# FelixBronnhuber/RenderBaby

Measured on AMD Instinct MI355X. Metric: Msamples/s (ray-segments/s), higher is better.
Workload: dtype f32; 1 GPU; C2 Cornell box (12 tris, 8 spheres, 1 area light), 1920x1080, 1024 spp, 8 bounces; width=1920, height=1080, spp=1024, max_depth=8, parallelism=single GPU, stripe_rows=8, walk=library default, tree_builder=, device=AMD Radeon Graphics (gfx950:sramecc+:xnack-, 256 CUs)

## Files before the change

include/rb_abi.h:

```cpp
#ifndef RB_ABI_H
#define RB_ABI_H

#include <stddef.h>
#include <stdint.h>

#ifdef __cplusplus
extern "C" {
#endif


typedef struct rb_camera {
    float pane_distance;
    float pane_width;
    float _pad0[2];
    float pos[3];
    float _pad1;
    float dir[3];
    float _pad2;
} rb_camera;

typedef struct rb_uniforms {
    uint32_t width;
    uint32_t height;
    uint32_t total_samples;
// ... 248 lines not shown
int rb_get_stats(rb_engine* e, rb_stats* out);
int rb_reset_stats(rb_engine* e);
int rb_last_dispatch_ms(rb_engine* e, float* ms);

int rb_bvh_build(const rb_gpu_triangle* tris, size_t n_tris,
                 rb_bvh_node* nodes_out, size_t nodes_capacity, size_t* n_nodes,
                 uint32_t* indices_out);

int rb_bvh_build_canonical(const rb_gpu_triangle* tris, size_t n_tris,
                           rb_bvh_node* nodes_out, size_t nodes_capacity, size_t* n_nodes,
                           uint32_t* indices_out);
int rb_bvh_build_device(int32_t device, const rb_gpu_triangle* tris, size_t n_tris,
                        rb_bvh_node* nodes_out, size_t nodes_capacity, size_t* n_nodes,
                        uint32_t* indices_out);
int rb_engine_tree(rb_engine* e, rb_bvh_node* nodes_out, size_t nodes_capacity, size_t* n_nodes,
                   uint32_t* indices_out, size_t indices_capacity, size_t* n_indices);
const char* rb_tree_builder(const rb_engine* e, float* build_ms);

int rb_debug_chunk_tree(const rb_gpu_triangle* tris, size_t n_tris, const rb_bvh_node* nodes, size_t n_nodes, const uint32_t* indices,
                        size_t n_indices, uint64_t out6[6]);
int rb_debug_engine_chunk_tree(rb_engine* e, uint64_t out6[6]);
typedef struct rb_debug_own_node {
    float lmin[3];
    uint32_t left;
    float lmax[3];
    uint32_t right;
    float rmin[3];
    float left_fa;
    float rmax[3];
    float right_fa;
} rb_debug_own_node;
typedef struct rb_debug_sphere_node {
    float cx[4], cy[4], cz[4], hx[4], hy[4], hz[4];
    uint32_t ref[4];
    uint32_t axes;
    uint32_t _pad[3];
} rb_debug_sphere_node;
int rb_debug_own_tree(const rb_gpu_triangle* tris, size_t n_tris, const rb_bvh_node* nodes, size_t n_nodes, const uint32_t* indices,
                      size_t n_indices, rb_debug_own_node* nodes_out, size_t nodes_capacity, uint32_t* slots_out, size_t slots_capacity,
                      uint32_t* slot_meta_out, size_t slot_meta_capacity, uint64_t counts3[3], uint32_t root_depth[2], float bounds6[6]);
int rb_debug_engine_own_tree(rb_engine* e, rb_debug_own_node* nodes_out, size_t nodes_capacity, uint32_t* slots_out, size_t slots_capacity,
                             uint32_t* slot_meta_out, size_t slot_meta_capacity, uint64_t counts3[3], uint32_t root_depth[2], float bounds6[6]);
int rb_debug_sphere_tree(const rb_sphere* spheres, size_t n, rb_debug_sphere_node* nodes_out, size_t nodes_capacity, float* leaf_out,
                         uint32_t* id_out, size_t spheres_capacity, uint64_t counts2[2], uint32_t root_depth[2]);
int rb_debug_engine_sphere_tree(rb_engine* e, rb_debug_sphere_node* nodes_out, size_t nodes_capacity, float* leaf_out, uint32_t* id_out,
                                size_t spheres_capacity, uint64_t counts2[2], uint32_t root_depth[2]);
const char* rb_chunk_tree_builder(const rb_engine* e, float* build_ms);
int rb_measure_l1_gather(int32_t device, uint64_t table_bytes, double* accesses_per_s);
int rb_debug_math(const float* a, const float* b, float* out8n, uint32_t n);
int rb_debug_walk_profile(uint64_t out64[64], int reset);
int rb_debug_rcp_exhaustive(uint32_t biased_exponent, uint32_t* out16);
int rb_debug_rcp_det_exhaustive(uint32_t biased_exponent, uint32_t* out16);
int rb_debug_triangle_trip(uint32_t n, uint32_t seed, uint32_t* out32);
int rb_debug_root_box(const float* rays, uint32_t n, const float* box6, uint32_t* out);
int rb_debug_normalize_sites(const float* xyz, uint32_t n, uint32_t n_unit, uint32_t seed0, uint32_t n_seeds, uint32_t* out16);
int rb_measure_salu_mix(int32_t device, uint32_t scalar_per_16, uint32_t branch, double* out3);
int rb_debug_rnd_pm1_exhaustive(uint32_t* out16);
int rb_debug_div_exhaustive(uint32_t b_begin, uint32_t b_count, uint32_t ea, uint32_t eb, uint32_t a_begin,
                            uint32_t a_count, unsigned long long* out16);

const char* rb_last_kernel_name(const rb_engine* e);

typedef struct rb_ray { float origin[3]; float _pad0; float dir[3]; float _pad1; } rb_ray;
enum { RB_HIT_NONE = 0, RB_HIT_GROUND = 1, RB_HIT_TRIANGLE = 2, RB_HIT_SPHERE = 3, RB_HIT_LIGHT = 4,
       RB_HIT_INVALID = 0xFFFFFFFFu };
typedef struct rb_hit {
    float t;
    uint32_t kind;
    uint32_t prim;
    uint32_t mesh;
    float u, v;
    uint32_t _pad[2];
    float normal[3];
    float _pad1;
} rb_hit;
typedef struct rb_surface {
    float albedo[3];
    uint32_t flags;
    float emissive[3];
    int32_t texture_index;
    float uv[2];
    float _pad[2];
} rb_surface;
int rb_cast_rays(rb_engine* e, const rb_ray* rays, size_t n, rb_hit* hits_out, rb_surface* surf_out);
int rb_render_hits(rb_engine* e, rb_hit* hits_out, rb_surface* surf_out);
int rb_pick(rb_engine* e, uint32_t px, uint32_t py, rb_hit* hit_out, rb_surface* surf_out);
const char* rb_last_query_kernel_name(const rb_engine* e);
int rb_last_query_ms(rb_engine* e, float* ms);

enum { RB_OCCL_VISIBLE = 0, RB_OCCL_OCCLUDED = 1, RB_OCCL_INVALID = 255 };
enum { RB_MASK_GROUND = 1, RB_MASK_TRIANGLES = 2, RB_MASK_SPHERES = 4, RB_MASK_LIGHTS = 8, RB_MASK_ALL = 15 };
int rb_occluded(rb_engine* e, const rb_ray* rays, const float* tmax, size_t n, uint32_t mask, uint8_t* out);
int rb_occluded_device(rb_engine* e, const rb_ray* d_rays, const float* d_tmax, size_t n, uint32_t mask, uint8_t* d_out);
int rb_cast_rays_device(rb_engine* e, const rb_ray* d_rays, size_t n, rb_hit* d_hits, rb_surface* d_surf);

typedef struct rb_radiance { float sum[3]; float weight; } rb_radiance;
#define RB_TRACE_PIECE_ITEMS (1u << 24)
int rb_trace_rays(rb_engine* e, const rb_ray* rays, const uint32_t* seeds, size_t n, uint32_t first_sample, uint32_t samples,
                  rb_radiance* out);
int rb_trace_rays_device(rb_engine* e, const rb_ray* d_rays, const uint32_t* d_seeds, size_t n, uint32_t first_sample,
                         uint32_t samples, rb_radiance* d_out);

enum { RB_CAM_PERSPECTIVE = 1, RB_CAM_ORTHO = 2, RB_CAM_EQUIRECT = 3 };
enum { RB_CAM_NO_JITTER = 1u };
typedef struct rb_camera_ex {
    uint32_t kind, width, height, flags;
    float pos[3];     float tan_half_fov;
    float right[3];   float half_width;
    float up[3];      float half_height;
    float forward[3]; float lens_radius;
    float focus_distance;
    uint32_t _reserved[3];
} rb_camera_ex;
#define RB_CAMERA_PIECE_ITEMS (1u << 23)
// ... 299 lines not shown
```

renderbaby_amd/_lib.py:

```python
import ctypes as C
import os

from . import abi

_HERE = os.path.dirname(os.path.abspath(__file__))
LIB_PATH = os.environ.get("RB_LIBRARY_PATH") or os.path.join(_HERE, "librenderbaby_hip.so")
_lib = None


P = C.POINTER
vp, u32, i32, sz = C.c_void_p, C.c_uint32, C.c_int, C.c_size_t
SIGNATURES = {
    "rb_create": (vp, [P(abi.Config)]),
    "rb_create_ex": (vp, [P(abi.Config), P(abi.Options)]),
    "rb_create_multi": (vp, [P(abi.Config), P(abi.Options), P(C.c_int32), u32]),
    "rb_comm_unique_id": (i32, [vp]),
    "rb_comm_available": (i32, []),
    "rb_comm_init_rank": (i32, [vp, vp, u32, u32]),
    "rb_comm_info": (i32, [vp, P(u32), P(u32), P(C.c_float)]),
    "rb_destroy": (None, [vp]),
    "rb_update": (i32, [vp, P(abi.Config)]),
    "rb_render": (i32, [vp, vp]),
    "rb_render_config": (i32, [vp, P(abi.Config), vp]),
    "rb_iter_begin": (i32, [vp, P(abi.Config)]),
    "rb_iter_has_next": (i32, [vp]),
    "rb_iter_next": (i32, [vp, vp]),
    "rb_iter_destroy": (None, [vp]),
    "rb_iter_set_passes_per_frame": (i32, [vp, u32]),
    "rb_last_error": (C.c_char_p, [vp]),
    "rb_get_size": (i32, [vp, P(u32), P(u32)]),
    "rb_clear": (i32, [vp]),
    "rb_dispatch": (i32, [vp, u32, u32]),
    "rb_reserve": (i32, [vp, u32]),
    "rb_sync": (i32, [vp]),
    "rb_read_rgba": (i32, [vp, vp]),
    "rb_read_accumulation": (i32, [vp, vp]),
    "rb_device_rgba": (i32, [vp, P(vp), P(sz)]),
    "rb_host_alloc": (vp, [sz]),
    "rb_host_free": (None, [vp]),
    "rb_local_rows": (i32, [vp, P(u32), P(u32)]),
    "rb_global_row": (i32, [vp, u32, P(u32)]),
    "rb_shard_layout": (i32, [u32, u32, u32, u32, P(u32), P(u32)]),
    "rb_shard_global_row": (u32, [u32, u32, u32, u32]),
    "rb_get_stats": (i32, [vp, P(abi.Stats)]),
    "rb_reset_stats": (i32, [vp]),
    "rb_last_dispatch_ms": (i32, [vp, P(C.c_float)]),
    "rb_bvh_build": (i32, [vp, sz, vp, sz, P(sz), vp]),
    "rb_bvh_build_canonical": (i32, [vp, sz, vp, sz, P(sz), vp]),
    "rb_bvh_build_device": (i32, [i32, vp, sz, vp, sz, P(sz), vp]),
    "rb_engine_tree": (i32, [vp, vp, sz, P(sz), vp, sz, P(sz)]),
    "rb_tree_builder": (C.c_char_p, [vp, vp]),
    "rb_debug_chunk_tree": (i32, [vp, sz, vp, sz, vp, sz, vp]),
    "rb_measure_l1_gather": (i32, [i32, C.c_uint64, P(C.c_double)]),
    "rb_debug_math": (i32, [vp, vp, vp, u32]),
    "rb_debug_walk_profile": (i32, [vp, i32]),
    "rb_debug_rcp_exhaustive": (i32, [u32, vp]),
    "rb_debug_rcp_det_exhaustive": (i32, [u32, vp]),
    "rb_debug_rnd_pm1_exhaustive": (i32, [vp]),
    "rb_debug_triangle_trip": (i32, [u32, u32, vp]),
    "rb_debug_root_box": (i32, [vp, u32, vp, vp]),
    "rb_debug_normalize_sites": (i32, [vp, u32, u32, u32, u32, vp]),
    "rb_measure_salu_mix": (i32, [i32, u32, u32, P(C.c_double)]),
    "rb_debug_div_exhaustive": (i32, [u32, u32, u32, u32, u32, u32, vp]),
    "rb_last_kernel_name": (C.c_char_p, [vp]),
    "rb_cast_rays": (i32, [vp, vp, sz, vp, vp]),
    "rb_render_hits": (i32, [vp, vp, vp]),
    "rb_pick": (i32, [vp, u32, u32, vp, vp]),
    "rb_occluded": (i32, [vp, vp, vp, sz, u32, vp]),
    "rb_occluded_device": (i32, [vp, vp, vp, sz, u32, vp]),
    "rb_cast_rays_device": (i32, [vp, vp, sz, vp, vp]),
    "rb_trace_rays": (i32, [vp, vp, vp, sz, u32, u32, vp]),
    "rb_trace_rays_device": (i32, [vp, vp, vp, sz, u32, u32, vp]),
    "rb_camera_rays": (i32, [i32, vp, C.c_uint64, sz, u32, u32, vp, vp]),
    "rb_trace_camera": (i32, [vp, vp, C.c_uint64, sz, u32, u32, vp]),
    "rb_trace_camera_device": (i32, [vp, vp, C.c_uint64, sz, u32, u32, vp]),
    "rb_last_camera_rays_ms": (i32, [vp, P(C.c_float)]),
    "rb_hemisphere_rays": (i32, [i32, vp, vp, sz, vp, u32, u32, vp, vp]),
    "rb_trace_hemisphere": (i32, [vp, vp, vp, sz, vp, u32, u32, vp]),
    "rb_trace_hemisphere_device": (i32, [vp, vp, vp, sz, vp, u32, u32, vp]),
    "rb_openness_hemisphere": (i32, [vp, vp, vp, sz, vp, u32, u32, vp]),
    "rb_openness_hemisphere_device": (i32, [vp, vp, vp, sz, vp, u32, u32, vp]),
    "rb_scene_emitters": (i32, [vp, vp, sz, P(sz)]),
    "rb_scene_emitters_device": (i32, [vp, vp, sz, vp]),
    "rb_light_rays": (i32, [i32, vp, sz, vp, vp, sz, vp, u32, u32, vp, vp, vp]),
    "rb_direct_light": (i32, [vp, vp, sz, vp, vp, sz, vp, u32, u32, vp]),
    "rb_direct_light_device": (i32, [vp, vp, sz, vp, vp, sz, vp, u32, u32, vp]),
    "rb_lightmap_surfels": (i32, [i32, vp, sz, vp, sz, vp, vp, vp]),
    "rb_lightmap_surfels_device": (i32, [vp, vp, vp, vp]),
    "rb_lightmap_resolve": (i32, [i32, u32, u32, vp, u32, vp]),
    "rb_bake_lightmap": (i32, [vp, vp, u32, u32, vp, vp]),
    "rb_bake_lightmap_device": (i32, [vp, vp, u32, u32, vp, vp]),
    "rb_last_lightmap_ms": (i32, [vp, P(C.c_float), P(C.c_float)]),
    "rb_probe_rays": (i32, [i32, vp, vp, sz, u32, u32, vp, vp]),
    "rb_bake_probes": (i32, [vp, vp, vp, sz, u32, u32, vp]),
    "rb_bake_probes_device": (i32, [vp, vp, vp, sz, u32, u32, vp]),
    "rb_last_probe_project_ms": (i32, [vp, P(C.c_float)]),
    "rb_probe_coefficients": (i32, [i32, vp, sz, vp]),
    "rb_probe_coefficients_device": (i32, [vp, vp, sz, vp]),
    "rb_light_points": (i32, [i32, vp, vp, vp, sz, vp]),
    "rb_light_points_device": (i32, [vp, vp, vp, vp, sz, vp]),
    "rb_bake_probe_depth": (i32, [vp, vp, vp, sz, u32, u32, C.c_float, vp]),
    "rb_bake_probe_depth_device": (i32, [vp, vp, vp, sz, u32, u32, C.c_float, vp]),
    "rb_last_probe_depth_project_ms": (i32, [vp, P(C.c_float)]),
    "rb_probe_moments": (i32, [i32, vp, sz, vp, vp]),
    "rb_probe_moments_device": (i32, [vp, vp, sz, vp, vp]),
    "rb_light_points_visible": (i32, [i32, vp, vp, vp, vp, sz, vp, vp]),
    "rb_light_points_visible_device": (i32, [vp, vp, vp, vp, vp, sz, vp, vp]),
    "rb_last_query_kernel_name": (C.c_char_p, [vp]),
    "rb_last_query_ms": (i32, [vp, P(C.c_float)]),
    "rb_denoise_default_params": (i32, [vp]),
    "rb_denoise_buffers": (i32, [i32, vp, u32, u32, vp, vp, vp, vp]),
    "rb_denoise": (i32, [vp, vp, vp, vp]),
# ... 62 lines not shown
```

renderbaby_amd/abi.py:

```python
import ctypes as C

import numpy as np

f4, u4, i4 = np.float32, np.uint32, np.int32

CAMERA = np.dtype([
    ("pane_distance", f4), ("pane_width", f4), ("_pad0", f4, (2,)),
    ("pos", f4, (3,)), ("_pad1", f4), ("dir", f4, (3,)), ("_pad2", f4)])

UNIFORMS = np.dtype([
    ("width", u4), ("height", u4), ("total_samples", u4), ("color_hash_enabled", u4),
    ("camera", CAMERA),
    ("spheres_count", u4), ("triangles_count", u4), ("bvh_node_count", u4),
    ("bvh_triangle_count", u4), ("bvh_root", u4), ("ground_height", f4),
    ("ground_enabled", u4), ("checkerboard_enabled", u4),
    ("sky_color", f4, (3,)), ("max_depth", u4),
    ("checkerboard_color_1", f4, (3,)), ("_pad1", u4),
    ("checkerboard_color_2", f4, (3,)), ("_pad2", u4)])

MATERIAL = np.dtype([
    ("ambient", f4, (3,)), ("_pad0", f4), ("diffuse", f4, (3,)), ("_pad1", f4),
    ("specular", f4, (3,)), ("shininess", f4), ("emissive", f4, (3,)), ("ior", f4),
    ("opacity", f4), ("illum", u4), ("texture_index", i4), ("_pad2", u4)])

# ... 37 lines not shown
PROBE_PIECE_ITEMS = 1 << 23
PROBE_GRID = np.dtype([("origin", f4, (3,)), ("_pad0", u4), ("step", f4, (3,)), ("_pad1", u4), ("counts", u4, (3,)), ("flags", u4)])
LIT = np.dtype([("value", f4, (3,)), ("weight", f4)])
LIGHT_PIECE_POINTS = 1 << 22
PROBE_DEPTH = np.dtype([("texel", f4, (64, 4))])
LIGHT_VISIBILITY = np.dtype([("normal_bias", f4), ("min_visibility", f4), ("flags", u4), ("_pad", u4)])
VIS_NO_WRAP, VIS_NO_DEPTH = 1, 2
EMITTER = np.dtype([("a", f4, (3,)), ("kind", u4), ("b", f4, (3,)), ("prim", u4), ("c", f4, (3,)), ("area", f4),
                    ("emissive", f4, (3,)), ("_pad", f4)])
LIGHT_PARAMS = np.dtype([("offset", f4), ("shorten", f4), ("mask", u4), ("flags", u4), ("_reserved", u4, (4,))])
MAX_EMITTERS = 1 << 24
OCCL_VISIBLE, OCCL_OCCLUDED, OCCL_INVALID = 0, 1, 255
MASK_GROUND, MASK_TRIANGLES, MASK_SPHERES, MASK_LIGHTS, MASK_ALL = 1, 2, 4, 8, 15
GUIDE = np.dtype([("normal", f4, (3,)), ("t", f4), ("pos", f4, (3,)), ("cls", u4), ("albedo", f4, (3,)), ("_pad", f4)])
DENOISE_PARAMS = np.dtype([("iterations", u4), ("normal_power_log2", u4), ("sigma_depth", f4), ("sigma_color", f4),
                           ("albedo_floor", f4), ("flags", u4), ("_reserved", u4, (2,))])
VIEW = np.dtype([("pos", f4, (3,)), ("cx", f4), ("right", f4, (3,)), ("cy", f4), ("up", f4, (3,)), ("sx", f4), ("fwd", f4, (3,)), ("sy", f4)])
REPROJECT_PARAMS = np.dtype([("sigma_depth", f4), ("normal_min", f4), ("albedo_floor", f4), ("max_history", f4), ("flags", u4),
                             ("_reserved", u4, (3,))])
FRAME_RECORD = np.dtype([("mean", f4, (3,)), ("count", f4)])
OWN_NODE = np.dtype([("lmin", f4, (3,)), ("left", u4), ("lmax", f4, (3,)), ("right", u4),
                     ("rmin", f4, (3,)), ("left_fa", f4), ("rmax", f4, (3,)), ("right_fa", f4)])
SPHERE_NODE = np.dtype([("cx", f4, (4,)), ("cy", f4, (4,)), ("cz", f4, (4,)), ("hx", f4, (4,)), ("hy", f4, (4,)), ("hz", f4, (4,)),
                        ("ref", u4, (4,)), ("axes", u4), ("_pad", u4, (3,))])

SIZES = {"camera": (CAMERA, 48), "uniforms": (UNIFORMS, 144), "material": (MATERIAL, 80),
         "sphere": (SPHERE, 96), "point_light": (POINT_LIGHT, 96), "mesh": (MESH, 96),
         "bvh_node": (BVH_NODE, 48), "gpu_triangle": (GPU_TRIANGLE, 64),
         "ray": (RAY, 32), "hit": (HIT, 48), "surface": (SURFACE, 48),
         "guide": (GUIDE, 48), "denoise_params": (DENOISE_PARAMS, 32), "view": (VIEW, 64),
         "reproject_params": (REPROJECT_PARAMS, 32), "frame_record": (FRAME_RECORD, 16), "camera_ex": (CAMERA_EX, 96),
         "surfel": (SURFEL, 32), "hemi_params": (HEMI_PARAMS, 32), "openness": (OPENNESS, 8),
         "lightmap_params": (LIGHTMAP_PARAMS, 32), "probe": (PROBE, 16), "sh9": (SH9, 112),
         "probe_grid": (PROBE_GRID, 48), "lit": (LIT, 16),
         "probe_depth": (PROBE_DEPTH, 1024), "light_visibility": (LIGHT_VISIBILITY, 16),
         "emitter": (EMITTER, 64), "light_params": (LIGHT_PARAMS, 32),
         "own_node": (OWN_NODE, 64), "sphere_node": (SPHERE_NODE, 128)}
for _n, (_dt, _sz) in SIZES.items():
    assert _dt.itemsize == _sz, (_n, _dt.itemsize, _sz)

KEEP, CREATE, UPDATE, DELETE = 0, 1, 2, 3

RB_OK = 0
ERR = {
    1: "PaneDistanceOutOfBounds", 2: "PaneWidthOutOfBounds", 3: "InvalidCameraDirection",
    4: "InvalidUniforms", 5: "InvalidSpheres", 6: "InvalidUVs", 7: "InvalidMeshes",
    8: "InvalidLights", 9: "InvalidTextures", 10: "CannotDeleteNonexistent",
    11: "UniformsNotInitialized", 12: "NoMoreFrames", 13: "InvalidBVH", 14: "UnsupportedDelete",
    15: "NullArgument", 16: "Device", 17: "NotInitialized", 18: "InvalidOptions"}
RB_ERR_NO_MORE_FRAMES = 12
RB_ERR_DEVICE = 16

KERNEL_DEFAULT, KERNEL_PIXEL, KERNEL_QUEUE, KERNEL_STREAM = 0, 1, 2, 3
FLAG_STATS = 1
FLAG_NO_SPHERE_BVH = 2
FLAG_FAST_BVH = 4
FLAG_DEVICE_BVH = 8
FLAG_DEVICE_LBVH = 16
FLAG_REFERENCE_WALK = 32
FLAG_HOST_BVH = 64
FLAG_GATHER_PEER_COPY = 128
FLAG_NO_RUN_AHEAD = 256
FLAG_SKIP_NEAR_DEGENERATE = 512
FLAG_CHUNK_WALK = 1024
FLAG_SPHERE_TREE_HOST = 2048
FLAG_SPHERE_TREE_DEVICE = 4096
FLAG_CHUNK_TREE_HOST = 8192
FLAG_CHUNK_TREE_DEVICE = 16384
FLAG_BUILD_TREE = 32768
FLAG_BUILD_TREE_HOST = 65536
COMM_ID_BYTES = 128


class Field(C.Structure):
    _fields_ = [("change", C.c_uint32), ("ptr", C.c_void_p), ("count", C.c_size_t)]


class Config(C.Structure):
    _fields_ = [(n, Field) for n in ("uniforms", "spheres", "uvs", "meshes", "lights", "bvh_nodes",
                                      "bvh_indices", "bvh_triangles", "textures")]


class Texture(C.Structure):
    _fields_ = [("width", C.c_uint32), ("height", C.c_uint32), ("rgba_data", C.c_void_p)]


class Options(C.Structure):
    _fields_ = [("device", C.c_int32), ("shard_rank", C.c_uint32), ("shard_count", C.c_uint32),
                ("stripe_rows", C.c_uint32), ("passes_per_launch", C.c_uint32), ("kernel", C.c_uint32),
                ("flags", C.c_uint32), ("_reserved", C.c_uint32 * 5)]


class Ray(C.Structure):
    _fields_ = [("origin", C.c_float * 3), ("_pad0", C.c_float), ("dir", C.c_float * 3), ("_pad1", C.c_float)]


class Hit(C.Structure):
    _fields_ = [("t", C.c_float), ("kind", C.c_uint32), ("prim", C.c_uint32), ("mesh", C.c_uint32), ("u", C.c_float),
                ("v", C.c_float), ("_pad", C.c_uint32 * 2), ("normal", C.c_float * 3), ("_pad1", C.c_float)]


class Surface(C.Structure):
    _fields_ = [("albedo", C.c_float * 3), ("flags", C.c_uint32), ("emissive", C.c_float * 3),
                ("texture_index", C.c_int32), ("uv", C.c_float * 2), ("_pad", C.c_float * 2)]


# ... 17 lines not shown
```

renderbaby_amd/csrc/rb_debug.hip:

```cpp
#include <algorithm>

#include "rb_device_shade.hpp"

#pragma clang fp contract(off)

namespace rb {
namespace {

__global__ void k_rcp_exhaustive(uint32_t expo, uint32_t* mismatch) {
    const uint32_t m = blockIdx.x * blockDim.x + threadIdx.x;
    if (m >= (1u << 23)) return;
    for (uint32_t sign = 0; sign < 2; sign++) {
        const uint32_t bits = (sign << 31) | ((expo & 0xFFu) << 23) | m;
        const float b = __uint_as_float(bits);
        float want, got;
        if (expo & 0x100u) {
            if (sign) continue;
            want = sqrtf(b);
            got = sqrt_exact(b);
        } else {
            if (!rcp_safe(b)) continue;
            want = 1.0f / b;
            got = rcp_newton(b);
        }
// ... 60 lines not shown
DEV void trip_case(uint32_t k, f3& o, f3& d, f3& v0, f3& e1, f3& e2) {
    o = mk(0.25f, 0.25f, -1.0f);
    d = mk(0.0f, 0.0f, 1.0f);
    v0 = mk(0.0f, 0.0f, 0.0f);
    e1 = mk(0.0f, 1.0f, 0.0f);
    e2 = mk(1.0f, 0.0f, 0.0f);
    const uint32_t eps = 0x358637BDu, big = 0x71800000u, one = 0x3F800000u, tmin = 0x3A83126Fu;
    const float nan = __uint_as_float(0x7FC00000u), inf = __uint_as_float(0x7F800000u);
    switch (k) {
        case 0: case 1: case 2: e1.y = __uint_as_float(eps - 1u + k); break;
        case 3: case 4: case 5: e1.y = -__uint_as_float(eps - 1u + (k - 3u)); break;
        case 6: case 7: case 8: e1.y = __uint_as_float(big - 1u + (k - 6u)); break;
        case 9: e1.y = -0x1p100f; break;
        case 10: e1.y = 0x1p120f; break;
        case 11: e1.y = __uint_as_float(0x3F80FFFFu); break;
        case 12: e1.y = __uint_as_float(0xC123FFFFu); break;
        case 13: e1.y = __uint_as_float(0x3FFFFFFFu); break;
        case 14: o.y = 0.0f; break;
        case 15: o.y = -0.0f; break;
        case 16: o.y = -0x1p-149f; break;
        case 17: o.y = 1.0f; o.x = 0.0f; break;
        case 18: o.y = __uint_as_float(one + 1u); o.x = 0.0f; break;
        case 19: o.x = 0.0f; break;
        case 20: o.x = -0.0f; break;
        case 21: o.x = -0x1p-149f; break;
        case 22: o.x = 0.75f; break;
        case 23: o.x = 0.75f; o.y = __uint_as_float(0x3E800001u); break;
        case 24: o.z = -__uint_as_float(tmin); break;
        case 25: o.z = -__uint_as_float(tmin + 1u); break;
        case 26: o.z = -__uint_as_float(tmin - 1u); break;
        case 27: o.z = 0.0f; break;
        case 28: o.z = 1.0f; break;
        case 29: o.x = nan; break;
        case 30: o.y = nan; break;
        case 31: o.z = nan; break;
        case 32: d.x = nan; break;
        case 33: d.y = nan; break;
        case 34: d.z = nan; break;
        case 35: o.x = inf; break;
        case 36: o.y = -inf; break;
        case 37: o.z = -inf; break;
        case 38: d.x = inf; break;
        case 39: d.y = -inf; break;
        case 40: d.z = inf; break;
        case 41: e1.y = 0.0f; break;
        case 42: e1.y = nan; break;
        default: e2.x = inf; break;
    }
}
DEV float trip_unit(uint32_t& s) {
    s = pcg(s);
    return (float)(int32_t)s * 0x1p-31f;
}
__global__ void __launch_bounds__(256) k_triangle_trip(uint32_t n_waves, uint32_t seed, uint32_t* mismatch) {
    const uint32_t wave = (blockIdx.x * 256u + threadIdx.x) >> 6, lane = threadIdx.x & 63u;
    if (wave >= n_waves + kTripCases) return;
    f3 o, d, v0, e1, e2;
    float hit_t = 1e20f;
    bool on = true;
    if (wave < n_waves) {
        uint32_t sw = pcg(seed ^ (wave * 0x9E3779B9u)), sl = pcg(sw + lane * 0x85EBCA6Bu + 1u);
        const uint32_t kind = pcg(sw) & 15u;
        const float scale = kind == 0u ? 0x1p-10f : kind == 1u ? 0x1p52f : 1.0f;
        v0 = mk(trip_unit(sw), trip_unit(sw), trip_unit(sw));
        e1 = scale * mk(trip_unit(sw), trip_unit(sw), trip_unit(sw));
        e2 = scale * mk(trip_unit(sw), trip_unit(sw), trip_unit(sw));
        o = 2.0f * mk(trip_unit(sl), trip_unit(sl), trip_unit(sl));
        const float a = 0.7f * trip_unit(sl) + 0.5f, b = 0.7f * trip_unit(sl) + 0.5f;
        const f3 to = (v0 + a * e1 + b * e2) - o;
        d = __builtin_amdgcn_rsqf(dot(to, to) + 1e-30f) * to;
        const uint32_t r = pcg(sl);
        if (r & 1u) hit_t = 2.0f * (float)(r >> 8) * 0x1p-24f;
        on = (r & 6u) != 0u;
    } else {
        trip_case(wave - n_waves, o, d, v0, e1, e2);
        on = (lane & 8u) == 0u;
    }
    auto uni = [](float x) { return __uint_as_float((uint32_t)__builtin_amdgcn_readfirstlane((int)__float_as_uint(x))); };
    const v4f ra = {uni(v0.x), uni(v0.y), uni(v0.z), 0.0f}, rb_ = {uni(e1.x), uni(e1.y), uni(e1.z), 0.0f},
              rc = {uni(e2.x), uni(e2.y), uni(e2.z), 1.0f};
    const uint32_t slot = (uint32_t)__builtin_amdgcn_readfirstlane((int)(wave + 1u));
    if (wave >= n_waves) {
        TriHit own;
        own.t = 1e20f, own.u = 0.0f, own.v = 0.0f, own.slot = 0u, own.hit = false;
        accept_slot<true>(ra, rb_, rc, slot, o, d, own);
        const uint32_t v = lane & 3u;
        hit_t = v == 0u ? 1e20f : v == 1u ? 0.5f : v == 2u ? own.t : __uint_as_float(__float_as_uint(own.t) + 1u);
    }
    TriHit want, got;
    want.t = hit_t, want.u = -2.0f, want.v = -3.0f, want.slot = 0xABCDu, want.hit = false;
    got = want;
    float big = 0x1p100f;
    if constexpr (RB_TRIP_BLOCK) asm("s_mov_b32 %0, 0x71800000" : "=s"(big));
    if (on) {
        accept_slot<true>(ra, rb_, rc, slot, o, d, want);
        if constexpr (RB_TRIP_BLOCK) accept_trip<RB_TRIP_ASM - 1>(ra, rb_, rc, slot, o, d, big, got);
        else accept_slot<true>(ra, rb_, rc, slot, o, d, got);
    }
    if (__float_as_uint(want.t) != __float_as_uint(got.t) || __float_as_uint(want.u) != __float_as_uint(got.u) ||
        __float_as_uint(want.v) != __float_as_uint(got.v) || want.slot != got.slot) {
        if (atomicAdd(&mismatch[0], 1u) == 0u) {
            mismatch[1] = wave * 64u + lane;
            const float in[16] = {o.x, o.y, o.z, d.x, d.y, d.z, ra.x, ra.y, ra.z, rb_.x, rb_.y, rb_.z, rc.x, rc.y, rc.z, hit_t};
            for (int k = 0; k < 16; k++) mismatch[2 + k] = __float_as_uint(in[k]);
            mismatch[18] = __float_as_uint(got.t), mismatch[19] = __float_as_uint(got.u), mismatch[20] = __float_as_uint(got.v);
            mismatch[21] = got.slot;
            mismatch[22] = __float_as_uint(want.t), mismatch[23] = __float_as_uint(want.u), mismatch[24] = __float_as_uint(want.v);
            mismatch[25] = want.slot;
        }
    }
}

template <int SALU, bool BRANCH>
__global__ void __launch_bounds__(256, 8) k_salu_mix(uint32_t rounds, float c, float* sink, unsigned long long* stamp) {
    float v[16];
#pragma unroll
    for (int k = 0; k < 16; k++) v[k] = (float)(threadIdx.x + k) * 0x1p-20f;
    const float c2 = c * 0x1p-20f;
    uint32_t s0 = rounds, s1 = rounds + 1u, s2 = rounds + 2u, s3 = rounds + 3u;
    const unsigned long long t0 = __builtin_amdgcn_s_memtime(), r0 = __builtin_amdgcn_s_memrealtime();
#define RB_MIX_F(k) "v_fmac_f32_e32 %" #k ", %[c], %[c2]\n\t"
#define RB_MIX_S(j) "s_add_u32 %[s" #j "], %[s" #j "], 1\n\t"
#define RB_MIX_Q0(a, b, c, d) RB_MIX_F(a) RB_MIX_F(b) RB_MIX_F(c) RB_MIX_F(d)
#define RB_MIX_Q1(a, b, c, d) RB_MIX_F(a) RB_MIX_F(b) RB_MIX_S(0) RB_MIX_F(c) RB_MIX_F(d)
#define RB_MIX_Q2(a, b, c, d) RB_MIX_F(a) RB_MIX_S(0) RB_MIX_F(b) RB_MIX_F(c) RB_MIX_S(1) RB_MIX_F(d)
#define RB_MIX_Q3(a, b, c, d) RB_MIX_F(a) RB_MIX_S(0) RB_MIX_F(b) RB_MIX_S(1) RB_MIX_F(c) RB_MIX_S(2) RB_MIX_F(d)
#define RB_MIX_Q4(a, b, c, d) RB_MIX_F(a) RB_MIX_S(0) RB_MIX_F(b) RB_MIX_S(1) RB_MIX_F(c) RB_MIX_S(2) RB_MIX_F(d) RB_MIX_S(3)
#define RB_MIX_BR "s_cbranch_execz .Lmix_out_%=\n\t"
#define RB_MIX_GROUP(Q, BR) Q(0, 1, 2, 3) Q(4, 5, 6, 7) Q(8, 9, 10, 11) Q(12, 13, 14, 15) BR
#define RB_MIX_ASM(Q, BR)                                                                                                 \
    asm volatile(RB_MIX_GROUP(Q, BR) RB_MIX_GROUP(Q, BR) RB_MIX_GROUP(Q, BR) RB_MIX_GROUP(Q, BR) ".Lmix_out_%=:"          \
                 : "+v"(v[0]), "+v"(v[1]), "+v"(v[2]), "+v"(v[3]), "+v"(v[4]), "+v"(v[5]), "+v"(v[6]), "+v"(v[7]), "+v"(v[8]), \
                   "+v"(v[9]), "+v"(v[10]), "+v"(v[11]), "+v"(v[12]), "+v"(v[13]), "+v"(v[14]), "+v"(v[15]), [s0] "+s"(s0), \
                   [s1] "+s"(s1), [s2] "+s"(s2), [s3] "+s"(s3)                                                            \
                 : [c] "v"(c), [c2] "v"(c2)                                                                                             \
                 : "scc")
    for (uint32_t r = rounds; r != 0u; r--) {
        if constexpr (BRANCH) {
            if constexpr (SALU == 0) RB_MIX_ASM(RB_MIX_Q0, RB_MIX_BR);
            else if constexpr (SALU == 4) RB_MIX_ASM(RB_MIX_Q1, RB_MIX_BR);
            else if constexpr (SALU == 8) RB_MIX_ASM(RB_MIX_Q2, RB_MIX_BR);
            else if constexpr (SALU == 12) RB_MIX_ASM(RB_MIX_Q3, RB_MIX_BR);
            else RB_MIX_ASM(RB_MIX_Q4, RB_MIX_BR);
        } else {
            if constexpr (SALU == 0) RB_MIX_ASM(RB_MIX_Q0, "");
            else if constexpr (SALU == 4) RB_MIX_ASM(RB_MIX_Q1, "");
            else if constexpr (SALU == 8) RB_MIX_ASM(RB_MIX_Q2, "");
            else if constexpr (SALU == 12) RB_MIX_ASM(RB_MIX_Q3, "");
            else RB_MIX_ASM(RB_MIX_Q4, "");
// ... 165 lines not shown
    while (lines * 2 * 128 <= table_bytes) lines *= 2;
    float4 *table = nullptr, *sink = nullptr;
    if (hipMalloc(reinterpret_cast<void**>(&table), lines * 128) != hipSuccess) return 0.0;
    if (hipMalloc(reinterpret_cast<void**>(&sink), 16) != hipSuccess) { (void)hipFree(table); return 0.0; }
    (void)hipMemset(table, 0, lines * 128);
    hipEvent_t t0, t1;
    (void)hipEventCreate(&t0);
    (void)hipEventCreate(&t1);
    double best = 0.0;
    for (int shape = 0; shape < 4; shape++) {
        const uint32_t inflight = (shape & 1) ? 16u : 8u, blocks = device_cu_count_cached() * ((shape & 2) ? 8u : 4u);
        for (int rep = 0; rep < 2; rep++) {
            (void)hipEventRecord(t0, nullptr);
            if (inflight == 16u) hipLaunchKernelGGL(k_l1_gather<16>, dim3(blocks), dim3(256), 0, nullptr, table, (uint32_t)(lines - 1), rounds, sink);
            else hipLaunchKernelGGL(k_l1_gather<8>, dim3(blocks), dim3(256), 0, nullptr, table, (uint32_t)(lines - 1), rounds, sink);
            (void)hipEventRecord(t1, nullptr);
            if (hipEventSynchronize(t1) != hipSuccess) break;
            float ms = 0.0f;
            (void)hipEventElapsedTime(&ms, t0, t1);
            if (ms > 0.0f) best = std::max(best, (double)blocks * 256.0 * rounds * inflight / (ms * 1e-3));
        }
    }
    (void)hipEventDestroy(t0);
    (void)hipEventDestroy(t1);
    (void)hipFree(table);
    (void)hipFree(sink);
    return best;
}
}
}

extern "C" {

int rb_debug_rcp_exhaustive(uint32_t biased_exponent, uint32_t* out16) {
    if (!out16) return RB_ERR_NULL_ARGUMENT;
    return rb::round_trip(out16, 64, 64, [&](uint32_t* d) {
        hipLaunchKernelGGL(rb::k_rcp_exhaustive, dim3((1u << 23) / 256), dim3(256), 0, nullptr, biased_exponent, d);
    });
}

int rb_debug_rcp_det_exhaustive(uint32_t biased_exponent, uint32_t* out16) {
    if (!out16) return RB_ERR_NULL_ARGUMENT;
    if (biased_exponent > 255u) return RB_ERR_INVALID_OPTIONS;
    return rb::round_trip(out16, 64, 64, [&](uint32_t* d) {
        hipLaunchKernelGGL(rb::k_rcp_det_exhaustive, dim3((1u << 23) / 256), dim3(256), 0, nullptr, biased_exponent, d);
    });
}

int rb_debug_triangle_trip(uint32_t n, uint32_t seed, uint32_t* out32) {
    if (!out32) return RB_ERR_NULL_ARGUMENT;
    if (n > (1u << 26)) return RB_ERR_INVALID_OPTIONS;
    return rb::round_trip(out32, 128, 128, [&](uint32_t* d) {
        const uint32_t n_waves = (n + 63u) / 64u, waves = n_waves + rb::kTripCases;
        hipLaunchKernelGGL(rb::k_triangle_trip, dim3((waves + 3u) / 4u), dim3(256), 0, nullptr, n_waves, seed, d);
    });
}

int rb_debug_root_box(const float* rays, uint32_t n, const float* box6, uint32_t* out) {
    if (!rays || !box6 || !out) return RB_ERR_NULL_ARGUMENT;
    if (n == 0u) return RB_OK;
    if (n > (1u << 24)) return RB_ERR_INVALID_OPTIONS;
    const size_t out_bytes = (size_t)n * 4u, in_bytes = (size_t)n * 24u;
    const rb::f3 bmin = {box6[0], box6[1], box6[2]}, bmax = {box6[3], box6[4], box6[5]};
    return rb::round_trip(out, out_bytes, out_bytes + in_bytes, [&](uint32_t* d) {
        float* dr = reinterpret_cast<float*>(d + n);
        (void)hipMemcpy(dr, rays, in_bytes, hipMemcpyHostToDevice);
        hipLaunchKernelGGL(rb::k_root_box, dim3((n + 255u) / 256u), dim3(256), 0, nullptr, dr, n, bmin, bmax, d);
    });
}

int rb_debug_normalize_sites(const float* xyz, uint32_t n, uint32_t n_unit, uint32_t seed0, uint32_t n_seeds, uint32_t* out16) {
    if (!out16 || (!xyz && n + n_unit != 0u)) return RB_ERR_NULL_ARGUMENT;
    if (n > (1u << 26) || n_unit > (1u << 26) || n_seeds > (1u << 26)) return RB_ERR_INVALID_OPTIONS;
    const size_t total = (size_t)n + n_unit + n_seeds, in_bytes = ((size_t)n + n_unit) * 12u;
    if (total == 0u) {
        std::fill(out16, out16 + 16, 0u);
        return RB_OK;
    }
    return rb::round_trip(out16, 64, 64 + in_bytes, [&](uint32_t* d) {
        float* dv = reinterpret_cast<float*>(d + 16);
        if (in_bytes) (void)hipMemcpy(dv, xyz, in_bytes, hipMemcpyHostToDevice);
        hipLaunchKernelGGL(rb::k_normalize_sites, dim3((uint32_t)((total + 255u) / 256u)), dim3(256), 0, nullptr, dv, n, n_unit, seed0, n_seeds, d);
    });
}

int rb_measure_salu_mix(int32_t device, uint32_t scalar_per_16, uint32_t branch, double* out3) {
    if (!out3) return RB_ERR_NULL_ARGUMENT;
    if (scalar_per_16 > 16u || (scalar_per_16 & 3u) != 0u) return RB_ERR_INVALID_OPTIONS;
    int before = -1;
    if (device >= 0 && (hipGetDevice(&before) != hipSuccess || hipSetDevice(device) != hipSuccess)) return RB_ERR_DEVICE;
    const bool ok = rb::measure_salu_mix(scalar_per_16, branch != 0u, 4096u, out3);
    if (before >= 0) (void)hipSetDevice(before);
    return ok ? RB_OK : RB_ERR_DEVICE;
}

int rb_debug_rnd_pm1_exhaustive(uint32_t* out16) {
    if (!out16) return RB_ERR_NULL_ARGUMENT;
    return rb::round_trip(out16, 64, 64, [&](uint32_t* d) {
        hipLaunchKernelGGL(rb::k_rnd_pm1_exhaustive, dim3(1u << 16), dim3(256), 0, nullptr, d);
    });
}

int rb_debug_div_exhaustive(uint32_t b_begin, uint32_t b_count, uint32_t ea, uint32_t eb, uint32_t a_begin,
                            uint32_t a_count, unsigned long long* out16) {
    if (!out16) return RB_ERR_NULL_ARGUMENT;
    return rb::round_trip(out16, 128, 128, [&](unsigned long long* d) {
        hipLaunchKernelGGL(rb::k_div_exhaustive, dim3((b_count + 255) / 256), dim3(256), 0, nullptr, b_begin, ea, eb, a_begin, a_count, d);
// ... 24 lines not shown
```

renderbaby_amd/csrc/rb_device_intersect.hpp:

```cpp
#pragma once
#include "rb_device_math.hpp"

#pragma clang fp contract(off)

namespace rb {
namespace {

DEV f3 sample_texture(const KParams& p, int32_t index, float uvx, float uvy) {
    if (index < 0) {
        if (p.u.checkerboard_enabled > 0u) {
            int32_t u2 = f2i(floorf(uvx * 10.0f));
            int32_t v2 = f2i(floorf(uvy * 10.0f));
            int32_t sum = (int32_t)((uint32_t)u2 + (uint32_t)v2);
            return (sum % 2 == 0) ? ld3(p.u.checkerboard_color_1) : ld3(p.u.checkerboard_color_2);
        }
        return mk(1.0f, 1.0f, 1.0f);
    }
    if ((uint32_t)index >= p.n_tex) return mk(0.0f, 0.0f, 0.0f);
    const v4u iw = ((cu4p)p.tex_info)[index];
    rb_texture_info info;
    info.offset = iw.x;
    info.width = iw.y;
    info.height = iw.z;
    float u = uvx - floorf(uvx);
    float v = uvy - floorf(uvy);
    uint32_t x = min(f2u(u * (float)info.width), info.width - 1u);
    uint32_t y = min(f2u((1.0f - v) * (float)info.height), info.height - 1u);
    const uint32_t pixel = cptr(p.tex_data)[info.offset + y * info.width + x];
    const RB_CONST float* lut = cptr(p.srgb_lut);
    return mk(lut[pixel & 255u], lut[(pixel >> 8) & 255u], lut[(pixel >> 16) & 255u]);
}

DEV float isect_sphere(f3 o, f3 d, float a, f3 center, float radius) {
    f3 oc = o - center;
    float half_b = dot(oc, d);
    float c = dot(oc, oc) - radius * radius;
    float disc = half_b * half_b - a * c;
    if (disc < 0.0f) return -1.0f;
    float sqrtd = sqrtf(disc);
    float root = (-half_b - sqrtd) / a;
    if (root <= 0.001f) {
        root = (-half_b + sqrtd) / a;
        if (root <= 0.001f) return -1.0f;
    }
    return root;
}

DEV float isect_triangle(f3 o, f3 d, f3 v0, f3 edge1, f3 edge2, float& uo, float& vo) {
    const f3 h = cross(d, edge2);
    const float a = dot(edge1, h);
    if (fabsf(a) < 1e-6f) return -1.0f;
    const float f = rcp_tri(a);
    const f3 s = o - v0;
    const float u = f * dot(s, h);
    if (u < 0.0f || u > 1.0f) return -1.0f;
    const f3 q = cross(s, edge1);
    const float v = f * dot(d, q);
    if (v < 0.0f || u + v > 1.0f) return -1.0f;
    const float t = f * dot(edge2, q);
    if (t > 0.0f) {
        uo = u;
        vo = v;
// ... 27 lines not shown
    asm("" : "+s"(a));
    return a < 0x7F800000u;
}
DEV uint64_t root_inside_mask(f3 o, f3 d, f3 bmin, f3 bmax) {
    return __builtin_amdgcn_fcmpf(o.x, bmin.x, 2) & __builtin_amdgcn_fcmpf(o.x, bmax.x, 4) & __builtin_amdgcn_fcmpf(o.y, bmin.y, 2) &
           __builtin_amdgcn_fcmpf(o.y, bmax.y, 4) & __builtin_amdgcn_fcmpf(o.z, bmin.z, 2) & __builtin_amdgcn_fcmpf(o.z, bmax.z, 4) &
           __builtin_amdgcn_fcmpf(d.x, d.y, 7) & __builtin_amdgcn_fcmpf(d.z, d.z, 7);
}
DEV bool root_inside(f3 o, f3 d, f3 bmin, f3 bmax) { return ((root_inside_mask(o, d, bmin, bmax) >> __lane_id()) & 1ull) != 0ull; }
constexpr uint32_t kBoxUnknown = 0u, kBoxMiss = 1u, kBoxHit = 2u;

DEV float isect_ground(f3 o, f3 d, float ground_height) {
    if (fabsf(d.y) < 1e-6f) return -1.0f;
    float t = (ground_height - o.y) / d.y;
    return (t > 0.0f) ? t : -1.0f;
}

template <bool STATS>
struct Tally {
    uint32_t segments = 0, paths = 0;
    unsigned long long nodes = 0, tris = 0, spheres = 0, lights = 0, mesh_hits = 0;
};
template <>
struct Tally<false> {
    uint32_t segments = 0, paths = 0;
};

DEV unsigned long long wave_sum(unsigned long long v) {
    for (int off = 32; off > 0; off >>= 1) v += __shfl_xor(v, off, 64);
    return v;
}
template <bool STATS>
DEV void flush_tally(const Tally<STATS>& t, unsigned long long* counters) {
    unsigned long long seg = wave_sum((unsigned long long)t.segments);
    unsigned long long pth = wave_sum((unsigned long long)t.paths);
    const bool lead = (__lane_id() == 0);
    if (lead) {
        atomicAdd(&counters[C_SEGMENTS], seg);
        atomicAdd(&counters[C_PATHS], pth);
    }
    if constexpr (STATS) {
        unsigned long long a = wave_sum(t.nodes), b = wave_sum(t.tris), c = wave_sum(t.spheres),
                           d = wave_sum(t.lights), e = wave_sum(t.mesh_hits);
        if (lead) {
            atomicAdd(&counters[C_NODES], a);
            atomicAdd(&counters[C_TRIS], b);
            atomicAdd(&counters[C_SPHERES], c);
            atomicAdd(&counters[C_LIGHTS], d);
            atomicAdd(&counters[C_MESH_HITS], e);
        }
    }
}

struct TriHit {
    float t, u, v;
    uint32_t slot;
    bool hit;
};

DEV void test_slot(const v4f a, const v4f b, const v4f c, uint32_t slot, f3 o, f3 d, TriHit& h) {
    float u, v;
    const float t = isect_triangle(o, d, mk(a.x, a.y, a.z), mk(b.x, b.y, b.z), mk(c.x, c.y, c.z), u, v);
    if (t > 0.001f && t < h.t) {
        h.hit = true;
        h.t = t;
        h.u = u;
        h.v = v;
        h.slot = slot;
    }
}

template <bool DET = false>
DEV void accept_slot(const v4f a, const v4f b, const v4f c, uint32_t slot, f3 o, f3 d, TriHit& hit) {
    const f3 v0 = mk(a.x, a.y, a.z), edge1 = mk(b.x, b.y, b.z), edge2 = mk(c.x, c.y, c.z);
    const f3 h = cross(d, edge2);
    const float det = dot(edge1, h);
    if (!(fabsf(det) < 1e-6f)) {
        const float f = DET ? rcp_det(det) : rcp_tri(det);
        const f3 s = o - v0;
        const float u = f * dot(s, h);
        if (!(u < 0.0f || u > 1.0f)) {
            const f3 q = cross(s, edge1);
            const float v = f * dot(d, q);
            if (!(v < 0.0f || u + v > 1.0f)) {
                const float t = f * dot(edge2, q);
                if (t > 0.0f && t > 0.001f && t < hit.t) {
                    hit.t = t;
                    hit.u = u;
                    hit.v = v;
                    hit.slot = slot;
                }
            }
        }
    }
}

#ifndef RB_TRIP_PLAIN
#define RB_TRIP_PLAIN 1
#endif
#ifndef RB_TRIP_ASM
#define RB_TRIP_ASM 3
#endif
#define RB_TRIP_BLOCK (RB_TRIP_ASM != 0 && RB_FAST_RCP && RB_RCP_DET)

template <int SKIP>
DEV void accept_trip(const v4f a, const v4f b, const v4f c, uint32_t slot, f3 o, f3 d, float big, TriHit& hit) {
    float r8, r10, r11, r12, r13, r14, r15, r16, r17;
    uint64_t entry, keep, m, ds;
#define RB_TRIP_HEAD                                                                                                     \
    "s_mov_b64 %[entry], exec\n\t"                                                                                       \
    "v_mul_f32_e32 %[r8], %[cz], %[dy]\n\t"                                                                              \
    "v_mul_f32_e32 %[r10], %[cy], %[dz]\n\t"                                                                             \
    "v_sub_f32_e32 %[r10], %[r8], %[r10]\n\t"                                                                            \
    "v_mul_f32_e32 %[r8], %[cx], %[dz]\n\t"                                                                              \
    "v_mul_f32_e32 %[r11], %[cz], %[dx]\n\t"                                                                             \
    "v_sub_f32_e32 %[r11], %[r8], %[r11]\n\t"                                                                            \
    "v_mul_f32_e32 %[r8], %[cy], %[dx]\n\t"                                                                              \
    "v_mul_f32_e32 %[r12], %[cx], %[dy]\n\t"                                                                             \
    "v_sub_f32_e32 %[r12], %[r8], %[r12]\n\t"                                                                            \
    "v_mul_f32_e32 %[r8], %[bx], %[r10]\n\t"                                                                             \
    "v_mul_f32_e32 %[r13], %[by], %[r11]\n\t"                                                                            \
    "v_add_f32_e32 %[r8], %[r8], %[r13]\n\t"                                                                             \
    "v_mul_f32_e32 %[r13], %[bz], %[r12]\n\t"                                                                            \
    "v_add_f32_e32 %[r13], %[r13], %[r8]\n\t"                                                                            \
    "v_cmpx_nlt_f32_e64 vcc, |%[r13]|, %[eps]\n\t"                                                  \
    "v_cmp_eq_u16_e64 %[m], -1, %[r13]\n\t"                                     \
    "v_cmp_nlt_f32_e64 vcc, |%[r13]|, %[big]\n\t"                                               \
    "v_rcp_f32_e32 %[r8], %[r13]\n\t"                                                                                    \
    "s_or_b64 %[m], vcc, %[m]\n\t"                                                                                       \
    "v_fma_f32 %[r14], -%[r13], %[r8], 1.0\n\t"                                                                          \
    "v_fmac_f32_e32 %[r8], %[r14], %[r8]\n\t"                                                                            \
    "s_and_saveexec_b64 %[keep], %[m]\n\t"                                                                               \
    "s_cbranch_execz .Ltrip_rcp_%=\n\t"                                                                                  \
    "v_div_scale_f32 %[r8], %[ds], %[r13], %[r13], 1.0\n\t"                   \
    "v_rcp_f32_e32 %[r14], %[r8]\n\t"                                                                                    \
    "v_div_scale_f32 %[r15], vcc, 1.0, %[r13], 1.0\n\t"                                                                  \
    "v_fma_f32 %[r16], -%[r8], %[r14], 1.0\n\t"                                                                          \
    "v_fmac_f32_e32 %[r14], %[r16], %[r14]\n\t"                                                                          \
    "v_mul_f32_e32 %[r16], %[r15], %[r14]\n\t"                                                                           \
    "v_fma_f32 %[r17], -%[r8], %[r16], %[r15]\n\t"                                                                       \
    "v_fmac_f32_e32 %[r16], %[r17], %[r14]\n\t"                                                                          \
    "v_fma_f32 %[r8], -%[r8], %[r16], %[r15]\n\t"                                                                        \
    "v_div_fmas_f32 %[r8], %[r8], %[r14], %[r16]\n\t"                                                                    \
    "v_div_fixup_f32 %[r8], %[r8], %[r13], 1.0\n"                                                                        \
    ".Ltrip_rcp_%=:\n\t"                                                                                                 \
    "s_mov_b64 exec, %[keep]\n\t"                                                                                        \
    "v_subrev_f32_e32 %[r13], %[ax], %[ox]\n\t"                                                                          \
    "v_subrev_f32_e32 %[r14], %[ay], %[oy]\n\t"                                                                          \
    "v_subrev_f32_e32 %[r15], %[az], %[oz]\n\t"                                                                          \
    "v_mul_f32_e32 %[r10], %[r13], %[r10]\n\t"                                                                           \
    "v_mul_f32_e32 %[r11], %[r14], %[r11]\n\t"                                                                           \
    "v_add_f32_e32 %[r10], %[r10], %[r11]\n\t"                                                                           \
    "v_mul_f32_e32 %[r11], %[r15], %[r12]\n\t"                                                                           \
    "v_add_f32_e32 %[r10], %[r11], %[r10]\n\t"                                                                           \
    "v_mul_f32_e32 %[r10], %[r10], %[r8]\n\t"                                                                     \
    "v_cmpx_ngt_f32_e32 vcc, 0, %[r10]\n\t"                                                                \
    "v_cmpx_nlt_f32_e32 vcc, 1.0, %[r10]\n\t"
#define RB_TRIP_TAIL                                                                                                     \
    "v_mul_f32_e32 %[r11], %[bz], %[r14]\n\t"                                                                            \
    "v_mul_f32_e32 %[r12], %[by], %[r15]\n\t"                                                                            \
    "v_sub_f32_e32 %[r12], %[r11], %[r12]\n\t"                                                                           \
    "v_mul_f32_e32 %[r11], %[bx], %[r15]\n\t"                                                                            \
    "v_mul_f32_e32 %[r15], %[bz], %[r13]\n\t"                                                                            \
    "v_sub_f32_e32 %[r15], %[r11], %[r15]\n\t"                                                                           \
    "v_mul_f32_e32 %[r11], %[by], %[r13]\n\t"                                                                            \
    "v_mul_f32_e32 %[r13], %[bx], %[r14]\n\t"                                                                            \
    "v_sub_f32_e32 %[r13], %[r11], %[r13]\n\t"                                                                           \
    "v_mul_f32_e32 %[r11], %[dx], %[r12]\n\t"                                                                            \
    "v_mul_f32_e32 %[r14], %[dy], %[r15]\n\t"                                                                            \
    "v_add_f32_e32 %[r11], %[r11], %[r14]\n\t"                                                                           \
    "v_mul_f32_e32 %[r14], %[dz], %[r13]\n\t"                                                                            \
    "v_add_f32_e32 %[r11], %[r14], %[r11]\n\t"                                                                           \
    "v_mul_f32_e32 %[r11], %[r11], %[r8]\n\t"                                                                     \
    "v_add_f32_e32 %[r14], %[r10], %[r11]\n\t"                                                                           \
    "v_cmpx_ngt_f32_e32 vcc, 0, %[r11]\n\t"                                                                \
    "v_cmpx_nlt_f32_e32 vcc, 1.0, %[r14]\n\t"
#define RB_TRIP_LAST                                                                                                     \
    "v_mul_f32_e32 %[r12], %[cx], %[r12]\n\t"                                                                            \
    "v_mul_f32_e32 %[r14], %[cy], %[r15]\n\t"                                                                            \
    "v_add_f32_e32 %[r12], %[r12], %[r14]\n\t"                                                                           \
    "v_mul_f32_e32 %[r13], %[cz], %[r13]\n\t"                                                                            \
    "v_add_f32_e32 %[r12], %[r13], %[r12]\n\t"                                                                           \
    "v_mul_f32_e32 %[r8], %[r12], %[r8]\n\t"                                                                      \
    "v_cmpx_lt_f32_e32 vcc, %[tmin], %[r8]\n\t"                                                           \
    "v_cmpx_lt_f32_e32 vcc, %[r8], %[ht]\n\t"                                                             \
    "v_mov_b32_e32 %[hs], %[slot]\n\t"                                                                                   \
    "v_mov_b32_e32 %[hv], %[r11]\n\t"                                                                                    \
    "v_mov_b32_e32 %[ht], %[r8]\n\t"                                                                                     \
    "v_mov_b32_e32 %[hu], %[r10]\n"
#define RB_TRIP_OPERANDS                                                                                                 \
    : [ht] "+v"(hit.t), [hu] "+v"(hit.u), [hv] "+v"(hit.v), [hs] "+v"(hit.slot), [r8] "=&v"(r8), [r10] "=&v"(r10),        \
      [r11] "=&v"(r11), [r12] "=&v"(r12), [r13] "=&v"(r13), [r14] "=&v"(r14), [r15] "=&v"(r15), [r16] "=&v"(r16),         \
      [r17] "=&v"(r17), [entry] "=&s"(entry), [keep] "=&s"(keep), [m] "=&s"(m), [ds] "=&s"(ds)                            \
    : [ax] "s"(a.x), [ay] "s"(a.y), [az] "s"(a.z), [bx] "s"(b.x), [by] "s"(b.y), [bz] "s"(b.z), [cx] "s"(c.x),            \
      [cy] "s"(c.y), [cz] "s"(c.z), [slot] "s"(slot), [ox] "v"(o.x), [oy] "v"(o.y), [oz] "v"(o.z), [dx] "v"(d.x),         \
      [dy] "v"(d.y), [dz] "v"(d.z), [eps] "s"(1e-6f), [big] "s"(big), [tmin] "s"(0.001f)                             \
    : "vcc", "scc"
#define RB_TRIP_SKIP "s_cbranch_execz .Ltrip_end_%=\n\t"
    if constexpr (SKIP == 2) {
        asm volatile(RB_TRIP_HEAD RB_TRIP_SKIP RB_TRIP_TAIL RB_TRIP_SKIP RB_TRIP_LAST ".Ltrip_end_%=:\n\t"
                     "s_mov_b64 exec, %[entry]" RB_TRIP_OPERANDS);
    } else if constexpr (SKIP == 1) {
        asm volatile(RB_TRIP_HEAD RB_TRIP_SKIP RB_TRIP_TAIL RB_TRIP_LAST ".Ltrip_end_%=:\n\t"
                     "s_mov_b64 exec, %[entry]" RB_TRIP_OPERANDS);
    } else {
        asm volatile(RB_TRIP_HEAD RB_TRIP_TAIL RB_TRIP_LAST "\ts_mov_b64 exec, %[entry]" RB_TRIP_OPERANDS);
    }
#undef RB_TRIP_SKIP
#undef RB_TRIP_HEAD
#undef RB_TRIP_TAIL
#undef RB_TRIP_LAST
#undef RB_TRIP_OPERANDS
}


DEV float cone_cos_bound(f3 d, v4f cone) {
    const float y = fabsf(__builtin_fmaf(d.z, cone.z, __builtin_fmaf(d.y, cone.y, d.x * cone.x)));
    const float k2 = __builtin_fmaf(cone.z, cone.z, __builtin_fmaf(cone.y, cone.y, cone.x * cone.x));
    const float root = 1.000001f * __builtin_amdgcn_sqrtf(fmaxf(__builtin_fmaf(-y, y, k2), 0.0f) + 4e-6f * k2);
    return __builtin_fmaf(-cone.w, root, y - 1e-6f);
}
DEV bool cone_admits_grazing(f3 d, v4f cone) {
    if (cone.w < 0.0f) return false;
    return !(cone_cos_bound(d, cone) >= kFastGrazeCos);
}
constexpr float kFastKF = 27.0f * 5.9604645e-8f * 1.01f;
constexpr float kFastKS = 20.0f * 5.9604645e-8f * 1.01f;
template <bool STATS>
struct FastWalk {
    f3 o, d, inv;
    float m_ref;
    TriHit h;
    uint32_t best_rank;
    uint32_t cur;
    uint32_t gend;
    bool graze;
    int sp;

    DEV void begin(const KParams& p, f3 o_, f3 d_) {
        o = o_;
        d = d_;
        h.hit = false;
        h.t = 1e20f;
        h.u = 0.0f;
        h.v = 0.0f;
        h.slot = 0u;
        best_rank = 0xFFFFFFFFu;
        inv = mk(rcp_exact(d.x), rcp_exact(d.y), rcp_exact(d.z));
        const f3 fb0 = ld3(p.fast_bmin), fb1 = ld3(p.fast_bmax);
        const float sx_ = fmaxf(fabsf(o.x - fb0.x), fabsf(o.x - fb1.x)), sy_ = fmaxf(fabsf(o.y - fb0.y), fabsf(o.y - fb1.y)),
                    sz_ = fmaxf(fabsf(o.z - fb0.z), fabsf(o.z - fb1.z));
        m_ref = 1e-6f * sqrtf(sx_ * sx_ + sy_ * sy_ + sz_ * sz_) + 1e-30f;
        cur = p.fast_root;
        gend = 0u;
        graze = false;
        sp = 0;
    }
    DEV bool at_leaf() const { return (cur & 0x80000000u) != 0u; }
    DEV uint32_t kind() const { return (graze ? 2u : 0u) | (cur >> 31); }

    DEV static volatile uint32_t* spill(const KParams& p, int at) {
        return p.stack_overflow + ((size_t)(uint32_t)(at - (int)kStackDepth) * (gridDim.x * blockDim.x) + blockIdx.x * blockDim.x + threadIdx.x);
    }
    DEV static void push(const KParams& p, uint32_t* stack, uint32_t stride, int at, uint32_t v) {
        if (__builtin_expect(at < (int)kStackDepth, 1)) stack[at * stride] = v;
// ... 150 lines not shown
            const float tn = fmaxf(fmaxf(fminf(t0.x, t1.x), fminf(t0.y, t1.y)), fminf(t0.z, t1.z));
            const float tf = fminf(fminf(fmaxf(t0.x, t1.x), fmaxf(t0.y, t1.y)), fmaxf(t0.z, t1.z));
            const bool finite = (t0.x == t0.x) && (t0.y == t0.y) && (t0.z == t0.z) && (t1.x == t1.x) && (t1.y == t1.y) &&
                                (t1.z == t1.z);
            if (thick && finite && tf >= fmaxf(tn, 0.0f)) return true;
        }
        uint32_t n = leaf_node;
        for (;;) {
            const v4f n0 = rnodes[n * 3u], n1 = rnodes[n * 3u + 1u];
            if constexpr (STATS) tl.nodes++;
            if (!isect_aabb(o, inv, mk(n0.x, n0.y, n0.z), mk(n1.x, n1.y, n1.z))) return false;
            if (n == 0u) return true;
            n = parent[n];
        }
    }

    DEV bool leaf_step(const KParams& p, uint32_t* stack, uint32_t stride, Tally<STATS>& tl) {
        const cf4p ftris = (cf4p)p.fast_tris;
        const RB_CONST uint32_t* fslots = cptr(p.fast_slots);
        const RB_CONST uint32_t* meta = cptr(p.slot_meta);
        const uint32_t first = cur & 0x0FFFFFFFu, count = ((cur >> 28) & 3u) + 1u;
        for (uint32_t j = first; j < first + count; j++) {
            const v4f a = ftris[j * 4u], b = ftris[j * 4u + 1u], c = ftris[j * 4u + 2u];
            if constexpr (STATS) tl.tris++;
            float u, v;
            const float t = isect_triangle(o, d, mk(a.x, a.y, a.z), mk(b.x, b.y, b.z), mk(c.x, c.y, c.z), u, v);
            if (t > 0.001f && !(t > h.t)) {
                const uint32_t slot = fslots[j];
                const uint32_t leaf_node = meta[slot * 2u], rank = meta[slot * 2u + 1u] & ~kSlotLarge;
                if ((t < h.t || rank < best_rank) && reference_would_test(p, leaf_node, tl)) {
                    h.hit = true;
                    h.t = t;
                    h.u = u;
                    h.v = v;
                    h.slot = slot;
                    best_rank = rank;
                    if constexpr (STATS) tl.mesh_hits++;
                }
            }
        }
        return pop(p, stack, stride);
    }
};

template <bool STATS>
DEV TriHit intersect_bvh_fast(const KParams& p, f3 o, f3 d, uint32_t* stack, uint32_t stride, Tally<STATS>& tl) {
    FastWalk<STATS> w;
    w.begin(p, o, d);
    while (w.step(p, stack, stride, tl)) {
    }
    return w.h;
}

template <bool STATS, bool MULTI = true, bool TRIP = false>
DEV TriHit intersect_bvh(const KParams& p, f3 o, f3 d, uint32_t* stack, uint32_t stride, Tally<STATS>& tl, uint32_t box = kBoxUnknown) {
    TriHit h;
    h.hit = false;
    h.t = 1e20f;
    h.u = 0.0f;
    h.v = 0.0f;
    h.slot = 0u;
    const uint32_t node_count = p.u.bvh_node_count;
    if (node_count == 0u) return h;
    if constexpr (MULTI) {
        if (p.fast_nodes != nullptr) return intersect_bvh_fast<STATS>(p, o, d, stack, stride, tl);
    }
    constexpr bool skip_box = TRIP && !MULTI && RB_ROOT_INSIDE != 0;
    const f3 inv = skip_box ? d : mk(rcp_exact(d.x), rcp_exact(d.y), rcp_exact(d.z));
    const cf4p nodes = (cf4p)p.nodes;
    const cf4p ptris = (cf4p)p.ptris;

    if (node_count == 1u) {
        const v4f n0 = nodes[0], n1 = nodes[1];
        const v4u n2 = ((cu4p)p.nodes)[2];
        if constexpr (STATS) tl.nodes++;
        const uint32_t first = n2.z, count = n2.w;
        const uint32_t end = (first + count < p.index_len) ? first + count : p.index_len;
        auto in_box = [&]() {
            const f3 b0 = mk(n0.x, n0.y, n0.z), b1 = mk(n1.x, n1.y, n1.z);
            if constexpr (skip_box) {
                const uint64_t unknown = __builtin_amdgcn_uicmp(box, kBoxUnknown, 32) & ~root_inside_mask(o, d, b0, b1);
                if (__builtin_expect(unknown == 0ull && box_finite(b0, b1), 1)) return box != kBoxMiss;
                return isect_aabb(o, mk(rcp_exact(d.x), rcp_exact(d.y), rcp_exact(d.z)), b0, b1);
            } else {
                return isect_aabb(o, inv, b0, b1);
            }
        };
        if (first < end && in_box()) {
            constexpr bool trip = TRIP && !MULTI;
            float big = 0x1p100f;
            if constexpr (trip && RB_TRIP_BLOCK) asm("s_mov_b32 %0, 0x71800000" : "=s"(big));
            auto test = [&](const v4f a, const v4f b, const v4f c, uint32_t slot) {
                if constexpr (STATS) tl.tris++;
                const float before = h.t;
                if constexpr (trip && RB_TRIP_BLOCK) accept_trip<RB_TRIP_ASM - 1>(a, b, c, slot, o, d, big, h);
                else accept_slot<!MULTI>(a, b, c, slot, o, d, h);
                if constexpr (STATS) tl.mesh_hits += (h.t != before) ? 1u : 0u;
            };
            if constexpr (trip && RB_TRIP_PLAIN != 0) {
                cf4p rec = ptris + (size_t)first * 4u;
                for (uint32_t slot = first; slot != end; slot++, rec += 4) {
                    v4f a = rec[0], b = rec[1], c = rec[2];
                    uint32_t live = __float_as_uint(c.w);
                    asm volatile("" : "+s"(a.x), "+s"(b.x), "+s"(live));
                    if (live != 0u) test(a, b, c, slot);
                }
            } else {
                const uint32_t last = end - 1u;
                cf4p rec = ptris + (size_t)first * 4u;
                v4f a = rec[0], b = rec[1], c = rec[2];
                bool live = __float_as_uint(c.w) != 0u;
                for (uint32_t slot = first;; slot++) {
                    if (slot < last) rec += 4;
                    const v4f na = rec[0], nb = rec[1], nc = rec[2];
                    if (live) test(a, b, c, slot);
                    if (slot == last) break;
                    a = na;
                    b = nb;
                    c = nc;
                    live = __float_as_uint(nc.w) != 0u;
                }
            }
            h.hit = h.t < 1e20f;
        }
        return h;
    }
    if constexpr (!MULTI) return h;

    int sp = 0;
    stack[0] = 0u;
    sp = 1;
    while (sp > 0) {
        sp--;
        const uint32_t node_idx = stack[sp * stride];
        if (node_idx >= node_count) continue;
        const v4f n0 = nodes[node_idx * 3u], n1 = nodes[node_idx * 3u + 1u];
        const v4u n2 = ((cu4p)p.nodes)[node_idx * 3u + 2u];
        if constexpr (STATS) tl.nodes++;
        if (!isect_aabb(o, inv, mk(n0.x, n0.y, n0.z), mk(n1.x, n1.y, n1.z))) continue;
        const uint32_t left = n2.x, right = n2.y, first = n2.z, count = n2.w;
        if (count > 0u) {
            for (uint32_t i = 0; i < count; i++) {
                const uint32_t slot = first + i;
                if (slot >= p.index_len) continue;
                const v4f a = ptris[slot * 4u], b = ptris[slot * 4u + 1u], c = ptris[slot * 4u + 2u];
                if (__float_as_uint(c.w) == 0u) continue;
                if constexpr (STATS) tl.tris++;
                const float before = h.t;
// ... 33 lines not shown
```

renderbaby_amd/csrc/rb_device_shade.hpp:

```cpp
#pragma once
#include "rb_device_intersect.hpp"

#pragma clang fp contract(off)

namespace rb {
namespace {

DEV const KParams& fresh_params(const KParams&) {
    const RB_CONST char* k = (const RB_CONST char*)__builtin_amdgcn_kernarg_segment_ptr();
    asm volatile("" : "+s"(k));
    return *(const KParams*)k;
}

struct Mat {
    f3 diffuse, specular, emissive;
    float fuzz;
    bool metal;
    int32_t tex;
};
DEV Mat load_mat(const rb_material* m) {
    const cf4p q = (cf4p)m;
    const v4f d = q[1], s = q[2], e = q[3];
    const v4u t = ((cu4p)m)[4];
    Mat r;
// ... 67 lines not shown
    const bool h0 = r0 != kSphNone, h1 = r1 != kSphNone, h2 = r2 != kSphNone;
    if (r3 != kSphNone && (h0 || h1 || h2)) push(r3);
    if (h2 && (h0 || h1)) push(r2);
    if (h1 && h0) push(r1);
    return h0 ? r0 : h1 ? r1 : h2 ? r2 : r3;
}

DEV void intersect_spheres_bvh(const KParams& p, f3 o, f3 d, float a, float& closest_t, uint32_t& sphere_idx,
                               uint32_t* stack, uint32_t stride, unsigned long long* n_tested) {
    const f3 inv = mk(__builtin_amdgcn_rcpf(d.x), __builtin_amdgcn_rcpf(d.y), __builtin_amdgcn_rcpf(d.z));
    const uint32_t dneg = sph_dir_signs(d);
    const cf4p leafs = (cf4p)p.sph_leaf;
    const RB_CONST uint32_t* ids = cptr(p.sph_id);
    float best = closest_t;
    uint32_t best_id = 0xFFFFFFFFu, cur = p.sph_root;
    int sp = 0;
    for (;;) {
        if (cur != kSphNone && (cur & 0x80000000u) == 0u) {
            cur = sphere_node_step(p, cur, o, inv, dneg, best, [&](uint32_t ref) {
                stack[sp * stride] = ref;
                sp++;
            });
            if (cur != kSphNone) continue;
        } else if (cur != kSphNone) {
            const uint32_t first = sph_leaf_first(cur), count = sph_leaf_count(cur);
            for (uint32_t j = first; j < first + count; j++) {
                const v4f cr = leafs[j];
                const uint32_t id = ids[j];
                if (n_tested) (*n_tested)++;
                const float t = isect_sphere(o, d, a, mk(cr.x, cr.y, cr.z), cr.w);
                if (t > 0.001f && (t < best || (t == best && best_id != 0xFFFFFFFFu && id < best_id))) {
                    best = t;
                    best_id = id;
                }
            }
        }
        if (sp == 0) break;
        sp--;
        cur = stack[sp * stride];
    }
    if (best_id != 0xFFFFFFFFu) {
        closest_t = best;
        sphere_idx = best_id;
    }
}

struct SegState {
    float closest_t;
    uint32_t kind;
    float uvx, uvy;
    bool use_tex, tri_won_a;
};

template <bool STATS>
DEV SegState segment_pre(const KParams& p, const Path& pt, const TriHit th, Tally<STATS>& tl) {
    const f3 o = pt.o, d = pt.d;
    tl.segments++;

    float closest_t = 1e20f;
    uint32_t kind = K_NONE;
    float uvx = 0.0f, uvy = 0.0f;
    bool use_tex = false;

    if (p.u.ground_enabled > 0u) {
        const float t = isect_ground(o, d, p.u.ground_height);
        if (t > 0.001f && t < closest_t) {
            closest_t = t;
            kind = K_GROUND;
            const f3 gp = o + t * d;
            uvx = gp.x;
            uvy = gp.z;
            use_tex = true;
        }
    }

    const bool tri_won_a = th.hit && th.t < closest_t;
    if (tri_won_a) {
        closest_t = th.t;
        kind = K_TRI;
    }

    SegState st;
    st.closest_t = closest_t;
    st.kind = kind;
    st.uvx = uvx;
    st.uvy = uvy;
    st.use_tex = use_tex;
    st.tri_won_a = tri_won_a;
    return st;
}

#ifndef RB_SCAN_LEAN
#define RB_SCAN_LEAN 1
#endif
#ifndef RB_SCAN_RECORD
#define RB_SCAN_RECORD 1
#endif
#ifndef RB_PASS2_MAD24
#define RB_PASS2_MAD24 1
#endif
DEV uint32_t shift_in_ge0(uint32_t cand, float x, float y) {
    const uint64_t ge = __builtin_amdgcn_fcmpf(x, y, 11 );
    uint32_t out;
    uint64_t carry;
    asm("v_addc_co_u32 %0, %1, %2, %2, %3" : "=v"(out), "=s"(carry) : "v"(cand), "s"(ge));
    return out;
}
template <bool STATS, bool SPHTREE = true, bool LEAN = false>
// ... 5 lines not shown
        if (p.sph_nodes != nullptr) {
            unsigned long long* cnt = nullptr;
            if constexpr (STATS) cnt = &tl.spheres;
            intersect_spheres_bvh(p, o, d, a, closest_t, sphere_idx, stack, stride, cnt);
            return;
        }
    }
    constexpr bool lean = LEAN && RB_SCAN_LEAN != 0;
    constexpr bool record = lean && RB_SCAN_RECORD != 0;
    for (uint32_t base = 0; base < ns; base += 32u) {
        uint32_t cand = 0u;
        if constexpr (lean) {
            const uint32_t n = (uint32_t)__builtin_amdgcn_readfirstlane((int)((ns - base < 32u) ? ns - base : 32u));
            constexpr uint32_t step = record ? 1u : 6u;
            cf4p sp_ = (record ? (cf4p)p.sph_scan : sph4) + (size_t)(base + n) * step;
            for (uint32_t k = n; k != 0u; k--) {
                sp_ -= step;
                const v4f cr = sp_[0];
                if constexpr (STATS) tl.spheres++;
                const f3 oc = o - mk(cr.x, cr.y, cr.z);
                const float half_b = dot(oc, d);
                const float c = dot(oc, oc) - (record ? cr.w : cr.w * cr.w);
                cand = shift_in_ge0(cand, half_b * half_b, a * c);
            }
        } else {
            const uint32_t n = (ns - base < 32u) ? ns - base : 32u;
            cf4p sp_ = sph4 + (size_t)base * 6u;
            for (uint32_t k = 0; k < n; k++, sp_ += 6) {
                const v4f cr = sp_[0];
                if constexpr (STATS) tl.spheres++;
                const f3 oc = o - mk(cr.x, cr.y, cr.z);
                const float half_b = dot(oc, d);
                const float c = dot(oc, oc) - cr.w * cr.w;
                const float disc = half_b * half_b - a * c;
                cand |= (disc < 0.0f) ? 0u : (1u << k);
            }
        }
        while (cand != 0u) {
            const uint32_t k = (uint32_t)__ffs((int)cand) - 1u;
            cand &= cand - 1u;
            const v4f cr = (LEAN && RB_PASS2_MAD24 != 0) ? (sph4 + (size_t)base * 6u)[__umul24(k, 6u)] : sph4[(base + k) * 6u];
            const float t = isect_sphere(o, d, a, mk(cr.x, cr.y, cr.z), cr.w);
            if (t > 0.001f && t < closest_t) {
                closest_t = t;
                sphere_idx = base + k;
            }
        }
    }
}

#ifndef RB_ONE_NORMALIZE
#define RB_ONE_NORMALIZE 1
#endif
template <bool STATS, bool PARK = true, bool JOINED = true, bool TRIM = false>
DEV bool segment_post(const KParams& p, Path& pt, const TriHit th, const SegState st, float closest_t, uint32_t sphere_idx,
                      Tally<STATS>& tl) {
    const f3 o = pt.o, d = pt.d;
    const float a = dot(d, d);
    uint32_t kind = st.kind;
    float uvx = st.uvx, uvy = st.uvy;
    bool use_tex = st.use_tex;
    const bool tri_won_a = st.tri_won_a;
    [[maybe_unused]] const uint32_t ns = p.u.spheres_count;
    [[maybe_unused]] const cf4p sph4 = (cf4p)p.spheres;
    if (sphere_idx != 0xFFFFFFFFu) kind = K_SPHERE;

    uint32_t light_idx = 0xFFFFFFFFu;
    const cf4p lgt4 = (cf4p)p.lights;
    for (uint32_t base = 0; base < p.n_lights; base += 32u) {
        const uint32_t n = (p.n_lights - base < 32u) ? p.n_lights - base : 32u;
        uint32_t cand = 0u;
        for (uint32_t k = 0; k < n; k++) {
            const v4f cr = lgt4[(base + k) * 6u];
            if constexpr (STATS) tl.lights++;
            const f3 oc = o - mk(cr.x, cr.y, cr.z);
            const float half_b = dot(oc, d);
            const float c = dot(oc, oc) - cr.w * cr.w;
            const float disc = half_b * half_b - a * c;
            cand |= (disc < 0.0f) ? 0u : (1u << k);
        }
        while (cand != 0u) {
            const uint32_t k = (uint32_t)__ffs((int)cand) - 1u;
            cand &= cand - 1u;
            const v4f cr = lgt4[(base + k) * 6u];
            const float t = isect_sphere(o, d, a, mk(cr.x, cr.y, cr.z), cr.w);
            if (t > 0.001f && t < closest_t) {
                closest_t = t;
                light_idx = base + k;
            }
        }
    }
    if (light_idx != 0xFFFFFFFFu) kind = K_LIGHT;

    if (kind == K_NONE) {
        pt.color = pt.color + pt.att * ld3(p.u.sky_color);
        return false;
    }

    const f3 pos = o + closest_t * d;
    f3 normal = mk(0.0f, 1.0f, 0.0f);
    Mat m;
    m.diffuse = mk(0, 0, 0);
    m.specular = mk(0, 0, 0);
    m.emissive = mk(0, 0, 0);
    m.fuzz = 1.0f;
    m.metal = false;
    m.tex = -1;
    if (tri_won_a) {
// ... 10 lines not shown
            if (kind == K_TRI) {
                m = load_mat(mm);
                use_tex = m.tex >= 0;
            } else {
                use_tex = load_tex_index(mm) >= 0;
            }
        }
    }
    if (kind == K_GROUND) {
        m.diffuse = mk(0.5f, 0.5f, 0.5f);
    } else if (kind == K_TRI) {
        const v4f s = ((cf4p)p.ptris)[th.slot * 4u + 3u];
        normal = mk(s.x, s.y, s.z);
    } else {
        if (sphere_idx != 0xFFFFFFFFu) {
            const rb_sphere* s = p.spheres + sphere_idx;
            if (kind == K_SPHERE) {
                m = load_mat(&s->material);
                use_tex = m.tex >= 0;
                const v4f cr = ((cf4p)s)[0];
                normal = normalize_for<TRIM>(pos - mk(cr.x, cr.y, cr.z));
            } else {
                use_tex = load_tex_index(&s->material) >= 0;
            }
        }
        if (kind == K_LIGHT) {
            const rb_point_light* l = p.lights + light_idx;
            m = load_mat(&l->material);
            const v4f cr = ((cf4p)l)[0];
            normal = normalize_for<TRIM>(pos - mk(cr.x, cr.y, cr.z));
        }
    }

    const bool is_metal = m.metal;

    pt.color = pt.color + pt.att * m.emissive;

    const f3 ruv = random_unit_vector<PARK, TRIM && PARK>(pt.seed);
    f3 scattered, albedo;
    bool absorbed = false;
    constexpr bool one_norm = JOINED && RB_ONE_NORMALIZE != 0;
    const f3 sd = normal + ruv;
    f3 nin = sd;
    if constexpr (one_norm) nin = normalize_for<TRIM>(is_metal ? d : sd);
    if (is_metal) {
        const f3 reflected = reflect_vector(one_norm ? nin : normalize_for<TRIM>(d), normal);
        scattered = reflected + m.fuzz * ruv;
        absorbed = dot(scattered, normal) <= 0.0f;
        albedo = m.specular;
    } else {
        scattered = near_zero(sd) ? normal : (one_norm ? nin : normalize_for<TRIM>(sd));
        albedo = m.diffuse;
        if (use_tex) {
            if (tri_won_a) tri_uv(p, th, uvx, uvy);
            albedo = albedo * sample_texture(p, m.tex, uvx, uvy);
        }
    }
    if (absorbed) return false;
    pt.att = pt.att * albedo;
    pt.o = pos + 0.001f * normal;
    pt.d = normalize_for<TRIM>(scattered);
    pt.depth++;
    return pt.depth < p.u.max_depth;
}

struct HitQuads {
    v4f h0, h1, h2, s0, s1, s2;
};
DEV void hit_quads_empty(HitQuads& out, uint32_t kind, f3 emissive) {
    const uint32_t none = 0xFFFFFFFFu;
    out.h0 = v4f{1e20f, __uint_as_float(kind), __uint_as_float(none), __uint_as_float(none)};
    out.h1 = out.h2 = out.s0 = out.s2 = v4f{0.0f, 0.0f, 0.0f, 0.0f};
    out.s1 = v4f{emissive.x, emissive.y, emissive.z, __uint_as_float(none)};
}
DEV void segment_resolve(const KParams& p, f3 o, f3 d, const TriHit th, const SegState st, float closest_t, uint32_t sphere_idx,
                         HitQuads& out) {
    const float a = dot(d, d);
    uint32_t kind = st.kind;
    float uvx = st.uvx, uvy = st.uvy;
    bool use_tex = st.use_tex;
    const bool tri_won_a = st.tri_won_a;
    if (sphere_idx != 0xFFFFFFFFu) kind = K_SPHERE;

    uint32_t light_idx = 0xFFFFFFFFu;
    const cf4p lgt4 = (cf4p)p.lights;
    for (uint32_t base = 0; base < p.n_lights; base += 32u) {
        const uint32_t n = (p.n_lights - base < 32u) ? p.n_lights - base : 32u;
        uint32_t cand = 0u;
        for (uint32_t k = 0; k < n; k++) {
            const v4f cr = lgt4[(base + k) * 6u];
            const f3 oc = o - mk(cr.x, cr.y, cr.z);
            const float half_b = dot(oc, d);
            const float c = dot(oc, oc) - cr.w * cr.w;
            const float disc = half_b * half_b - a * c;
            cand |= (disc < 0.0f) ? 0u : (1u << k);
        }
        while (cand != 0u) {
            const uint32_t k = (uint32_t)__ffs((int)cand) - 1u;
            cand &= cand - 1u;
            const v4f cr = lgt4[(base + k) * 6u];
            const float t = isect_sphere(o, d, a, mk(cr.x, cr.y, cr.z), cr.w);
            if (t > 0.001f && t < closest_t) {
                closest_t = t;
                light_idx = base + k;
            }
        }
    }
    if (light_idx != 0xFFFFFFFFu) kind = K_LIGHT;
// ... 19 lines not shown
        const v4u p0 = pr[0], p1 = pr[1];
        tri_uv(p, th, uvx, uvy);
        if (p.u.color_hash_enabled != 0u) {
            use_tex = false;
            if (kind == K_TRI) m.diffuse = hash_to_color(p0.w + 1u);
        } else {
            const rb_material* mm = &p.meshes[p1.w].material;
            if (kind == K_TRI) {
                m = load_mat(mm);
                use_tex = m.tex >= 0;
            } else {
                use_tex = load_tex_index(mm) >= 0;
            }
        }
        if (kind == K_TRI) {
            prim = p0.w;
            mesh = p1.w;
            bu = th.u;
            bv = th.v;
            const v4f s = ((cf4p)p.ptris)[th.slot * 4u + 3u];
            normal = mk(s.x, s.y, s.z);
        }
    }
    if (kind == K_GROUND) m.diffuse = mk(0.5f, 0.5f, 0.5f);
    if (sphere_idx != 0xFFFFFFFFu) {
        const rb_sphere* s = p.spheres + sphere_idx;
        if (kind == K_SPHERE) {
            m = load_mat(&s->material);
            use_tex = m.tex >= 0;
            const v4f cr = ((cf4p)s)[0];
            normal = normalize(pos - mk(cr.x, cr.y, cr.z));
            prim = sphere_idx;
        } else {
            use_tex = load_tex_index(&s->material) >= 0;
        }
    }
    if (kind == K_LIGHT) {
        const rb_point_light* l = p.lights + light_idx;
        m = load_mat(&l->material);
        const v4f cr = ((cf4p)l)[0];
        normal = normalize(pos - mk(cr.x, cr.y, cr.z));
        prim = light_idx;
    }
    f3 albedo = m.metal ? m.specular : m.diffuse;
    if (!m.metal && use_tex) albedo = albedo * sample_texture(p, m.tex, uvx, uvy);
    out.h0 = v4f{closest_t, __uint_as_float(kind), __uint_as_float(prim), __uint_as_float(mesh)};
    out.h1 = v4f{bu, bv, 0.0f, 0.0f};
    out.h2 = v4f{normal.x, normal.y, normal.z, 0.0f};
    out.s0 = v4f{albedo.x, albedo.y, albedo.z, __uint_as_float((m.metal ? 1u : 0u) | (use_tex ? 2u : 0u))};
    out.s1 = v4f{m.emissive.x, m.emissive.y, m.emissive.z, __uint_as_float((uint32_t)m.tex)};
    out.s2 = v4f{uvx, uvy, 0.0f, 0.0f};
}

template <bool STATS, bool SPHTREE = true, bool PARK = true, bool JOINED = true, bool LEAN = false, bool TRIM = false>
DEV bool segment_finish(const KParams& p, Path& pt, const TriHit th, uint32_t* stack, uint32_t stride,
                        Tally<STATS>& tl) {
    const SegState st = segment_pre<STATS>(fresh_params(p), pt, th, tl);
    float closest_t = st.closest_t;
    uint32_t sphere_idx = 0xFFFFFFFFu;
    segment_spheres<STATS, SPHTREE, LEAN>(fresh_params(p), pt.o, pt.d, dot(pt.d, pt.d), closest_t, sphere_idx, stack, stride, tl);
    return segment_post<STATS, PARK, JOINED, TRIM>(fresh_params(p), pt, th, st, closest_t, sphere_idx, tl);
}

template <bool STATS, bool MULTI = true, bool JOINED = true, bool TRIP = false>
DEV bool segment(const KParams& p, Path& pt, uint32_t* stack, uint32_t stride, Tally<STATS>& tl, uint32_t box = kBoxUnknown) {
    const TriHit th = intersect_bvh<STATS, MULTI, TRIP>(fresh_params(p), pt.o, pt.d, stack, stride, tl, box);
    return segment_finish<STATS, MULTI, true, JOINED, !MULTI, TRIP && !MULTI>(p, pt, th, stack, stride, tl);
}

DEV void start_path_hashed(const KParams& p, uint32_t x, uint32_t y, uint32_t pixel_index, uint32_t sample_hash, Path& pt) {
    const Cam& c = p.cam;
    uint32_t seed = pcg(pixel_index + sample_hash);
    const float off_x = rnd(seed) - 0.5f;
    const float off_y = rnd(seed) - 0.5f;
    const float ax = (float)x + off_x, ay = (float)y + off_y;
    float qx, qy;
    if (c.fast_wh) {
        qx = __builtin_copysignf(div_newton(ax, c.wm1, c.inv_wm1), ax);
        qy = __builtin_copysignf(div_newton(ay, c.hm1, c.inv_hm1), ay);
    } else {
        qx = ax / c.wm1;
        qy = ay / c.hm1;
    }
    const float u = ((qx * 2.0f) - 1.0f) * c.aspect;
    const float v = 1.0f - qy * 2.0f;
    pt.o = ld3(c.pos);
    pt.d = normalize(((c.fov * u) * ld3(c.right) + (c.fov * v) * ld3(c.up)) + ld3(c.fwd));
    pt.seed = seed;
    pt.color = mk(0, 0, 0);
    pt.att = mk(1, 1, 1);
    pt.depth = 0;
}

DEV void start_ray_hashed(const KParams& p, uint32_t x, uint32_t y, uint32_t pixel_index, uint32_t sample_hash, f3& d, uint32_t& seed_out) {
    const Cam& c = p.cam;
    uint32_t seed = pcg(pixel_index + sample_hash);
    const float off_x = rnd(seed) - 0.5f;
    const float off_y = rnd(seed) - 0.5f;
    const float ax = (float)x + off_x, ay = (float)y + off_y;
    float qx, qy;
    if (c.fast_wh) {
        qx = __builtin_copysignf(div_newton(ax, c.wm1, c.inv_wm1), ax);
        qy = __builtin_copysignf(div_newton(ay, c.hm1, c.inv_hm1), ay);
    } else {
        qx = ax / c.wm1;
        qy = ay / c.hm1;
    }
    const float u = ((qx * 2.0f) - 1.0f) * c.aspect;
    const float v = 1.0f - qy * 2.0f;
    d = normalize(((c.fov * u) * ld3(c.right) + (c.fov * v) * ld3(c.up)) + ld3(c.fwd));
    seed_out = seed;
}

DEV void start_path(const KParams& p, uint32_t x, uint32_t y, uint32_t pixel_index, uint32_t sample_offset, Path& pt) {
    start_path_hashed(p, x, y, pixel_index, pcg(sample_offset), pt);
}

DEV uint32_t global_row(const KParams& p, uint32_t ly) {
    if (p.shard_count <= 1u) return ly;
    if (p.stripe_rows == 1u) return ly * p.shard_count + p.shard_rank;
// ... 65 lines not shown
```

renderbaby_amd/csrc/rb_engine.hpp:

```cpp
#pragma once
#include <hip/hip_runtime_api.h>

#include <algorithm>
#include <memory>
#include <mutex>
#include <string>
#include <vector>

#include "rb_color_plan.hpp"
#include "rb_internal.hpp"
#include "rb_rccl.hpp"
#include "rb_stage_timer.hpp"
#include "rb_update_plan.hpp"

namespace rb {

template <typename T>
struct DevBuf {
    T* ptr = nullptr;
    size_t count = 0;
    ~DevBuf() { release(); }
    void release() {
        if (ptr) (void)hipFree(ptr);
        ptr = nullptr;
// ... 35 lines not shown
    uint32_t root = 0, depth = 0;
    BuildRecord rec;
};

struct ChunkAccel {
    DevBuf<ChunkNode> nodes;
    DevBuf<float> a, b, c;
    DevBuf<uint32_t> rank_slot;
    DevBuf<uint32_t> pos_slot, pos_rank;
    size_t n_nodes = 0;
    uint32_t root = 0, depth = 0;
    BuildRecord rec;
};

struct OwnAccel {
    DevBuf<SphereNode> nodes;
    DevBuf<PrepTri> tris;
    DevBuf<uint32_t> slots, slot_meta, ref_parent, stack_overflow;
    DevBuf<GrazeNode> gnodes;
    DevBuf<uint32_t> gslots;
    DeviceTreeInfo info{};
    BuildRecord rec;
};

struct MeshWalks {
    bool host_mesh = false;
    bool chunk = false;
    bool own_named = false;
    bool own(uint32_t n_tris) const { return host_mesh && (own_named || n_tris >= kOwnTreeDefaultMinTriangles); }
};

}

struct rb_engine {
    std::mutex mu;
    mutable std::mutex err_mu;
    mutable std::string error;
    int device = 0;
    hipStream_t stream = nullptr;
    hipStream_t copy_stream = nullptr;
    hipStream_t accum_stream = nullptr;
    hipStream_t trace_stream = nullptr;
    hipEvent_t ev_begin = nullptr, ev_end = nullptr;
    hipEvent_t ev_top = nullptr;
    hipEvent_t ev_traced[2] = {nullptr, nullptr};
    hipEvent_t ev_accumulated[2] = {nullptr, nullptr};
    std::vector<hipEvent_t> ev_pool;
    uint32_t ev_used = 0;
    const char* last_kernel_name = "";
    rb_options opt{};

    rb::SceneFacts sc;
    bool scene_valid = false;
    rb_progressive prh{};
    bool iter_initialized = false;
    uint32_t iter_passes_per_frame = 1;

    bool prep_dirty = true;
    uint32_t prep_tri_count = 0xFFFFFFFFu;

    rb::DevBuf<rb_sphere> spheres;
    rb::DevBuf<float> sph_scan;
    rb::DevBuf<rb_point_light> lights;
    rb::DevBuf<rb_mesh> meshes;
    rb::DevBuf<rb_bvh_node> nodes;
    rb::DevBuf<uint32_t> indices;
    rb::DevBuf<rb_gpu_triangle> tris;
    rb::DevBuf<rb::PrepTri> ptris;
    rb::DevBuf<rb::PrepTriShade> pshade;
    rb::DevBuf<float> uvs;
    rb::DevBuf<uint32_t> tex_data;
    rb::DevBuf<rb_texture_info> tex_info;
    rb::DevBuf<float> srgb_lut;
    rb::FrameSlot slot[2];
    int cur = 0;
    bool spec_valid = false;
    uint32_t spec_first = 0, spec_n = 0;
    rb::DevBuf<unsigned long long> counters;
    rb::DevBuf<uint32_t> queue;
    rb::SphereAccel sph;
    rb::ChunkAccel chunk;
    rb::OwnAccel own;
    rb::BuildRecord tree;
    std::vector<rb_gpu_triangle> host_tris;
    std::vector<uint32_t> host_indices;
    size_t host_tri_len = 0, host_index_len = 0;
    bool host_tris_stale = false, host_indices_stale = false;
    bool stack_depth_covers = true;
    rb::DevBuf<float> colors;
    size_t color_part_floats = 0;
    uint64_t color_budget = 0;

    rb::DevBuf<rb_ray> q_rays;
    rb::DevBuf<rb_hit> q_hits;
    rb::DevBuf<rb_surface> q_surf;
    rb::DevBuf<float> q_tmax;
    rb::DevBuf<uint8_t> q_occl;
    rb::DevBuf<float> rad_colors;
    rb::DevBuf<uint32_t> rad_seeds, rad_queue;
    rb::DevBuf<rb_radiance> rad_out;
    rb::DevBuf<rb_surfel> hemi_surfels;
    rb::DevBuf<rb_openness> hemi_open;
    rb::DevBuf<rb_probe> probe_pos;
    rb::DevBuf<rb_sh9> probe_out;
    rb::DevBuf<rb_probe_depth> depth_out;
    rb::DevBuf<rb_emitter> emit_table, emit_given;
// ... 89 lines not shown
```

renderbaby_amd/csrc/rb_internal.hpp:

```cpp
#pragma once

#include <cstddef>
#include <cstdint>
#include <string>
#include <vector>

#include "../../include/rb_abi.h"

#if defined(__HIPCC__) || defined(__HIP__)
#define RB_HD __host__ __device__
#else
#define RB_HD
#endif

namespace rb {

constexpr uint32_t kStackDepth = 32;
constexpr uint32_t kStackEntryBytes = 4;
constexpr uint32_t kDefaultStripeRows = 8;

void bvh_build(const rb_gpu_triangle* tris, size_t n_tris, std::vector<rb_bvh_node>& nodes,
               std::vector<uint32_t>& indices);
bool bvh_validate(const rb_bvh_node* nodes, uint32_t node_count, uint32_t max_stack, std::string& why,
                  uint32_t* depth_out);
// ... 202 lines not shown
    const uint32_t* tex_data;
    const rb_texture_info* tex_info;
    const float* srgb_lut;
    const SphereNode* fast_nodes;
    const GrazeNode* gnodes;
    const uint32_t* gslots;
    uint32_t fast_skip_second_pass;
    const float* fast_tris;
    const uint32_t* fast_slots;
    const uint32_t* slot_meta;
    const uint32_t* ref_parent;
    uint32_t fast_root;
    float fast_margin;
    float fast_bmin[3];
    float fast_root_amax;
    float fast_bmax[3];
    uint32_t _pad_fast;
    const ChunkNode* chunk_nodes;
    const float* chunk_a;
    const float* chunk_b;
    const float* chunk_c;
    const uint32_t* chunk_rank_slot;
    uint32_t chunk_root;
    uint32_t chunk_n;
    const SphereNode4* sph_nodes;
    const float* sph_leaf;
    const uint32_t* sph_id;
    uint32_t sph_root;
    uint32_t _pad_sph;
    const float* accum_in;
    float* accum_out;
    uint32_t* out_rgba;
    unsigned long long* counters;
    uint32_t* queue;
    float* colors;
    uint32_t n_lights;
    uint32_t n_meshes;
    uint32_t index_len;
    uint32_t n_uvs;
    uint32_t n_tex;
    uint32_t first_pass, n_passes, samples_per_pass;
    uint32_t shard_rank, shard_count, stripe_rows, local_rows;
    uint32_t stack_depth;
    uint32_t blocks_per_cu;
    uint32_t queue_batch;
    uint32_t queue_groups;
    uint32_t queue_region;
    uint32_t no_leaf_stepping;
    uint32_t lds_mode;
    uint32_t magic_S, magic_tiles_x;
    uint32_t* stack_overflow;
    Cam cam;
    const float* sph_scan;
};

struct LaunchInfo {
    uint32_t grid, block;
    size_t lds_bytes;
    const char* kernel_name;
};

enum QueryWalk : uint32_t { kWalkPlain, kWalkBvh, kWalkChunk };
inline QueryWalk query_walk(KParams& p) {
    if (p.u.bvh_node_count > 1u && !p.no_leaf_stepping && p.chunk_nodes != nullptr) return kWalkChunk;
    p.fast_nodes = nullptr;
    return (p.u.bvh_node_count > 1u || p.sph_nodes != nullptr) ? kWalkBvh : kWalkPlain;
}

struct QueryArgs {
    const rb_ray* rays;
    rb_hit* hits;
    rb_surface* surf;
    uint32_t n;
    uint32_t win_x, win_y, win_w, win_h;
    uint32_t win_global;
};
#ifndef RB_QUERY_PIECE_LOG2
#define RB_QUERY_PIECE_LOG2 22
#endif
constexpr uint32_t kQueryPiece = 1u << RB_QUERY_PIECE_LOG2;
int launch_query(const KParams& p, const QueryArgs& q, void* stream, LaunchInfo* info);
struct OcclArgs {
    QueryArgs q;
    const float* tmax;
    uint8_t* out;
    uint32_t mask;
};
int launch_occluded(const KParams& p, const OcclArgs& a, void* stream, LaunchInfo* info);
struct RadArgs {
    const rb_ray* rays;
    const uint32_t* seeds;
    float* colors;
    rb_radiance* out;
    uint32_t* queue;
    uint32_t n;
    uint32_t seed_base;
    uint32_t first_sample, samples;
    uint32_t batch, magic_S;
};
int launch_radiance(const KParams& p, const RadArgs& a, void* stream, LaunchInfo* info, bool records = false);
struct CamGenArgs {
    rb_camera_ex cam;
    rb_ray* recs;
    uint32_t* seeds;
    uint32_t first_pixel;
    uint32_t n;
    uint32_t item_base;
    uint32_t first_sample, samples;
    uint32_t linear;
};
int launch_camera_rays(const CamGenArgs& g, void* stream);
struct HemiGenArgs {
// ... 142 lines not shown
```

renderbaby_amd/csrc/rb_kernels.hip:

```cpp
#include "rb_device_shade.hpp"

namespace rb {
namespace {
constexpr float kChunkFMax = 1.5e5f;
constexpr float kChunkKS = 24.0f * 5.9604645e-8f * 1.01f;
constexpr float kChunkKP = 12.0f * 5.9604645e-8f * 1.01f;
constexpr float kChunkKT = 11.0f * 5.9604645e-8f * 1.01f;
constexpr float kChunkKD = 16.0f * 5.9604645e-8f * 1.01f;
}
}
#define RB_CHUNK_MARGINS_DEFINED
#include "rb_device_chunk.hpp"
#include "rb_launch_plan.hpp"
#include "rb_host_cam.hpp"

#pragma clang fp contract(off)

namespace rb {
namespace {

constexpr uint32_t kPixelBlock = 256;

template <bool STATS>
__global__ void __launch_bounds__(kPixelBlock) k_pixel(const KParams p) {
// ... 264 lines not shown
            uint32_t b = 0;
            if (lane == 0u) b = atomicAdd(p.queue, batch);
            b = (uint32_t)__builtin_amdgcn_readfirstlane((int)b);
            if (b >= total_items) return false;
            loc_next = b;
            loc_end = (total_items - b < batch) ? total_items : b + batch;
            return true;
        }
        while (tried < p.queue_groups) {
            uint32_t b = 0;
            if (lane == 0u) b = atomicAdd(p.queue + grp * kQueueStride, batch);
            b = (uint32_t)__builtin_amdgcn_readfirstlane((int)b);
            uint32_t it = 0;
            if (band_item(p, grp, b, total_items, it)) {
                loc_next = it;
                loc_end = (total_items - it < batch) ? total_items : it + batch;
                return true;
            }
            grp = (grp + 1u == p.queue_groups) ? 0u : grp + 1u;
            tried++;
        }
        return false;
    }

    template <class IsIdle, class OnItem>
    DEV void refill(const KParams& p, uint32_t lane, uint32_t total_items, uint32_t S, uint32_t tiles_x,
                    uint32_t sample_base, IsIdle&& is_idle, OnItem&& on_item) {
        unsigned long long idle = __ballot(is_idle());
        for (int round = 0; round < 2 && idle != 0ull; round++) {
            if (loc_next == loc_end) {
                if (exhausted) break;
                if (!reserve(p, lane, total_items)) {
                    exhausted = true;
                    break;
                }
            }
            const ItemRows rows = item_rows(p, loc_next, S, tiles_x, sample_base);
            const uint32_t avail = loc_end - loc_next;
            const uint32_t rank = (uint32_t)__popcll(idle & ((1ull << lane) - 1ull));
            const bool take = ((idle >> lane) & 1ull) != 0ull && rank < avail;
            const uint32_t n_idle = (uint32_t)__popcll(idle);
            const uint32_t taken = n_idle < avail ? n_idle : avail;
            if (take) {
                uint32_t x = 0, y = 0, sample_hash = 0;
                if (item_pixel(p, rows, rank, x, y, sample_hash)) on_item(loc_next + rank, x, y, sample_hash);
            }
            loc_next += taken;
            idle = __ballot(is_idle());
            if (taken == n_idle) break;
        }
    }
};

template <bool STATS, bool MULTI, bool STAGED, bool JOINED>
DEV void trace_body(const KParams& p, v4f* s_ring) {
    extern __shared__ __attribute__((aligned(16))) uint32_t s_stack[];
    const uint32_t tid = threadIdx.x;
    const uint32_t lane = tid & 63u;
    const uint32_t tiles_x = (p.u.width + 7u) / 8u;
    const uint32_t tiles_y = (p.local_rows + 7u) / 8u;
    const uint32_t S = p.n_passes * p.samples_per_pass;
    const uint32_t total_items = tiles_x * tiles_y * S * 64u;
    float4* __restrict__ colors = reinterpret_cast<float4*>(p.colors);
    Tally<STATS> tl;
    ColorRing cring(s_ring, tid >> 6, lane, STAGED ? kRingWaveStaged : kRingWave);
    bool active = false, exhausted = false;
    uint32_t item = 0;
    uint32_t loc_next = 0, loc_end = 0;
    const uint32_t batch = p.queue_batch;
    {
        const uint64_t first = (uint64_t)(blockIdx.x * (kTraceBlock / 64u) + (tid >> 6)) * batch;
        if (first < total_items) {
            loc_next = (uint32_t)__builtin_amdgcn_readfirstlane((int)(uint32_t)first);
            loc_end = (total_items - loc_next < batch) ? total_items : loc_next + batch;
        }
    }
    Path pt;
    pt.depth = 0;

    for (;;) {
        unsigned long long idle = __ballot(!active);
        uint32_t box = kBoxUnknown;
        for (int round = 0; round < 2 && idle != 0ull; round++) {
            if (loc_next == loc_end) {
                if (exhausted) break;
                uint32_t b = 0;
                if (lane == 0u) b = atomicAdd(p.queue, batch);
                b = (uint32_t)__builtin_amdgcn_readfirstlane((int)b);
                if (b >= total_items) {
                    exhausted = true;
                    break;
                }
                loc_next = b;
                loc_end = (total_items - b < batch) ? total_items : b + batch;
            }
            const KParams& rp = fresh_params(p);
            const uint32_t rS = rp.n_passes * rp.samples_per_pass, r_tiles_x = (rp.u.width + 7u) / 8u;
            const uint32_t r_sample_base = rp.first_pass * rp.samples_per_pass, r_width = rp.u.width;
            const uint32_t direct_mask = (rp.queue_batch % (kRingRows * 64u)) ? kDirect : 0u;
            const ItemRows rows = item_rows(rp, loc_next, rS, r_tiles_x, r_sample_base);
            const uint32_t avail = loc_end - loc_next;
            const uint32_t rank = (uint32_t)__popcll(idle & ((1ull << lane) - 1ull));
            const bool take = !active && rank < avail;
            const uint32_t n_idle = (uint32_t)__popcll(idle);
            const uint32_t taken = n_idle < avail ? n_idle : avail;
            if constexpr (STAGED) {
                if (rows.in0 == 0u || rows.in0 + taken > 64u) {
                    const uint32_t nx = rows.in0 != 0u ? 1u : 0u, row = (loc_next >> 6) + nx;
                    cring.open_row(colors, lane, row, active, item);
                    cring.stage_row(rp, lane, row, rows.tx[nx], rows.ty[nx], rows.hs[nx]);
                    __builtin_amdgcn_fence(__ATOMIC_ACQ_REL, "wavefront");
                }
                if (take) {
                    const uint32_t it = loc_next + rank;
                    if (cring.take(it, pt.d, pt.seed, box)) {
                        pt.o = ld3(rp.cam.pos);
                        pt.color = mk(0, 0, 0);
                        pt.att = mk(1, 1, 1);
                        pt.depth = 0;
                        item = it;
                        if (rp.u.max_depth > 0u) {
                            active = true;
                        } else {
                            colors[it] = make_float4(0.0f, 0.0f, 0.0f, 0.0f);
                            tl.paths++;
                        }
                    }
                }
            } else {
                if (direct_mask == 0u) {
                    if (rows.in0 == 0u) cring.open_row(colors, lane, loc_next >> 6, active, item);
                    else if (rows.in0 + taken > 64u) cring.open_row(colors, lane, (loc_next >> 6) + 1u, active, item);
                }
                if (take) {
                    const uint32_t it = loc_next + rank;
                    uint32_t x = 0, y = 0, sample_hash = 0;
                    if (item_pixel(rp, rows, rank, x, y, sample_hash)) {
                        start_path_hashed(rp, x, y, y * r_width + x, sample_hash, pt);
                        item = it | direct_mask;
                        if (rp.u.max_depth > 0u) {
                            active = true;
                        } else {
                            colors[it] = make_float4(0.0f, 0.0f, 0.0f, 0.0f);
                            tl.paths++;
                        }
                    }
                }
            }
            loc_next += taken;
            idle = __ballot(!active) & ~0ull;
            if (taken == n_idle) break;
        }
        if (__ballot(active) == 0ull && exhausted && loc_next == loc_end) break;
        if (active) {
            const bool alive = segment<STATS, MULTI, JOINED, !MULTI>(p, pt, &s_stack[tid], kTraceBlock, tl, box);
            if (!alive) {
                cring.finish(colors, item, pt.color);
                tl.paths++;
                active = false;
            }
        }
    }
    for (uint32_t k = 0; k < kRingRows; k++) cring.drain(colors, lane, k);
    flush_tally<STATS>(tl, fresh_params(p).counters);
}
template <bool STATS, bool MULTI, int WAVES = RB_TRACE_WAVES>
__global__ void __launch_bounds__(kTraceBlock, WAVES) k_trace(const KParams p) {
    __shared__ __attribute__((aligned(16))) v4f s_ring[(kTraceBlock / 64u) * (MULTI ? kRingWave : kRingWaveStaged)];
    trace_body<STATS, MULTI, !MULTI, !(STATS && MULTI)>(p, s_ring);
}
template <bool STATS, bool MULTI, int WAVES = RB_TRACE_WAVES>
__global__ void __launch_bounds__(kTraceBlock, WAVES) k_trace_direct(const KParams p) {
    __shared__ __attribute__((aligned(16))) v4f s_ring[(kTraceBlock / 64u) * kRingRows * 64u];
    trace_body<STATS, MULTI, false, STATS || MULTI>(p, s_ring);
}

#ifndef RB_BVH_WAVES
#define RB_BVH_WAVES 1
#endif
template <bool STATS, bool LDS, uint32_t BLOCK>
__global__ void __launch_bounds__(BLOCK, RB_BVH_WAVES) k_trace_bvh(const KParams p) {
    extern __shared__ __attribute__((aligned(16))) uint32_t s_stack[];
    const uint32_t tid = threadIdx.x;
    const uint32_t lane = tid & 63u;
    const uint32_t width = p.u.width;
    const uint32_t tiles_x = (width + 7u) / 8u;
    const uint32_t tiles_y = (p.local_rows + 7u) / 8u;
    const uint32_t S = p.n_passes * p.samples_per_pass;
    const uint32_t total_items = tiles_x * tiles_y * S * 64u;
    const uint32_t sample_base = p.first_pass * p.samples_per_pass;
    const uint32_t node_count = p.u.bvh_node_count;
    float4* __restrict__ colors = reinterpret_cast<float4*>(p.colors);
    const cf4p nodes = (cf4p)p.nodes;
    const cf4p ptris = (cf4p)p.ptris;
    uint32_t* const stack = stack_column(s_stack, tid);
    Tally<STATS> tl;

    v4f* const lds_nodes = reinterpret_cast<v4f*>(s_stack + p.stack_depth * BLOCK);
    v4f* const lds_tris = lds_nodes + node_count * 3u;
    if constexpr (LDS) {
        const v4f* gn = reinterpret_cast<const v4f*>(p.nodes);
        const v4f* gt = reinterpret_cast<const v4f*>(p.ptris);
        for (uint32_t i = tid; i < node_count * 3u; i += BLOCK) lds_nodes[i] = gn[i];
        for (uint32_t i = tid; i < p.index_len * 3u; i += BLOCK) {
            const uint32_t slot = i / 3u, part = i - slot * 3u;
            lds_tris[i] = gt[slot * 4u + part];
        }
        __syncthreads();
    }
    auto node_q = [&](uint32_t idx, uint32_t part) -> v4f {
        if constexpr (LDS) return lds_nodes[idx * 3u + part];
        else return nodes[idx * 3u + part];
    };
    auto tri_q = [&](uint32_t slot, uint32_t part) -> v4f {
        if constexpr (LDS) return lds_tris[slot * 3u + part];
        else return ptris[slot * 4u + part];
    };

    enum : uint32_t { IDLE = 0, BEGIN = 1, TRAV = 2, FINISH = 3 };
    uint32_t state = IDLE;
    uint32_t item = 0;
    ItemQueue iq(p, total_items);
    Path pt;
    pt.depth = 0;
    TriHit th;
    th.hit = false;
    th.t = 1e20f;
    th.u = th.v = 0.0f;
// ... 755 lines not shown
                                                       uint32_t width, uint32_t height, uint32_t padded_rows,
                                                       uint32_t stripe_rows, uint32_t n) {
    const uint32_t x = blockIdx.x * 256u + threadIdx.x;
    if (x >= width) return;
    for (uint32_t y = blockIdx.y; y < height; y += gridDim.y) {
        const uint32_t s = y / stripe_rows, r = y - s * stripe_rows;
        const uint32_t rank = s % n, local_row = (s / n) * stripe_rows + r;
        frame[(size_t)y * width + x] = gathered[((size_t)rank * padded_rows + local_row) * width + x];
    }
}

}

int device_cu_count(int device) {
    hipDeviceProp_t prop;
    if (hipGetDeviceProperties(&prop, device) != hipSuccess) return 256;
    return prop.multiProcessorCount > 0 ? prop.multiProcessorCount : 256;
}

uint32_t device_cu_count_cached() {
    static int cached[64] = {0};
    int dev = 0;
    (void)hipGetDevice(&dev);
    if (dev < 0 || dev >= 64) return (uint32_t)device_cu_count(dev);
    if (cached[dev] == 0) cached[dev] = device_cu_count(dev);
    return (uint32_t)cached[dev];
}

uint32_t stream_kernel_max_threads(uint32_t blocks_per_cu) {
    return device_cu_count_cached() * (blocks_per_cu ? blocks_per_cu : 8u) * 256u;
}

Cam host_cam(const rb_uniforms& u) {
    auto fast_den = [](float b) {
        uint32_t x;
        __builtin_memcpy(&x, &b, 4);
        x &= 0x7FFFFFFFu;
        return (x - 0x0D800000u) < 0x64000000u && (x - 0x21800000u) < 0x3C000000u && (x & 0x007FFFFFu) != 0x007FFFFFu;
    };
    Cam c{};
    const CamBasis b = host_cam_basis(u.camera, u.width, u.height);
    c.aspect = b.aspect;
    for (int i = 0; i < 3; i++) c.pos[i] = u.camera.pos[i], c.fwd[i] = b.fwd[i], c.right[i] = b.right[i], c.up[i] = b.up[i];
    c.fov = b.fov;
    c.wm1 = b.wm1;
    c.hm1 = b.hm1;
    c.fast_wh = (RB_FAST_DIV && fast_den(c.wm1) && fast_den(c.hm1)) ? 1u : 0u;
    c.inv_wm1 = c.fast_wh ? 1.0f / c.wm1 : 0.0f;
    c.inv_hm1 = c.fast_wh ? 1.0f / c.hm1 : 0.0f;
    return c;
}

using TraceKernel = void (*)(const KParams);
constexpr LaunchConsts kLaunchConsts = {kTraceBlock, kRingRows, kTraceManyItems, kChunkWaveLds, kSphWaveLds, RB_SPH_WAVES, RB_CHUNK_WAVES, RB_XCD_BANDS != 0};
template <bool STATS>
static TraceKernel trace_kernel(const LaunchPlan& pl) {
    switch (pl.variant) {
        case kTraceSph: return k_trace_sph<STATS>;
        case kTraceChunk: return pl.sph_tree ? k_trace_chunk<STATS, true> : k_trace_chunk<STATS, false>;
        case kTraceFast: return k_trace_fast<STATS>;
        case kTraceBvhLds: return k_trace_bvh<STATS, true, 1024u>;
        case kTraceBvh: return k_trace_bvh<STATS, false, kTraceBlock>;
        case kTracePlain: break;
    }
    if (pl.plain == kPlainMulti) return k_trace<STATS, true>;
    if constexpr (!STATS)
        if (pl.big) return pl.plain == kPlainStaged ? k_trace<false, false, RB_TRACE_WAVES_BIG> : k_trace_direct<false, false, RB_TRACE_WAVES_BIG>;
    return pl.plain == kPlainStaged ? k_trace<STATS, false> : k_trace_direct<STATS, false>;
}

int launch_render(const KParams& p_, uint32_t kernel, bool stats, void* stream_, LaunchInfo* info) {
    KParams p = p_;
    p.cam = host_cam(p.u);
    hipStream_t stream = static_cast<hipStream_t>(stream_);
    LaunchInfo li{};
    const size_t lds = (size_t)kStackEntryBytes * p.stack_depth * 256u;
    li.lds_bytes = lds;
    if (kernel == RB_KERNEL_PIXEL) {
        const uint32_t tiles_x = (p.u.width + 15u) / 16u, tiles_y = (p.local_rows + 15u) / 16u;
        li.grid = tiles_x * tiles_y;
        li.block = kPixelBlock;
        li.kernel_name = "k_pixel";
        if (li.grid == 0) return 0;
        if (stats)
            hipLaunchKernelGGL(k_pixel<true>, dim3(li.grid), dim3(li.block), lds, stream, p);
        else
            hipLaunchKernelGGL(k_pixel<false>, dim3(li.grid), dim3(li.block), lds, stream, p);
    } else if (kernel == RB_KERNEL_QUEUE) {
        const uint64_t items = (uint64_t)((p.u.width + 7u) / 8u) * ((p.local_rows + 7u) / 8u) * 64u;
        li.grid = persistent_blocks(items, kQueueBlock, device_cu_count_cached(), p.blocks_per_cu ? p.blocks_per_cu : 8u);
        li.block = kQueueBlock;
        li.kernel_name = "k_queue";
        if (li.grid == 0) return 0;
        hipError_t e = hipMemsetAsync(p.queue, 0, sizeof(uint32_t), stream);
        if (e != hipSuccess) return (int)e;
        if (stats)
            hipLaunchKernelGGL(k_queue<true>, dim3(li.grid), dim3(li.block), lds, stream, p);
        else
            hipLaunchKernelGGL(k_queue<false>, dim3(li.grid), dim3(li.block), lds, stream, p);
    } else {
        int dev = 0;
        (void)hipGetDevice(&dev);
        const LaunchPlan pl = plan_launch(p, stats, device_cu_count_cached(), max_dynamic_lds(dev), kLaunchConsts);
        li = pl.li;
        if (li.grid == 0) return 0;
        KParams q = p;
        q.queue_batch = pl.queue_batch, q.queue_groups = pl.queue_groups, q.queue_region = pl.queue_region;
        q.magic_S = pl.magic_S, q.magic_tiles_x = pl.magic_tiles_x;
        hipError_t e = hipSuccess;
        if (pl.queue_groups > 1u) {
            QueueInit qi;
            for (uint32_t g = 0; g < kQueueGroups; g++) qi.start[g] = pl.queue_start[g];
            hipLaunchKernelGGL(k_queue_init, dim3(1), dim3(64), 0, stream, p.queue, qi);
            e = hipGetLastError();
        } else {
            e = hipMemsetD32Async(reinterpret_cast<hipDeviceptr_t>(p.queue), (int)pl.queue_start[0], 1, stream);
        }
        if (e != hipSuccess) return (int)e;
        const TraceKernel fn = stats ? trace_kernel<true>(pl) : trace_kernel<false>(pl);
        if (pl.variant == kTraceBvhLds) {
            e = hipFuncSetAttribute(reinterpret_cast<const void*>(fn), hipFuncAttributeMaxDynamicSharedMemorySize, (int)li.lds_bytes);
            if (e != hipSuccess) return (int)e;
        }
        hipLaunchKernelGGL(fn, dim3(li.grid), dim3(li.block), li.lds_bytes, stream, q);
    }
    if (info) *info = li;
    return (int)hipGetLastError();
}

int launch_accumulate(const KParams& p, void* stream_) {
    const uint64_t tiles = (uint64_t)((p.u.width + 7u) / 8u) * ((p.local_rows + 7u) / 8u);
    if (tiles == 0 || p.n_passes * p.samples_per_pass == 0) return 0;
    hipLaunchKernelGGL(k_accumulate, dim3((uint32_t)((tiles + 3u) / 4u)), dim3(256), 0, static_cast<hipStream_t>(stream_), p);
    return (int)hipGetLastError();
}

int launch_prep_tris(const rb_gpu_triangle* tris, uint32_t tri_count, const uint32_t* indices,
                     uint32_t index_len, PrepTri* out, PrepTriShade* shade, void* stream_) {
    if (index_len == 0) return 0;
    hipStream_t stream = static_cast<hipStream_t>(stream_);
    const uint32_t block = 256, grid = (index_len + block - 1) / block;
    hipLaunchKernelGGL(k_prep_tris, dim3(grid), dim3(block), 0, stream, tris, tri_count, indices, index_len, out,
                       shade);
    return (int)hipGetLastError();
}

int launch_prep_materials(void* first_material, uint32_t stride, uint32_t n, void* stream_) {
    if (n == 0) return 0;
    hipStream_t stream = static_cast<hipStream_t>(stream_);
    hipLaunchKernelGGL(k_prep_materials, dim3((n + 255) / 256), dim3(256), 0, stream,
                       static_cast<unsigned char*>(first_material), stride, n);
    return (int)hipGetLastError();
}

int launch_prep_sphere_scan(const rb_sphere* spheres, uint32_t n, float* out, void* stream_) {
    if (n == 0) return 0;
    hipStream_t stream = static_cast<hipStream_t>(stream_);
    hipLaunchKernelGGL(k_prep_sphere_scan, dim3((n + 255) / 256), dim3(256), 0, stream, spheres, n, reinterpret_cast<float4*>(out));
// ... 40 lines not shown
```

renderbaby_amd/csrc/rb_launch_plan.hpp:

```cpp
#pragma once
#include <algorithm>
#include <cstdint>

#include "rb_internal.hpp"

namespace rb {

struct LaunchConsts {
    uint32_t trace_block, ring_rows;
    uint64_t many_items;
    uint32_t chunk_wave_lds, sph_wave_lds;
    uint32_t sph_waves, chunk_waves;
    bool xcd_bands;
};

enum TraceVariant : uint32_t { kTracePlain, kTraceBvh, kTraceBvhLds, kTraceFast, kTraceSph, kTraceChunk };
enum PlainKind : uint32_t { kPlainMulti, kPlainStaged, kPlainDirect };

struct LaunchPlan {
    TraceVariant variant = kTracePlain;
    LaunchInfo li{};
    PlainKind plain = kPlainDirect;
    bool big = false;
    bool sph_tree = false;
    uint32_t queue_batch = 0, queue_groups = 1, queue_region = 0, magic_S = 0, magic_tiles_x = 0;
    uint32_t queue_start[kQueueGroups] = {};
};

inline uint32_t dense_blocks_per_cu(uint64_t items, uint32_t cus) { return (items >= (uint64_t)cus * 8u * 4u * 1024u) ? 8u : 4u; }

inline uint32_t persistent_blocks(uint64_t items, uint32_t block, uint32_t cus, uint32_t blocks_per_cu) {
    uint32_t blocks = cus * blocks_per_cu;
    const uint64_t needed = (items + block - 1) / block;
    if (needed < blocks) blocks = (uint32_t)needed;
    return blocks;
}

inline uint64_t reservation(uint64_t items, uint64_t waves, bool plain) {
    uint64_t batch = items / (waves * (plain ? 8u : 64u));
    batch = (batch / 64u) * 64u;
    if (batch < 64u) batch = 64u;
    if (batch > (plain ? 512u : 4096u)) batch = (plain ? 512u : 4096u);
    return batch;
}

inline uint32_t magic_of(uint64_t d) { return d > 1u ? (uint32_t)((1ull << 32) / d) : 0xFFFFFFFFu; }

inline LaunchPlan plan_launch(const KParams& p, bool stats, uint32_t cus, size_t max_lds, const LaunchConsts& k) {
    LaunchPlan pl;
    const size_t lds = (size_t)kStackEntryBytes * p.stack_depth * 256u;
    const uint64_t tiles = (uint64_t)((p.u.width + 7u) / 8u) * ((p.local_rows + 7u) / 8u);
    const uint64_t items = tiles * 64u * p.n_passes * p.samples_per_pass;
    const bool multi = p.u.bvh_node_count > 1u && !p.no_leaf_stepping;
    const size_t scene_lds = (size_t)p.u.bvh_node_count * 48u + (size_t)p.index_len * 48u;
    TraceVariant v = kTracePlain;
    if (multi && p.chunk_nodes != nullptr) v = kTraceChunk;
    else if (multi && p.fast_nodes != nullptr) v = kTraceFast;
    else if (multi) v = (p.lds_mode != 1u && lds * 4u + scene_lds <= max_lds) ? kTraceBvhLds : kTraceBvh;
    else if (p.sph_nodes != nullptr && !p.no_leaf_stepping) v = kTraceSph;
    static const char* const names[] = {"k_trace", "k_trace_bvh", "k_trace_bvh_lds", "k_trace_fast", "k_trace_sph", "k_trace_chunk"};
    pl.variant = v;
    pl.sph_tree = p.sph_nodes != nullptr;
    pl.li.kernel_name = names[v];
    pl.li.block = v == kTraceBvhLds ? 1024u : k.trace_block;
    pl.li.lds_bytes = v == kTraceBvhLds ? lds * 4u + scene_lds : v == kTraceChunk ? lds + (k.trace_block / 64u) * k.chunk_wave_lds
                                        : v == kTraceSph ? lds + (k.trace_block / 64u) * k.sph_wave_lds : lds;
    const uint32_t blocks_per_cu = v == kTraceBvhLds ? 1u : p.blocks_per_cu ? p.blocks_per_cu : v == kTraceFast ? 4u : v == kTraceSph ? k.sph_waves
                                                                                                   : v == kTraceChunk ? k.chunk_waves : dense_blocks_per_cu(items, cus);
    pl.li.grid = persistent_blocks(items, pl.li.block, cus, blocks_per_cu);
    if (pl.li.grid == 0) return pl;
    const uint64_t waves = (uint64_t)pl.li.grid * (pl.li.block / 64u);
    uint64_t batch = reservation(items, waves, v == kTracePlain);
    if (v == kTracePlain && batch >= 256u) batch = (batch / 256u) * 256u;
    if (p.queue_batch) batch = p.queue_batch;
    pl.queue_batch = (uint32_t)batch;
    pl.magic_S = magic_of((uint64_t)p.n_passes * p.samples_per_pass);
    pl.magic_tiles_x = magic_of((p.u.width + 7u) / 8u);
    const uint64_t row_items = (uint64_t)((p.u.width + 7u) / 8u) * 64u * p.n_passes * p.samples_per_pass;
    const uint64_t stripe = std::max<uint64_t>(((4u * row_items + batch - 1u) / batch) * batch, 8u * batch);
    const bool banded = v != kTracePlain && k.xcd_bands && pl.li.grid >= kQueueGroups && items >= 4u * kQueueGroups * stripe && stripe < (1ull << 30);
    if (banded) {
        pl.queue_groups = kQueueGroups;
        pl.queue_region = (uint32_t)stripe;
        for (uint32_t g = 0; g < kQueueGroups; g++) {
            const uint64_t blocks_g = (pl.li.grid + kQueueGroups - 1u - g) / kQueueGroups;
            pl.queue_start[g] = (uint32_t)std::min<uint64_t>(blocks_g * (pl.li.block / 64u) * batch, 0x7FFFFFFFull);
        }
    } else {
        pl.queue_start[0] = (uint32_t)(waves * batch);
    }
    if (v == kTracePlain) {
        pl.plain = (p.u.bvh_node_count > 1u || p.sph_nodes != nullptr) ? kPlainMulti
                   : pl.queue_batch % (k.ring_rows * 64u) == 0u        ? kPlainStaged : kPlainDirect;
        pl.big = pl.plain != kPlainMulti && !stats && items >= k.many_items;
    }
    return pl;
}

}
```

renderbaby_amd/csrc/rb_runtime.cpp:

```cpp
#include <cmath>
#include <cstdarg>
#include <cstdio>
#include <cstdlib>
#include <cstring>

#include "rb_engine.hpp"

static thread_local std::string g_create_error;

int rb::fail(const rb_engine* e, int code, const char* fmt, ...) {
    char buf[512];
    va_list ap;
    va_start(ap, fmt);
    vsnprintf(buf, sizeof buf, fmt, ap);
    va_end(ap);
    if (e) {
        std::lock_guard<std::mutex> g(e->err_mu);
        e->error = buf;
    } else {
        g_create_error = buf;
    }
    return code;
}

// ... 128 lines not shown
    int rc = rb::launch_prep_tris(e->tris.ptr, tri_count, e->indices.ptr, len, e->ptris.ptr, e->pshade.ptr, e->stream);
    if (rc) return rb::fail(e, RB_ERR_DEVICE, "prep kernel launch failed: %s", hipGetErrorString(static_cast<hipError_t>(rc)));
    e->prep_dirty = false;
    e->prep_tri_count = tri_count;
    e->chunk.rec = e->own.rec = {};
    rc = rb::build_chunk_tree(e, tri_count);
    return (rc || e->chunk.rec.built()) ? rc : rb::build_own_tree(e, tri_count);
}

rb::KParams rb::make_params(rb_engine* e, uint32_t first_pass, uint32_t n_passes, int src, int dst) {
    rb::KParams p{};
    p.u = e->sc.uniforms;
    p.u.spheres_count = rb::spheres_count(e->sc);
    p.u.bvh_node_count = rb::node_count(e->sc);
    p.u.bvh_triangle_count = rb::triangle_count(e->sc);
    p.spheres = e->spheres.ptr;
    p.sph_scan = e->sph_scan.ptr;
    p.lights = e->lights.ptr;
    p.meshes = e->meshes.ptr;
    p.nodes = e->nodes.ptr;
    p.indices = e->indices.ptr;
    p.tris = e->tris.ptr;
    p.ptris = e->ptris.ptr;
    p.pshade = e->pshade.ptr;
    p.uvs = e->uvs.ptr;
    p.tex_data = e->tex_data.ptr;
    p.tex_info = e->tex_info.ptr;
    p.srgb_lut = e->srgb_lut.ptr;
    p.accum_in = e->slot[src].accum.ptr;
    p.accum_out = e->slot[dst].accum.ptr;
    p.out_rgba = e->slot[dst].rgba.ptr;
    p.counters = e->counters.ptr;
    p.queue = e->queue.ptr;
    p.n_lights = e->sc.n_lights;
    p.n_meshes = e->sc.n_meshes;
    p.index_len = e->sc.n_indices;
    p.n_uvs = e->sc.n_uvs;
    p.n_tex = e->sc.n_tex;
    p.first_pass = first_pass;
    p.n_passes = n_passes;
    p.samples_per_pass = e->prh.samples_per_pass;
    const rb::ShardLayout rows = e->sc.layout(e->sc.height);
    p.shard_rank = rows.rank;
    p.shard_count = rows.count;
    p.stripe_rows = rows.stripe;
    p.local_rows = e->sc.local_rows;
    p.colors = e->colors.ptr;
    p.stack_depth = rb::accel_params(e, p);
    e->stack_depth_covers = p.stack_depth <= rb::kStackDepth;
    p.blocks_per_cu = e->opt._reserved[0];
    p.queue_batch = e->opt._reserved[2] ? std::min<uint32_t>(((std::min<uint32_t>(e->opt._reserved[2], 4096u) + 63u) / 64u) * 64u, 4096u) : 0u;
    p.no_leaf_stepping = e->opt._reserved[3];
    p.lds_mode = e->opt._reserved[4];
    return p;
}

int rb::require_ready(rb_engine* e) {
    if (!e->sc.initialized) return rb::fail(e, RB_ERR_NOT_INITIALIZED, "engine has not received its first update");
    if (!e->scene_valid) return rb::fail(e, RB_ERR_DEVICE, "the last update failed half-way on the device; send the scene again");
    if (!e->sc.have_uniforms) return rb::fail(e, RB_ERR_UNIFORMS_NOT_INITIALIZED, "Uniforms must be initialized");
    return RB_OK;
}

void rb::copy_error(rb_engine* g, const rb_engine* part) {
    std::string msg;
    {
        std::lock_guard<std::mutex> l(part->err_mu);
        msg = part->error;
    }
    std::lock_guard<std::mutex> l(g->err_mu);
    g->error = "device " + std::to_string(part->device) + ": " + msg;
}

namespace {

int clear_accum(rb_engine* e) {
    const size_t px = static_cast<size_t>(e->sc.width) * e->sc.padded_rows;
    e->spec_valid = false;
    if (px) HIP_TRY(e, hipMemsetAsync(e->slot[e->cur].accum.ptr, 0, px * 16, e->stream));
    return RB_OK;
}

int accumulate_timing(rb_engine* e) {
    float ms = 0.0f;
    if (e->last_launches > 0) {
        HIP_TRY(e, hipEventSynchronize(e->ev_end));
        HIP_TRY(e, hipEventElapsedTime(&ms, e->ev_begin, e->ev_end));
    }
    e->last_dispatch_ms = ms;
    if (e->timing_pending) {
        e->stats.kernel_ms += ms;
        for (uint32_t i = 0; i + 4 <= e->ev_used; i += 4) {
            float t = 0.0f, a = 0.0f;
            HIP_TRY(e, hipEventElapsedTime(&t, e->ev_pool[i], e->ev_pool[i + 1]));
            HIP_TRY(e, hipEventElapsedTime(&a, e->ev_pool[i + 2], e->ev_pool[i + 3]));
            e->stats.trace_ms += t;
            e->stats.accumulate_ms += a;
        }
        e->timing_pending = false;
    }
    return RB_OK;
}

uint64_t color_budget_bytes(rb_engine* e) {
    if (e->opt._reserved[1]) return static_cast<uint64_t>(e->opt._reserved[1]) << 20;
    if (e->color_budget == 0) {
// ... 27 lines not shown
    *plan_out = pl;
    return RB_OK;
}

int queue_group(rb_engine* e, uint32_t first_pass, uint32_t n_passes, int src, int dst, const rb::ColorPlan& pl) {
    const uint32_t kernel = rb::kernel_of(e->opt);
    const bool stats = (e->opt.flags & RB_FLAG_STATS) != 0;
    const bool two_phase = kernel == RB_KERNEL_STREAM;
    const bool overlap = two_phase && pl.parts == 2;
    hipStream_t acc = overlap ? e->accum_stream : e->stream;
    HIP_TRY(e, hipEventRecord(e->ev_begin, e->stream));
    if (overlap) {
        HIP_TRY(e, hipEventRecord(e->ev_top, e->stream));
        HIP_TRY(e, hipStreamWaitEvent(acc, e->ev_top, 0));
        HIP_TRY(e, hipStreamWaitEvent(e->trace_stream, e->ev_top, 0));
    }
    uint32_t launches = 0;
    e->ev_used = 0;
    for (uint32_t done = 0; done < n_passes;) {
        const uint32_t n = std::min(pl.chunk, n_passes - done);
        const uint32_t part = overlap ? launches % 2u : 0u;
        hipStream_t ts = part ? e->trace_stream : e->stream;
        rb::KParams p = make_params(e, first_pass + done, n, done == 0 ? src : dst, dst);
        if (!e->stack_depth_covers) return rb::fail(e, RB_ERR_DEVICE, "internal: a traversal is deeper than its LDS stack column (%u entries)", p.stack_depth);
        if (two_phase) p.colors = e->colors.ptr + part * e->color_part_floats;
        p.queue = e->queue.ptr + part * rb::kQueueWords;
        rb::LaunchInfo li{};
        hipEvent_t ev[4] = {nullptr, nullptr, nullptr, nullptr};
        if (e->ev_used + 4 <= 1024) {
            while (e->ev_pool.size() < e->ev_used + 4) {
                hipEvent_t x;
                HIP_TRY(e, hipEventCreate(&x));
                e->ev_pool.push_back(x);
            }
            for (int i = 0; i < 4; ++i) ev[i] = e->ev_pool[e->ev_used + i];
            e->ev_used += 4;
        }
        if (overlap && launches >= 2) HIP_TRY(e, hipStreamWaitEvent(ts, e->ev_accumulated[part], 0));
        if (ev[0]) HIP_TRY(e, hipEventRecord(ev[0], ts));
        int rc = rb::launch_render(p, kernel, stats, ts, &li);
        if (rc) return rb::fail(e, RB_ERR_DEVICE, "render kernel launch failed: %s", hipGetErrorString(static_cast<hipError_t>(rc)));
        if (ev[1]) HIP_TRY(e, hipEventRecord(ev[1], ts));
        if (overlap) {
            HIP_TRY(e, hipEventRecord(e->ev_traced[part], ts));
            HIP_TRY(e, hipStreamWaitEvent(acc, e->ev_traced[part], 0));
        }
        if (ev[2]) HIP_TRY(e, hipEventRecord(ev[2], acc));
        if (two_phase) {
            rc = rb::launch_accumulate(p, acc);
            if (rc) return rb::fail(e, RB_ERR_DEVICE, "accumulate kernel launch failed: %s", hipGetErrorString(static_cast<hipError_t>(rc)));
        }
        if (ev[3]) HIP_TRY(e, hipEventRecord(ev[3], acc));
        if (overlap) HIP_TRY(e, hipEventRecord(e->ev_accumulated[part], acc));
        if (li.kernel_name) e->last_kernel_name = li.kernel_name;
        done += n;
        launches++;
    }
    if (overlap) HIP_TRY(e, hipStreamWaitEvent(e->stream, e->ev_accumulated[(launches - 1u) % 2u], 0));
    HIP_TRY(e, hipEventRecord(e->ev_end, e->stream));
    HIP_TRY(e, hipEventRecord(e->slot[dst].done, e->stream));
    e->last_launches = launches;
    e->timing_pending = true;
    e->stats.launches += launches;
    return RB_OK;
}

int dispatch(rb_engine* e, uint32_t first_pass, uint32_t n_passes, int src, int dst) {
    int rc = ensure_prepared(e);
    if (rc) return rc;
    if (n_passes == 0 || e->sc.width == 0 || e->sc.local_rows == 0) {
        e->last_launches = 0;
        return RB_OK;
    }
    if (e->timing_pending) {
        rc = accumulate_timing(e);
        if (rc) return rc;
    }
    rb::ColorPlan pl;
    rc = reserve_colors(e, n_passes, &pl);
    if (rc) return rc;
    rc = queue_group(e, first_pass, n_passes, src, dst, pl);
    if (rc) {
        (void)hipStreamSynchronize(e->accum_stream);
        (void)hipStreamSynchronize(e->trace_stream);
        (void)hipStreamSynchronize(e->stream);
        e->last_launches = 0;
        e->timing_pending = false;
    }
    return rc;
}

int read_slot_rgba(rb_engine* e, int slot, uint8_t* out) {
    if (!out) return rb::fail(e, RB_ERR_NULL_ARGUMENT, "rgba_out is NULL");
    const uint32_t sc = e->opt.shard_count > 1 ? e->opt.shard_count : 1;
    const size_t bytes = static_cast<size_t>(e->sc.width) * 4 * (sc == 1 ? e->sc.height : e->sc.padded_rows);
    if (bytes == 0) return RB_OK;
    hipPointerAttribute_t attr{};
    if (hipPointerGetAttributes(&attr, out) == hipSuccess && attr.type == hipMemoryTypeHost) {
        HIP_TRY(e, hipStreamWaitEvent(e->copy_stream, e->slot[slot].done, 0));
        HIP_TRY(e, hipMemcpyAsync(out, e->slot[slot].rgba.ptr, bytes, hipMemcpyDeviceToHost, e->copy_stream));
        HIP_TRY(e, hipStreamSynchronize(e->copy_stream));
        return RB_OK;
    }
    (void)hipGetLastError();
    HIP_TRY(e, hipEventSynchronize(e->slot[slot].done));
    HIP_TRY(e, hipMemcpy(out, e->slot[slot].rgba.ptr, bytes, hipMemcpyDeviceToHost));
    return RB_OK;
// ... 96 lines not shown
            if (px) HIP_TRY(e, hipMemsetAsync(o.rgba.ptr, 0, px * 4, e->stream));
        }
        const uint32_t n2 = std::min(per, e->prh.total_passes - e->prh.current_pass);
        rc = dispatch(e, e->prh.current_pass, n2, e->cur, 1 - e->cur);
        if (rc) return rc;
        e->spec_valid = true;
        e->spec_first = e->prh.current_pass;
        e->spec_n = n2;
    }
    return RB_OK;
}

int iter_next_locked(rb_engine* e, uint8_t* rgba_out) {
    if (!(e->prh.current_pass < e->prh.total_passes))
        return rb::fail(e, RB_ERR_NO_MORE_FRAMES, "No more frames available");
    const bool multiproc = e->net.nranks > 1;
    if (!rgba_out && !(multiproc && e->net.rank != 0)) return rb::fail(e, RB_ERR_NULL_ARGUMENT, "rgba_out is NULL");
    int rc = iter_advance(e, e->iter_passes_per_frame);
    if (rc) return rc;
    if (multiproc) {
        std::string why;
        if (rb::gather_process(e->net, e->slot[e->cur].rgba.ptr, e->sc.width, e->sc.height, e->sc.padded_rows,
                               e->sc.layout(e->sc.height).stripe, e->copy_stream, e->slot[e->cur].done,
                               rgba_out, why))
            return rb::fail(e, RB_ERR_DEVICE, "%s", why.c_str());
        return RB_OK;
    }
    return read_slot_rgba(e, e->cur, rgba_out);
}

rb_engine* create_single(const rb_config* cfg, const rb_options& opt) {
    if (opt.shard_count > 1 && opt.shard_rank >= opt.shard_count) {
        rb::fail(nullptr, RB_ERR_INVALID_OPTIONS, "shard_rank %u >= shard_count %u", opt.shard_rank, opt.shard_count);
        return nullptr;
    }
    if (opt.kernel > RB_KERNEL_STREAM) { rb::fail(nullptr, RB_ERR_INVALID_OPTIONS, "unknown kernel %u", opt.kernel); return nullptr; }
    if ((opt.flags & rb::kBuildTreeFlags) == rb::kBuildTreeFlags) {
        rb::fail(nullptr, RB_ERR_INVALID_OPTIONS, "RB_FLAG_BUILD_TREE and RB_FLAG_BUILD_TREE_HOST exclude each other");
        return nullptr;
    }
    int dev = opt.device;
    if (dev < 0) {
        if (hipGetDevice(&dev) != hipSuccess) { rb::fail(nullptr, RB_ERR_DEVICE, "no HIP device available"); return nullptr; }
    }
    if (hipSetDevice(dev) != hipSuccess) { rb::fail(nullptr, RB_ERR_DEVICE, "hipSetDevice(%d) failed", dev); return nullptr; }
    rb_engine* e = new rb_engine();
    e->device = dev;
    e->opt = opt;
    e->sc.own_tree = rb::builds_tree(opt);
    e->sc.shard_rank = opt.shard_rank, e->sc.shard_count = opt.shard_count, e->sc.stripe_rows = opt.stripe_rows;
    if (const char* rw = std::getenv("RB_REFERENCE_WALK"); rw && rw[0] == '1')
        e->opt.flags = (e->opt.flags & ~(rb::kOwnTreeFlags | RB_FLAG_DEVICE_LBVH | RB_FLAG_CHUNK_WALK | RB_FLAG_SKIP_NEAR_DEGENERATE)) |
                       RB_FLAG_REFERENCE_WALK;
    auto bail = [&](const char* what, hipError_t st) -> rb_engine* {
        rb::fail(nullptr, RB_ERR_DEVICE, "%s failed: %s", what, hipGetErrorString(st));
        rb_destroy(e);
        return nullptr;
    };
    hipError_t st;
    if ((st = hipStreamCreateWithFlags(&e->stream, hipStreamNonBlocking)) != hipSuccess) return bail("hipStreamCreate", st);
    if ((st = hipStreamCreateWithFlags(&e->copy_stream, hipStreamNonBlocking)) != hipSuccess) return bail("hipStreamCreate", st);
    if ((st = hipStreamCreateWithFlags(&e->accum_stream, hipStreamNonBlocking)) != hipSuccess) return bail("hipStreamCreate", st);
    if ((st = hipStreamCreateWithFlags(&e->trace_stream, hipStreamNonBlocking)) != hipSuccess) return bail("hipStreamCreate", st);
    for (hipEvent_t* x : {&e->ev_top, &e->ev_traced[0], &e->ev_traced[1], &e->ev_accumulated[0], &e->ev_accumulated[1]})
        if ((st = hipEventCreateWithFlags(x, hipEventDisableTiming)) != hipSuccess) return bail("hipEventCreate", st);
    if ((st = hipEventCreate(&e->ev_begin)) != hipSuccess) return bail("hipEventCreate", st);
    if ((st = hipEventCreate(&e->ev_end)) != hipSuccess) return bail("hipEventCreate", st);
    for (rb::FrameSlot& s : e->slot)
        if ((st = hipEventCreateWithFlags(&s.done, hipEventDisableTiming)) != hipSuccess) return bail("hipEventCreate", st);
    if ((st = e->counters.resize(rb::C_COUNT)) != hipSuccess) return bail("hipMalloc(counters)", st);
    if ((st = e->queue.resize(2 * rb::kQueueWords)) != hipSuccess) return bail("hipMalloc(queue)", st);
    if ((st = hipMemsetAsync(e->counters.ptr, 0, sizeof(unsigned long long) * rb::C_COUNT, e->stream)) != hipSuccess)
        return bail("hipMemset(counters)", st);
    float lut[256];
    for (int i = 0; i < 256; ++i) lut[i] = powf(static_cast<float>(i) / 255.0f, 2.2f);
    if ((st = e->srgb_lut.resize(256)) != hipSuccess) return bail("hipMalloc(lut)", st);
    if ((st = hipMemcpy(e->srgb_lut.ptr, lut, sizeof lut, hipMemcpyHostToDevice)) != hipSuccess) return bail("hipMemcpy(lut)", st);
    const rb_uniforms* u = static_cast<const rb_uniforms*>(cfg->uniforms.ptr);
    e->prh.samples_per_pass = 1;
    e->prh.total_samples = u->total_samples;
    e->prh.total_passes = u->total_samples;
    e->prh.current_pass = 0;
    return e;
}

bool check_create(const rb_config* cfg) {
    g_create_error.clear();
    int rc = rb::check_tags(cfg, g_create_error);
    if (!rc) rc = rb::check_first_config(cfg, g_create_error);
    return rc == RB_OK;
}

rb_engine* create_impl(const rb_config* cfg, const rb_options* opt_in) {
    if (!check_create(cfg)) return nullptr;
    rb_options opt{};
    opt.device = -1;
    if (opt_in) opt = *opt_in;
    return create_single(cfg, opt);
}

#define PART_TRY(g, part, call)            \
    do {                                   \
        rb::set_device(part);              \
        const int _rc = (call);            \
        if (_rc) {                         \
            copy_error((g), (part));       \
// ... 471 lines not shown
    e->stats.mesh_hits = c[rb::C_MESH_HITS];
    *out = e->stats;
    return RB_OK;
}

static int part_reset_stats(rb_engine* e);

int rb_reset_stats(rb_engine* e) {
    if (!e) return RB_ERR_NULL_ARGUMENT;
    std::lock_guard<std::mutex> lock(e->mu);
    if (rb::is_group(e)) {
        for (auto& p : e->parts) PART_TRY(e, p.get(), part_reset_stats(p.get()));
        return RB_OK;
    }
    rb::set_device(e);
    return part_reset_stats(e);
}

static int part_reset_stats(rb_engine* e) {
    {
        const int rc = accumulate_timing(e);
        if (rc) return rc;
    }
    HIP_TRY(e, hipMemsetAsync(e->counters.ptr, 0, sizeof(unsigned long long) * rb::C_COUNT, e->stream));
    e->stats = rb_stats{};
    return RB_OK;
}

int rb_last_dispatch_ms(rb_engine* e, float* ms) {
    if (!e || !ms) return RB_ERR_NULL_ARGUMENT;
    std::lock_guard<std::mutex> lock(e->mu);
    if (rb::is_group(e)) {
        *ms = 0.0f;
        for (auto& p : e->parts) {
            PART_TRY(e, p.get(), accumulate_timing(p.get()));
            *ms = std::max(*ms, p->last_dispatch_ms);
        }
        return RB_OK;
    }
    rb::set_device(e);
    int rc = accumulate_timing(e);
    if (rc) return rc;
    *ms = e->last_dispatch_ms;
    return RB_OK;
}

const char* rb_version(void) { return "renderbaby-hip 0.3 (gfx950)"; }

const char* rb_last_kernel_name(const rb_engine* e) {
    if (!e) return "";
    return rb::is_group(e) ? e->parts[0]->last_kernel_name : e->last_kernel_name;
}

int rb_device_name(int device, char* buf, size_t buf_len) {
    if (!buf || buf_len == 0) return RB_ERR_NULL_ARGUMENT;
    hipDeviceProp_t prop;
    if (device < 0 && hipGetDevice(&device) != hipSuccess) return RB_ERR_DEVICE;
    if (hipGetDeviceProperties(&prop, device) != hipSuccess) return RB_ERR_DEVICE;
    snprintf(buf, buf_len, "%s (%s, %d CUs)", prop.name, prop.gcnArchName, prop.multiProcessorCount);
    return RB_OK;
}

int rb_debug_walk_profile(uint64_t out64[64], int reset) {
    if (!out64) return RB_ERR_NULL_ARGUMENT;
    static_assert(sizeof(unsigned long long) == sizeof(uint64_t), "counter width");
    if (hipDeviceSynchronize() != hipSuccess) return RB_ERR_DEVICE;
    return rb::debug_walk_profile(reinterpret_cast<unsigned long long*>(out64), reset) == 0 ? RB_OK : RB_ERR_DEVICE;
}

}
```

renderbaby_amd/csrc/rb_update_plan.hpp:

```cpp
#pragma once
#include <algorithm>
#include <cstdarg>
#include <cstdint>
#include <cstdio>
#include <string>
#include <vector>

#include "rb_internal.hpp"

namespace rb {

struct ShardLayout {
    uint32_t rank = 0, count = 1, stripe = kDefaultStripeRows;
    uint32_t whole_rows = 0;
    uint32_t owned = 0;
    uint32_t padded = 0;
    uint32_t global_row(uint32_t local) const { return count == 1 ? local : ((local / stripe) * count + rank) * stripe + local % stripe; }
};
inline ShardLayout shard_layout(uint32_t height, uint32_t shard_rank, uint32_t shard_count, uint32_t stripe_rows) {
    ShardLayout l;
    l.rank = shard_rank, l.count = shard_count > 1 ? shard_count : 1, l.stripe = stripe_rows ? stripe_rows : kDefaultStripeRows;
    l.whole_rows = l.owned = l.padded = height;
    if (l.count > 1) {
        const uint32_t stripes = (height + l.stripe - 1) / l.stripe;
        const uint32_t mine = l.rank < stripes ? (stripes - l.rank + l.count - 1) / l.count : 0;
        l.padded = ((stripes + l.count - 1) / l.count) * l.stripe;
        l.whole_rows = l.owned = mine * l.stripe;
        if (mine && (stripes - 1) % l.count == l.rank) l.owned -= stripes * l.stripe - height;
    }
    return l;
}

struct SceneFacts {
    bool initialized = false;
    bool have_uniforms = false;
    uint32_t n_spheres = 0, n_lights = 0, n_meshes = 0, n_nodes = 0, n_indices = 0, n_tris = 0, n_uvs = 0, n_tex = 0;
    uint32_t last_change_spheres = RB_KEEP, last_change_nodes = RB_KEEP, last_change_tris = RB_KEEP;
    uint32_t last_spheres_sent = 0;
    uint32_t bvh_stack = 0;
    uint32_t max_mesh_index = 0;
    std::vector<rb_bvh_node> host_nodes;
    rb_uniforms uniforms{};
    uint32_t width = 0, height = 0, local_rows = 0, padded_rows = 0;
    bool own_tree = false;
    uint32_t shard_rank = 0, shard_count = 0, stripe_rows = 0;
    ShardLayout layout(uint32_t h) const { return shard_layout(h, shard_rank, shard_count, stripe_rows); }
};

enum Field : uint32_t { kUniforms, kSpheres, kUvs, kMeshes, kLights, kNodes, kIndices, kTriangles, kTextures, kFieldCount };
struct Refusal {
    int code;
    const char* text;
};
struct FieldDesc {
    const char* name;
    rb_field rb_config::*member;
    uint32_t SceneFacts::*len;
    bool bvh;
    Refusal not_create;
    Refusal del;
};
constexpr Refusal kNoRefusal{RB_OK, ""};
constexpr FieldDesc kFields[kFieldCount] = {
    {"uniforms", &rb_config::uniforms, nullptr, false, {RB_ERR_INVALID_UNIFORMS, "Invalid Uniforms"}, {RB_ERR_CANNOT_DELETE_NONEXISTENT, "Cannot delete none existent"}},
    {"spheres", &rb_config::spheres, &SceneFacts::n_spheres, false, {RB_ERR_INVALID_SPHERES, "Invalid Spheres"}, kNoRefusal},
    {"uvs", &rb_config::uvs, &SceneFacts::n_uvs, false, {RB_ERR_INVALID_UVS, "Invalid UVs"}, {RB_ERR_UNSUPPORTED_DELETE, "not yet implemented: Implement UVs Deletion"}},
    {"meshes", &rb_config::meshes, &SceneFacts::n_meshes, false, {RB_ERR_INVALID_MESHES, "Invalid Meshes"}, {RB_ERR_UNSUPPORTED_DELETE, "not yet implemented: Implement meshes Deletion"}},
    {"lights", &rb_config::lights, &SceneFacts::n_lights, false, {RB_ERR_INVALID_LIGHTS, "Invalid Lights"}, {RB_ERR_UNSUPPORTED_DELETE, "not yet implemented: Implement lights Deletion"}},
    {"bvh_nodes", &rb_config::bvh_nodes, &SceneFacts::n_nodes, true, kNoRefusal, kNoRefusal},
    {"bvh_indices", &rb_config::bvh_indices, &SceneFacts::n_indices, true, kNoRefusal, kNoRefusal},
    {"bvh_triangles", &rb_config::bvh_triangles, &SceneFacts::n_tris, true, kNoRefusal, kNoRefusal},
    {"textures", &rb_config::textures, &SceneFacts::n_tex, false, {RB_ERR_INVALID_TEXTURES, "Invalid Textures"}, {RB_ERR_UNSUPPORTED_DELETE, "not yet implemented: Implement textures Deletion"}},
};
inline const rb_field& field_of(const rb_config* c, Field f) { return c->*kFields[f].member; }
inline bool has_data(const rb_field& f) { return f.change == RB_CREATE || f.change == RB_UPDATE; }

enum class Act : uint8_t { None, Take, Delete };
enum class OwnTree : uint8_t { Keep, Rebuild, Empty };
struct UpdatePlan {
    Act act[kFieldCount] = {};
    uint32_t len[kFieldCount] = {};
    bool resize = false;
    ShardLayout frame;
    OwnTree own_tree = OwnTree::Keep;
    uint32_t bvh_stack = 0, max_mesh_index = 0;
    uint32_t last_change_spheres = RB_KEEP, last_change_nodes = RB_KEEP, last_change_tris = RB_KEEP, last_spheres_sent = 0;
    bool have_uniforms = false;
};

inline int refuse(std::string& why, int code, const char* fmt, ...) __attribute__((format(printf, 3, 4)));
inline int refuse(std::string& why, int code, const char* fmt, ...) {
    char buf[512];
    va_list ap;
    va_start(ap, fmt);
    vsnprintf(buf, sizeof buf, fmt, ap);
    va_end(ap);
    why = buf;
    return code;
}

// ... 97 lines not shown
    } else if (pl.act[kNodes] == Act::Take) {
        nodes = static_cast<const rb_bvh_node*>(f_nodes.ptr);
        if (f_nodes.count >= (1ull << 31)) return refuse(why, RB_ERR_INVALID_BVH, "too many BVH nodes");
        len[kNodes] = f_nodes.count;
    } else if (pl.act[kNodes] == Act::Delete) {
        len[kNodes] = 0;
    }
    if (len[kIndices] >= (1ull << 31)) return refuse(why, RB_ERR_INVALID_BVH, "too many BVH indices");
    pl.bvh_stack = sc.bvh_stack;
    if (const uint32_t n_nodes = static_cast<uint32_t>(len[kNodes])) {
        std::string fault;
        if (!bvh_validate(nodes, n_nodes, kStackDepth, fault, &pl.bvh_stack)) return refuse(why, RB_ERR_INVALID_BVH, "%s", fault.c_str());
        for (uint32_t i = 0; i < n_nodes; ++i) {
            const rb_bvh_node& n = nodes[i];
            if (n.primitive_count > 0 && static_cast<uint64_t>(n.first_primitive) + n.primitive_count > len[kIndices])
                return refuse(why, RB_ERR_INVALID_BVH, "leaf %u covers [%u, +%u) of %llu bvh_indices", i, n.first_primitive, n.primitive_count,
                              static_cast<unsigned long long>(len[kIndices]));
        }
    }
    pl.max_mesh_index = sc.max_mesh_index;
    if (pl.act[kTriangles] == Act::Take) {
        const rb_gpu_triangle* t = static_cast<const rb_gpu_triangle*>(f_tris.ptr);
        pl.max_mesh_index = 0;
        for (size_t i = 0; i < f_tris.count; ++i) pl.max_mesh_index = std::max(pl.max_mesh_index, t[i].mesh_index);
        if (f_tris.count >= (1ull << 31)) return refuse(why, RB_ERR_INVALID_BVH, "too many triangles");
    } else if (pl.act[kTriangles] == Act::Delete) {
        pl.max_mesh_index = 0;
    }
    const uint32_t color_hash = u ? u->color_hash_enabled : sc.uniforms.color_hash_enabled;
    if (len[kTriangles] > 0 && color_hash == 0 && pl.max_mesh_index >= len[kMeshes])
        return refuse(why, RB_ERR_INVALID_MESHES, "a triangle references mesh %u of %llu", pl.max_mesh_index, static_cast<unsigned long long>(len[kMeshes]));
    if (pl.act[kTextures] == Act::Take) {
        const rb_texture* t = static_cast<const rb_texture*>(cfg->textures.ptr);
        for (size_t i = 0; i < cfg->textures.count; ++i) {
            if (t[i].width == 0 || t[i].height == 0) return refuse(why, RB_ERR_INVALID_TEXTURES, "texture %zu is empty", i);
            if (!t[i].rgba_data) return refuse(why, RB_ERR_INVALID_TEXTURES, "texture %zu has no data", i);
        }
    }
    if (u) {
        pl.frame = sc.layout(u->height);
        if (static_cast<uint64_t>(u->width) * pl.frame.padded >= (1ull << 31))
            return refuse(why, RB_ERR_INVALID_UNIFORMS, "frame of %u x %u pixels is too large", u->width, u->height);
        pl.resize = u->width != sc.width || u->height != sc.height;
    }
    for (uint32_t i = 0; i < kFieldCount; ++i) pl.len[i] = static_cast<uint32_t>(len[i]);
    pl.have_uniforms = has_data(cfg->uniforms);
    pl.last_change_spheres = cfg->spheres.change;
    pl.last_spheres_sent = has_data(cfg->spheres) ? static_cast<uint32_t>(std::min<size_t>(cfg->spheres.count, 0xFFFFFFFFu)) : 0xFFFFFFFFu;
    pl.last_change_nodes = sc.own_tree ? f_tris.change : f_nodes.change;
    pl.last_change_tris = f_tris.change;
    return RB_OK;
}

inline void commit_field(SceneFacts& sc, const UpdatePlan& pl, const rb_config* cfg, Field f) {
    if (f == kUniforms) {
        if (pl.act[f] == Act::Take) {
            sc.uniforms = *static_cast<const rb_uniforms*>(cfg->uniforms.ptr);
            sc.width = sc.uniforms.width, sc.height = sc.uniforms.height;
            sc.local_rows = pl.frame.whole_rows, sc.padded_rows = pl.frame.padded;
        }
        sc.have_uniforms = pl.have_uniforms;
        return;
    }
    if (pl.act[f] == Act::None) return;
    sc.*kFields[f].len = pl.len[f];
    if (f == kNodes) {
        const rb_bvh_node* src = static_cast<const rb_bvh_node*>(cfg->bvh_nodes.ptr);
        sc.host_nodes.assign(src, src + pl.len[f]);
    }
}

inline void commit_own_tree(SceneFacts& sc, std::vector<rb_bvh_node>&& nodes, size_t n_tris) {
    sc.n_nodes = static_cast<uint32_t>(nodes.size());
    sc.n_indices = static_cast<uint32_t>(std::max<size_t>(n_tris, 1));
    sc.host_nodes = std::move(nodes);
}

inline void commit_end(SceneFacts& sc, const UpdatePlan& pl) {
    sc.last_change_spheres = pl.last_change_spheres;
    sc.last_spheres_sent = pl.last_spheres_sent;
    sc.last_change_nodes = pl.last_change_nodes;
    sc.last_change_tris = pl.last_change_tris;
    sc.bvh_stack = pl.bvh_stack;
    sc.max_mesh_index = pl.max_mesh_index;
    sc.initialized = true;
}

inline uint32_t patch_count(uint32_t change, uint32_t given, uint32_t len) {
    if (change == RB_CREATE || change == RB_UPDATE) return len;
    if (change == RB_DELETE) return 0u;
    return std::min(given, len);
}
inline uint32_t spheres_count(const SceneFacts& sc) { return patch_count(sc.last_change_spheres, sc.uniforms.spheres_count, std::min(sc.n_spheres, sc.last_spheres_sent)); }
inline uint32_t node_count(const SceneFacts& sc) { return patch_count(sc.last_change_nodes, sc.uniforms.bvh_node_count, sc.n_nodes); }
inline uint32_t triangle_count(const SceneFacts& sc) { return patch_count(sc.last_change_tris, sc.uniforms.bvh_triangle_count, sc.n_tris); }

}
```

renderbaby_amd/engine.py:

```python
import ctypes as C
from dataclasses import dataclass
from functools import partial
from typing import Any, List, Optional

import numpy as np

from . import abi
from ._lib import load
from .bvh import own_tree_readback, sphere_tree_readback
from ._marshal import (SEEDS, Form, device_new, device_tensor, download, grid_records, host_in, host_out, host_ptr, is_tensor, probe_records,
                       ray_records, surfel_records, torch_device, upload)


class RenderError(RuntimeError):

    def __init__(self, code, message):
        super().__init__(f"[{abi.ERR.get(code, code)}] {message}")
        self.code = code
        self.message = message


@dataclass
class Change:
    tag: int
# ... 315 lines not shown
        self._check(self._lib.rb_iter_set_passes_per_frame(self._h, passes_per_frame))
        return FrameIterator(self)

    def clear(self):
        self._check(self._lib.rb_clear(self._h))

    def dispatch(self, first_pass, n_passes):
        self._check(self._lib.rb_dispatch(self._h, first_pass, n_passes))

    def reserve(self, n_passes):
        self._check(self._lib.rb_reserve(self._h, n_passes))

    def sync(self):
        self._check(self._lib.rb_sync(self._h))

    def read_rgba(self):
        w, h = self._frame_shape()
        out = np.empty((h, w, 4), dtype=np.uint8)
        self._check(self._lib.rb_read_rgba(self._h, out.ctypes.data))
        return out

    def read_accumulation(self):
        w, h = self._frame_shape()
        out = np.empty((h, w, 4), dtype=np.float32)
        self._check(self._lib.rb_read_accumulation(self._h, out.ctypes.data))
        return out

    def device_rgba(self):
        p, n = C.c_void_p(), C.c_size_t()
        self._check(self._lib.rb_device_rgba(self._h, C.byref(p), C.byref(n)))
        return p.value, n.value

    def local_rows(self):
        r, pr = C.c_uint32(), C.c_uint32()
        self._check(self._lib.rb_local_rows(self._h, C.byref(r), C.byref(pr)))
        return r.value, pr.value

    def global_row(self, local_row):
        g = C.c_uint32()
        self._check(self._lib.rb_global_row(self._h, local_row, C.byref(g)))
        return g.value

    def stats(self):
        s = abi.Stats()
        self._check(self._lib.rb_get_stats(self._h, C.byref(s)))
        return s.as_dict()

    def reset_stats(self):
        self._check(self._lib.rb_reset_stats(self._h))

    def last_kernel_name(self):
        return (self._lib.rb_last_kernel_name(self._h) or b"").decode()

    _ray_records = staticmethod(ray_records)

    def _device_call(self, fn, *args):
        import torch
        torch.cuda.current_stream(self.query_device).synchronize()
        self._check(fn(self._h, *args))
        self._check(self._lib.rb_sync(self._h))

    def _query(self, form, name, *args):
        if form.on_device:
            self._device_call(getattr(self._lib, name + "_device"), *args)
        else:
            self._check(getattr(self._lib, name)(self._h, *args))

    def _staged(self, *arrays):
        f = Form(self.query_device, *arrays, staged=True)
        return f, partial(self._query, f)

    def _last_ms(self, fn, count=1):
        ms = [C.c_float() for _ in range(count)]
        self._check(fn(self._h, *[C.byref(m) for m in ms]))
        return ms[0].value if count == 1 else tuple(m.value for m in ms)

    def _builder(self, fn):
        ms = C.c_float()
        name = (fn(self._h, C.byref(ms)) or b"").decode()
        return name, ms.value

    def cast_rays(self, origins, dirs, surfaces=False, hits_out=None, surfaces_out=None):
        return self.cast_ray_records(ray_records(origins, dirs), surfaces, hits_out, surfaces_out)

    def cast_ray_records(self, rays, surfaces=False, hits_out=None, surfaces_out=None):
        f = Form(self.query_device, rays, hits_out, surfaces_out)
        rays, rp = f.input("rays", rays, abi.RAY, flat=False)
        n = len(rays)
        hits, hp = f.output("hits_out", hits_out, abi.HIT, n)
        surf, sp = f.output("surfaces_out", surfaces_out, abi.SURFACE, n) if (surfaces or surfaces_out is not None) else (None, None)
        self._query(f, "rb_cast_rays", rp, n, hp, sp)
        return hits if surf is None else (hits, surf)

    def occluded(self, origins, dirs, tmax=None, mask=abi.MASK_ALL, out=None):
        return self.occluded_records(ray_records(origins, dirs), tmax, mask, out)

    def occluded_records(self, rays, tmax=None, mask=abi.MASK_ALL, out=None):
        f = Form(self.query_device, rays, tmax, out)
        rays, rp = f.input("rays", rays, abi.RAY, flat=False)
        n = len(rays)
        tmax, tp = f.optional("tmax", tmax, np.float32, n)
        res, op = f.output("out", out, np.uint8, n)
        self._query(f, "rb_occluded", rp, tp, n, int(mask), op)
        return res

    def trace_rays(self, origins, dirs, seeds=None, samples=1, first_sample=0, out=None):
# ... 514 lines not shown
```

Measured before the change: 39680 Msamples/s.

## Add UV-free flat trace kernels for untextured single-BVH scenes

Adds a UV template flag through triangle hit, BVH walk and shading, so that when no mesh or sphere is textured the trip asm skips tracking barycentric u/v. New k_trace_flat kernels are chosen by the launch plan when scene facts say UVs are unused. This is meant to cut VGPR pressure and moves in the triangle inner loop. It adds host-side scene scanning, more kernel variants and debug hooks, and the checkerboard path may differ if triangle UVs were ever needed.

```diff
diff --git a/include/rb_abi.h b/include/rb_abi.h
--- a/include/rb_abi.h
+++ b/include/rb_abi.h
@@ -324,6 +324,7 @@
 int rb_debug_rcp_exhaustive(uint32_t biased_exponent, uint32_t* out16);
 int rb_debug_rcp_det_exhaustive(uint32_t biased_exponent, uint32_t* out16);
 int rb_debug_triangle_trip(uint32_t n, uint32_t seed, uint32_t* out32);
+int rb_debug_triangle_trip_flat(uint32_t n, uint32_t seed, uint32_t* out32);
 int rb_debug_root_box(const float* rays, uint32_t n, const float* box6, uint32_t* out);
 int rb_debug_normalize_sites(const float* xyz, uint32_t n, uint32_t n_unit, uint32_t seed0, uint32_t n_seeds, uint32_t* out16);
 int rb_measure_salu_mix(int32_t device, uint32_t scalar_per_16, uint32_t branch, double* out3);
@@ -332,6 +333,13 @@
                             uint32_t a_count, unsigned long long* out16);
 
 const char* rb_last_kernel_name(const rb_engine* e);
+enum {
+    RB_TRACE_FORM_FLAT = 1u,
+    RB_TRACE_FORM_BIG = 4u,
+    RB_TRACE_FORM_STAGED = 8u,
+    RB_TRACE_FORM_MULTI = 16u
+};
+uint32_t rb_debug_trace_form(const rb_engine* e);
 
 typedef struct rb_ray { float origin[3]; float _pad0; float dir[3]; float _pad1; } rb_ray;
 enum { RB_HIT_NONE = 0, RB_HIT_GROUND = 1, RB_HIT_TRIANGLE = 2, RB_HIT_SPHERE = 3, RB_HIT_LIGHT = 4,
diff --git a/renderbaby_amd/_lib.py b/renderbaby_amd/_lib.py
--- a/renderbaby_amd/_lib.py
+++ b/renderbaby_amd/_lib.py
@@ -58,6 +58,8 @@
     "rb_debug_rcp_det_exhaustive": (i32, [u32, vp]),
     "rb_debug_rnd_pm1_exhaustive": (i32, [vp]),
     "rb_debug_triangle_trip": (i32, [u32, u32, vp]),
+    "rb_debug_triangle_trip_flat": (i32, [u32, u32, vp]),
+    "rb_debug_trace_form": (u32, [vp]),
     "rb_debug_root_box": (i32, [vp, u32, vp, vp]),
     "rb_debug_normalize_sites": (i32, [vp, u32, u32, u32, u32, vp]),
     "rb_measure_salu_mix": (i32, [i32, u32, u32, P(C.c_double)]),
diff --git a/renderbaby_amd/abi.py b/renderbaby_amd/abi.py
--- a/renderbaby_amd/abi.py
+++ b/renderbaby_amd/abi.py
@@ -113,6 +113,7 @@
 RB_ERR_DEVICE = 16
 
 KERNEL_DEFAULT, KERNEL_PIXEL, KERNEL_QUEUE, KERNEL_STREAM = 0, 1, 2, 3
+TRACE_FORM_FLAT, TRACE_FORM_BIG, TRACE_FORM_STAGED, TRACE_FORM_MULTI = 1, 4, 8, 16
 FLAG_STATS = 1
 FLAG_NO_SPHERE_BVH = 2
 FLAG_FAST_BVH = 4
diff --git a/renderbaby_amd/csrc/rb_debug.hip b/renderbaby_amd/csrc/rb_debug.hip
--- a/renderbaby_amd/csrc/rb_debug.hip
+++ b/renderbaby_amd/csrc/rb_debug.hip
@@ -136,6 +136,7 @@
     s = pcg(s);
     return (float)(int32_t)s * 0x1p-31f;
 }
+template <bool FLAT>
 __global__ void __launch_bounds__(256) k_triangle_trip(uint32_t n_waves, uint32_t seed, uint32_t* mismatch) {
     const uint32_t wave = (blockIdx.x * 256u + threadIdx.x) >> 6, lane = threadIdx.x & 63u;
     if (wave >= n_waves + kTripCases) return;
@@ -178,7 +179,12 @@
     if constexpr (RB_TRIP_BLOCK) asm("s_mov_b32 %0, 0x71800000" : "=s"(big));
     if (on) {
         accept_slot<true>(ra, rb_, rc, slot, o, d, want);
-        if constexpr (RB_TRIP_BLOCK) accept_trip<RB_TRIP_ASM - 1>(ra, rb_, rc, slot, o, d, big, got);
+        if constexpr (FLAT && RB_TRIP_BLOCK) {
+            TriHitT<false> flat;
+            flat.t = got.t, flat.slot = got.slot, flat.hit = false;
+            accept_trip<RB_TRIP_ASM - 1, false>(ra, rb_, rc, slot, o, d, big, flat);
+            got.t = flat.t, got.slot = flat.slot, got.u = want.u, got.v = want.v;
+        } else if constexpr (RB_TRIP_BLOCK) accept_trip<RB_TRIP_ASM - 1>(ra, rb_, rc, slot, o, d, big, got);
         else accept_slot<true>(ra, rb_, rc, slot, o, d, got);
     }
     if (__float_as_uint(want.t) != __float_as_uint(got.t) || __float_as_uint(want.u) != __float_as_uint(got.u) ||
@@ -450,7 +456,16 @@
     if (n > (1u << 26)) return RB_ERR_INVALID_OPTIONS;
     return rb::round_trip(out32, 128, 128, [&](uint32_t* d) {
         const uint32_t n_waves = (n + 63u) / 64u, waves = n_waves + rb::kTripCases;
-        hipLaunchKernelGGL(rb::k_triangle_trip, dim3((waves + 3u) / 4u), dim3(256), 0, nullptr, n_waves, seed, d);
+        hipLaunchKernelGGL(rb::k_triangle_trip<false>, dim3((waves + 3u) / 4u), dim3(256), 0, nullptr, n_waves, seed, d);
+    });
+}
+
+int rb_debug_triangle_trip_flat(uint32_t n, uint32_t seed, uint32_t* out32) {
+    if (!out32) return RB_ERR_NULL_ARGUMENT;
+    if (n > (1u << 26)) return RB_ERR_INVALID_OPTIONS;
+    return rb::round_trip(out32, 128, 128, [&](uint32_t* d) {
+        const uint32_t n_waves = (n + 63u) / 64u, waves = n_waves + rb::kTripCases;
+        hipLaunchKernelGGL(rb::k_triangle_trip<true>, dim3((waves + 3u) / 4u), dim3(256), 0, nullptr, n_waves, seed, d);
     });
 }
 
diff --git a/renderbaby_amd/csrc/rb_device_intersect.hpp b/renderbaby_amd/csrc/rb_device_intersect.hpp
--- a/renderbaby_amd/csrc/rb_device_intersect.hpp
+++ b/renderbaby_amd/csrc/rb_device_intersect.hpp
@@ -6,8 +6,9 @@
 namespace rb {
 namespace {
 
+template <bool TEXEL = true>
 DEV f3 sample_texture(const KParams& p, int32_t index, float uvx, float uvy) {
-    if (index < 0) {
+    if (!TEXEL || index < 0) {
         if (p.u.checkerboard_enabled > 0u) {
             int32_t u2 = f2i(floorf(uvx * 10.0f));
             int32_t v2 = f2i(floorf(uvy * 10.0f));
@@ -141,20 +142,31 @@
     }
 }
 
-struct TriHit {
+template <bool UV>
+struct TriHitT {
     float t, u, v;
     uint32_t slot;
     bool hit;
 };
-
-DEV void test_slot(const v4f a, const v4f b, const v4f c, uint32_t slot, f3 o, f3 d, TriHit& h) {
+template <>
+struct TriHitT<false> {
+    float t;
+    uint32_t slot;
+    bool hit;
+};
+using TriHit = TriHitT<true>;
+
+template <bool UV>
+DEV void test_slot(const v4f a, const v4f b, const v4f c, uint32_t slot, f3 o, f3 d, TriHitT<UV>& h) {
     float u, v;
     const float t = isect_triangle(o, d, mk(a.x, a.y, a.z), mk(b.x, b.y, b.z), mk(c.x, c.y, c.z), u, v);
     if (t > 0.001f && t < h.t) {
         h.hit = true;
         h.t = t;
-        h.u = u;
-        h.v = v;
+        if constexpr (UV) {
+            h.u = u;
+            h.v = v;
+        }
         h.slot = slot;
     }
 }
@@ -192,8 +204,8 @@
 #endif
 #define RB_TRIP_BLOCK (RB_TRIP_ASM != 0 && RB_FAST_RCP && RB_RCP_DET)
 
-template <int SKIP>
-DEV void accept_trip(const v4f a, const v4f b, const v4f c, uint32_t slot, f3 o, f3 d, float big, TriHit& hit) {
+template <int SKIP, bool UV = true>
+DEV void accept_trip(const v4f a, const v4f b, const v4f c, uint32_t slot, f3 o, f3 d, float big, TriHitT<UV>& hit) {
     float r8, r10, r11, r12, r13, r14, r15, r16, r17;
     uint64_t entry, keep, m, ds;
 #define RB_TRIP_HEAD                                                                                                     \
@@ -273,33 +285,56 @@
     "v_mul_f32_e32 %[r8], %[r12], %[r8]\n\t"                                                                      \
     "v_cmpx_lt_f32_e32 vcc, %[tmin], %[r8]\n\t"                                                           \
     "v_cmpx_lt_f32_e32 vcc, %[r8], %[ht]\n\t"                                                             \
-    "v_mov_b32_e32 %[hs], %[slot]\n\t"                                                                                   \
+    "v_mov_b32_e32 %[hs], %[slot]\n\t"
+#define RB_TRIP_MOVES_UV                                                                                                 \
     "v_mov_b32_e32 %[hv], %[r11]\n\t"                                                                                    \
     "v_mov_b32_e32 %[ht], %[r8]\n\t"                                                                                     \
     "v_mov_b32_e32 %[hu], %[r10]\n"
-#define RB_TRIP_OPERANDS                                                                                                 \
-    : [ht] "+v"(hit.t), [hu] "+v"(hit.u), [hv] "+v"(hit.v), [hs] "+v"(hit.slot), [r8] "=&v"(r8), [r10] "=&v"(r10),        \
+#define RB_TRIP_MOVES_T                                                                                                  \
+    "v_mov_b32_e32 %[ht], %[r8]\n"
+#define RB_TRIP_OUT_UV [ht] "+v"(hit.t), [hu] "+v"(hit.u), [hv] "+v"(hit.v), [hs] "+v"(hit.slot)
+#define RB_TRIP_OUT_T [ht] "+v"(hit.t), [hs] "+v"(hit.slot)
+#define RB_TRIP_TEMPS                                                                                                    \
+    [r8] "=&v"(r8), [r10] "=&v"(r10),                                                                                     \
       [r11] "=&v"(r11), [r12] "=&v"(r12), [r13] "=&v"(r13), [r14] "=&v"(r14), [r15] "=&v"(r15), [r16] "=&v"(r16),         \
-      [r17] "=&v"(r17), [entry] "=&s"(entry), [keep] "=&s"(keep), [m] "=&s"(m), [ds] "=&s"(ds)                            \
-    : [ax] "s"(a.x), [ay] "s"(a.y), [az] "s"(a.z), [bx] "s"(b.x), [by] "s"(b.y), [bz] "s"(b.z), [cx] "s"(c.x),            \
+      [r17] "=&v"(r17), [entry] "=&s"(entry), [keep] "=&s"(keep), [m] "=&s"(m), [ds] "=&s"(ds)
+#define RB_TRIP_IN                                                                                                       \
+    [ax] "s"(a.x), [ay] "s"(a.y), [az] "s"(a.z), [bx] "s"(b.x), [by] "s"(b.y), [bz] "s"(b.z), [cx] "s"(c.x),              \
       [cy] "s"(c.y), [cz] "s"(c.z), [slot] "s"(slot), [ox] "v"(o.x), [oy] "v"(o.y), [oz] "v"(o.z), [dx] "v"(d.x),         \
-      [dy] "v"(d.y), [dz] "v"(d.z), [eps] "s"(1e-6f), [big] "s"(big), [tmin] "s"(0.001f)                             \
-    : "vcc", "scc"
+      [dy] "v"(d.y), [dz] "v"(d.z), [eps] "s"(1e-6f)
+#define RB_TRIP_CLOBBERS "vcc", "scc"
+#define RB_TRIP_OPS_UV : RB_TRIP_OUT_UV, RB_TRIP_TEMPS : RB_TRIP_IN, [big] "s"(big), [tmin] "s"(0.001f) : RB_TRIP_CLOBBERS
+#define RB_TRIP_OPS_T : RB_TRIP_OUT_T, RB_TRIP_TEMPS : RB_TRIP_IN, [big] "s"(big), [tmin] "s"(0.001f) : RB_TRIP_CLOBBERS
 #define RB_TRIP_SKIP "s_cbranch_execz .Ltrip_end_%=\n\t"
-    if constexpr (SKIP == 2) {
-        asm volatile(RB_TRIP_HEAD RB_TRIP_SKIP RB_TRIP_TAIL RB_TRIP_SKIP RB_TRIP_LAST ".Ltrip_end_%=:\n\t"
-                     "s_mov_b64 exec, %[entry]" RB_TRIP_OPERANDS);
-    } else if constexpr (SKIP == 1) {
-        asm volatile(RB_TRIP_HEAD RB_TRIP_SKIP RB_TRIP_TAIL RB_TRIP_LAST ".Ltrip_end_%=:\n\t"
-                     "s_mov_b64 exec, %[entry]" RB_TRIP_OPERANDS);
+#define RB_TRIP_EMIT(MOVES, OPS)                                                                                         \
+    if constexpr (SKIP == 2) {                                                                                           \
+        asm volatile(RB_TRIP_HEAD RB_TRIP_SKIP RB_TRIP_TAIL RB_TRIP_SKIP RB_TRIP_LAST MOVES ".Ltrip_end_%=:\n\t"         \
+                     "s_mov_b64 exec, %[entry]" OPS);                                                                    \
+    } else if constexpr (SKIP == 1) {                                                                                    \
+        asm volatile(RB_TRIP_HEAD RB_TRIP_SKIP RB_TRIP_TAIL RB_TRIP_LAST MOVES ".Ltrip_end_%=:\n\t"                      \
+                     "s_mov_b64 exec, %[entry]" OPS);                                                                    \
+    } else {                                                                                                             \
+        asm volatile(RB_TRIP_HEAD RB_TRIP_TAIL RB_TRIP_LAST MOVES "\ts_mov_b64 exec, %[entry]" OPS);                     \
+    }
+    if constexpr (UV) {
+        RB_TRIP_EMIT(RB_TRIP_MOVES_UV, RB_TRIP_OPS_UV)
     } else {
-        asm volatile(RB_TRIP_HEAD RB_TRIP_TAIL RB_TRIP_LAST "\ts_mov_b64 exec, %[entry]" RB_TRIP_OPERANDS);
-    }
+        RB_TRIP_EMIT(RB_TRIP_MOVES_T, RB_TRIP_OPS_T)
+    }
+#undef RB_TRIP_EMIT
 #undef RB_TRIP_SKIP
 #undef RB_TRIP_HEAD
+#undef RB_TRIP_MOVES_UV
+#undef RB_TRIP_MOVES_T
+#undef RB_TRIP_OUT_UV
+#undef RB_TRIP_OUT_T
+#undef RB_TRIP_TEMPS
+#undef RB_TRIP_IN
+#undef RB_TRIP_CLOBBERS
+#undef RB_TRIP_OPS_UV
+#undef RB_TRIP_OPS_T
 #undef RB_TRIP_TAIL
 #undef RB_TRIP_LAST
-#undef RB_TRIP_OPERANDS
 }
 
 
@@ -556,13 +591,16 @@
     return w.h;
 }
 
-template <bool STATS, bool MULTI = true, bool TRIP = false>
-DEV TriHit intersect_bvh(const KParams& p, f3 o, f3 d, uint32_t* stack, uint32_t stride, Tally<STATS>& tl, uint32_t box = kBoxUnknown) {
-    TriHit h;
+template <bool STATS, bool MULTI = true, bool TRIP = false, bool UV = true>
+DEV TriHitT<UV> intersect_bvh(const KParams& p, f3 o, f3 d, uint32_t* stack, uint32_t stride, Tally<STATS>& tl, uint32_t box = kBoxUnknown) {
+    static_assert(UV || (TRIP && !MULTI && RB_TRIP_BLOCK && RB_TRIP_PLAIN != 0), "the flat forms exist for the hand-laid trip only");
+    TriHitT<UV> h;
     h.hit = false;
     h.t = 1e20f;
-    h.u = 0.0f;
-    h.v = 0.0f;
+    if constexpr (UV) {
+        h.u = 0.0f;
+        h.v = 0.0f;
+    }
     h.slot = 0u;
     const uint32_t node_count = p.u.bvh_node_count;
     if (node_count == 0u) return h;
@@ -597,7 +635,7 @@
             auto test = [&](const v4f a, const v4f b, const v4f c, uint32_t slot) {
                 if constexpr (STATS) tl.tris++;
                 const float before = h.t;
-                if constexpr (trip && RB_TRIP_BLOCK) accept_trip<RB_TRIP_ASM - 1>(a, b, c, slot, o, d, big, h);
+                if constexpr (trip && RB_TRIP_BLOCK) accept_trip<RB_TRIP_ASM - 1, UV>(a, b, c, slot, o, d, big, h);
                 else accept_slot<!MULTI>(a, b, c, slot, o, d, h);
                 if constexpr (STATS) tl.mesh_hits += (h.t != before) ? 1u : 0u;
             };
diff --git a/renderbaby_amd/csrc/rb_device_shade.hpp b/renderbaby_amd/csrc/rb_device_shade.hpp
--- a/renderbaby_amd/csrc/rb_device_shade.hpp
+++ b/renderbaby_amd/csrc/rb_device_shade.hpp
@@ -143,8 +143,8 @@
     bool use_tex, tri_won_a;
 };
 
-template <bool STATS>
-DEV SegState segment_pre(const KParams& p, const Path& pt, const TriHit th, Tally<STATS>& tl) {
+template <bool STATS, bool UV = true>
+DEV SegState segment_pre(const KParams& p, const Path& pt, const TriHitT<UV> th, Tally<STATS>& tl) {
     const f3 o = pt.o, d = pt.d;
     tl.segments++;
 
@@ -256,8 +256,8 @@
 #ifndef RB_ONE_NORMALIZE
 #define RB_ONE_NORMALIZE 1
 #endif
-template <bool STATS, bool PARK = true, bool JOINED = true, bool TRIM = false>
-DEV bool segment_post(const KParams& p, Path& pt, const TriHit th, const SegState st, float closest_t, uint32_t sphere_idx,
+template <bool STATS, bool PARK = true, bool JOINED = true, bool TRIM = false, bool UV = true>
+DEV bool segment_post(const KParams& p, Path& pt, const TriHitT<UV> th, const SegState st, float closest_t, uint32_t sphere_idx,
                       Tally<STATS>& tl) {
     const f3 o = pt.o, d = pt.d;
     const float a = dot(d, d);
@@ -374,8 +374,10 @@
         scattered = near_zero(sd) ? normal : (one_norm ? nin : normalize_for<TRIM>(sd));
         albedo = m.diffuse;
         if (use_tex) {
-            if (tri_won_a) tri_uv(p, th, uvx, uvy);
-            albedo = albedo * sample_texture(p, m.tex, uvx, uvy);
+            if constexpr (UV) {
+                if (tri_won_a) tri_uv(p, th, uvx, uvy);
+            }
+            albedo = albedo * sample_texture<UV>(p, m.tex, uvx, uvy);
         }
     }
     if (absorbed) return false;
@@ -501,20 +503,20 @@
     out.s2 = v4f{uvx, uvy, 0.0f, 0.0f};
 }
 
-template <bool STATS, bool SPHTREE = true, bool PARK = true, bool JOINED = true, bool LEAN = false, bool TRIM = false>
-DEV bool segment_finish(const KParams& p, Path& pt, const TriHit th, uint32_t* stack, uint32_t stride,
+template <bool STATS, bool SPHTREE = true, bool PARK = true, bool JOINED = true, bool LEAN = false, bool TRIM = false, bool UV = true>
+DEV bool segment_finish(const KParams& p, Path& pt, const TriHitT<UV> th, uint32_t* stack, uint32_t stride,
                         Tally<STATS>& tl) {
-    const SegState st = segment_pre<STATS>(fresh_params(p), pt, th, tl);
+    const SegState st = segment_pre<STATS, UV>(fresh_params(p), pt, th, tl);
     float closest_t = st.closest_t;
     uint32_t sphere_idx = 0xFFFFFFFFu;
     segment_spheres<STATS, SPHTREE, LEAN>(fresh_params(p), pt.o, pt.d, dot(pt.d, pt.d), closest_t, sphere_idx, stack, stride, tl);
-    return segment_post<STATS, PARK, JOINED, TRIM>(fresh_params(p), pt, th, st, closest_t, sphere_idx, tl);
-}
-
-template <bool STATS, bool MULTI = true, bool JOINED = true, bool TRIP = false>
+    return segment_post<STATS, PARK, JOINED, TRIM, UV>(fresh_params(p), pt, th, st, closest_t, sphere_idx, tl);
+}
+
+template <bool STATS, bool MULTI = true, bool JOINED = true, bool TRIP = false, bool UV = true>
 DEV bool segment(const KParams& p, Path& pt, uint32_t* stack, uint32_t stride, Tally<STATS>& tl, uint32_t box = kBoxUnknown) {
-    const TriHit th = intersect_bvh<STATS, MULTI, TRIP>(fresh_params(p), pt.o, pt.d, stack, stride, tl, box);
-    return segment_finish<STATS, MULTI, true, JOINED, !MULTI, TRIP && !MULTI>(p, pt, th, stack, stride, tl);
+    const TriHitT<UV> th = intersect_bvh<STATS, MULTI, TRIP, UV>(fresh_params(p), pt.o, pt.d, stack, stride, tl, box);
+    return segment_finish<STATS, MULTI, true, JOINED, !MULTI, TRIP && !MULTI, UV>(p, pt, th, stack, stride, tl);
 }
 
 DEV void start_path_hashed(const KParams& p, uint32_t x, uint32_t y, uint32_t pixel_index, uint32_t sample_hash, Path& pt) {
diff --git a/renderbaby_amd/csrc/rb_engine.hpp b/renderbaby_amd/csrc/rb_engine.hpp
--- a/renderbaby_amd/csrc/rb_engine.hpp
+++ b/renderbaby_amd/csrc/rb_engine.hpp
@@ -111,6 +111,8 @@
 
     rb::SceneFacts sc;
     bool scene_valid = false;
+    bool trace_uv = false;
+    uint32_t last_trace_form = 0;
     rb_progressive prh{};
     bool iter_initialized = false;
     uint32_t iter_passes_per_frame = 1;
diff --git a/renderbaby_amd/csrc/rb_internal.hpp b/renderbaby_amd/csrc/rb_internal.hpp
--- a/renderbaby_amd/csrc/rb_internal.hpp
+++ b/renderbaby_amd/csrc/rb_internal.hpp
@@ -278,12 +278,14 @@
     uint32_t* stack_overflow;
     Cam cam;
     const float* sph_scan;
+    uint32_t no_uv;
 };
 
 struct LaunchInfo {
     uint32_t grid, block;
     size_t lds_bytes;
     const char* kernel_name;
+    uint32_t trace_form;
 };
 
 enum QueryWalk : uint32_t { kWalkPlain, kWalkBvh, kWalkChunk };
diff --git a/renderbaby_amd/csrc/rb_kernels.hip b/renderbaby_amd/csrc/rb_kernels.hip
--- a/renderbaby_amd/csrc/rb_kernels.hip
+++ b/renderbaby_amd/csrc/rb_kernels.hip
@@ -340,7 +340,7 @@
     }
 };
 
-template <bool STATS, bool MULTI, bool STAGED, bool JOINED>
+template <bool STATS, bool MULTI, bool STAGED, bool JOINED, bool UV = true>
 DEV void trace_body(const KParams& p, v4f* s_ring) {
     extern __shared__ __attribute__((aligned(16))) uint32_t s_stack[];
     const uint32_t tid = threadIdx.x;
@@ -441,7 +441,7 @@
         }
         if (__ballot(active) == 0ull && exhausted && loc_next == loc_end) break;
         if (active) {
-            const bool alive = segment<STATS, MULTI, JOINED, !MULTI>(p, pt, &s_stack[tid], kTraceBlock, tl, box);
+            const bool alive = segment<STATS, MULTI, JOINED, !MULTI, UV>(p, pt, &s_stack[tid], kTraceBlock, tl, box);
             if (!alive) {
                 cring.finish(colors, item, pt.color);
                 tl.paths++;
@@ -462,6 +462,19 @@
     __shared__ __attribute__((aligned(16))) v4f s_ring[(kTraceBlock / 64u) * kRingRows * 64u];
     trace_body<STATS, MULTI, false, STATS || MULTI>(p, s_ring);
 }
+#define RB_TRACE_FLAT (RB_TRIP_BLOCK && RB_TRIP_PLAIN != 0)
+#if RB_TRACE_FLAT
+template <int WAVES>
+__global__ void __launch_bounds__(kTraceBlock, WAVES) k_trace_flat(const KParams p) {
+    __shared__ __attribute__((aligned(16))) v4f s_ring[(kTraceBlock / 64u) * kRingWaveStaged];
+    trace_body<false, false, true, true, false>(p, s_ring);
+}
+template <int WAVES>
+__global__ void __launch_bounds__(kTraceBlock, WAVES) k_trace_flat_direct(const KParams p) {
+    __shared__ __attribute__((aligned(16))) v4f s_ring[(kTraceBlock / 64u) * kRingRows * 64u];
+    trace_body<false, false, false, false, false>(p, s_ring);
+}
+#endif
 
 #ifndef RB_BVH_WAVES
 #define RB_BVH_WAVES 1
@@ -1323,7 +1336,8 @@
 }
 
 using TraceKernel = void (*)(const KParams);
-constexpr LaunchConsts kLaunchConsts = {kTraceBlock, kRingRows, kTraceManyItems, kChunkWaveLds, kSphWaveLds, RB_SPH_WAVES, RB_CHUNK_WAVES, RB_XCD_BANDS != 0};
+constexpr LaunchConsts kLaunchConsts = {kTraceBlock, kRingRows, kTraceManyItems, kChunkWaveLds, kSphWaveLds, RB_SPH_WAVES, RB_CHUNK_WAVES, RB_XCD_BANDS != 0,
+                                        RB_TRACE_FLAT != 0};
 template <bool STATS>
 static TraceKernel trace_kernel(const LaunchPlan& pl) {
     switch (pl.variant) {
@@ -1335,6 +1349,14 @@
         case kTracePlain: break;
     }
     if (pl.plain == kPlainMulti) return k_trace<STATS, true>;
+#if RB_TRACE_FLAT
+    if constexpr (!STATS)
+        if (pl.flat) {
+            constexpr int W6 = RB_TRACE_WAVES, W8 = RB_TRACE_WAVES_BIG;
+            const bool staged = pl.plain == kPlainStaged;
+            return pl.big ? (staged ? k_trace_flat<W8> : k_trace_flat_direct<W8>) : (staged ? k_trace_flat<W6> : k_trace_flat_direct<W6>);
+        }
+#endif
     if constexpr (!STATS)
         if (pl.big) return pl.plain == kPlainStaged ? k_trace<false, false, RB_TRACE_WAVES_BIG> : k_trace_direct<false, false, RB_TRACE_WAVES_BIG>;
     return pl.plain == kPlainStaged ? k_trace<STATS, false> : k_trace_direct<STATS, false>;
@@ -1375,6 +1397,9 @@
         const LaunchPlan pl = plan_launch(p, stats, device_cu_count_cached(), max_dynamic_lds(dev), kLaunchConsts);
         li = pl.li;
         if (li.grid == 0) return 0;
+        if (pl.variant == kTracePlain)
+            li.trace_form = (pl.flat ? RB_TRACE_FORM_FLAT : 0u) | (pl.big ? RB_TRACE_FORM_BIG : 0u) | (pl.plain == kPlainStaged ? RB_TRACE_FORM_STAGED : 0u) |
+                            (pl.plain == kPlainMulti ? RB_TRACE_FORM_MULTI : 0u);
         KParams q = p;
         q.queue_batch = pl.queue_batch, q.queue_groups = pl.queue_groups, q.queue_region = pl.queue_region;
         q.magic_S = pl.magic_S, q.magic_tiles_x = pl.magic_tiles_x;
diff --git a/renderbaby_amd/csrc/rb_launch_plan.hpp b/renderbaby_amd/csrc/rb_launch_plan.hpp
--- a/renderbaby_amd/csrc/rb_launch_plan.hpp
+++ b/renderbaby_amd/csrc/rb_launch_plan.hpp
@@ -12,6 +12,7 @@
     uint32_t chunk_wave_lds, sph_wave_lds;
     uint32_t sph_waves, chunk_waves;
     bool xcd_bands;
+    bool flat = false;
 };
 
 enum TraceVariant : uint32_t { kTracePlain, kTraceBvh, kTraceBvhLds, kTraceFast, kTraceSph, kTraceChunk };
@@ -22,6 +23,7 @@
     LaunchInfo li{};
     PlainKind plain = kPlainDirect;
     bool big = false;
+    bool flat = false;
     bool sph_tree = false;
     uint32_t queue_batch = 0, queue_groups = 1, queue_region = 0, magic_S = 0, magic_tiles_x = 0;
     uint32_t queue_start[kQueueGroups] = {};
@@ -93,6 +95,7 @@
         pl.plain = (p.u.bvh_node_count > 1u || p.sph_nodes != nullptr) ? kPlainMulti
                    : pl.queue_batch % (k.ring_rows * 64u) == 0u        ? kPlainStaged : kPlainDirect;
         pl.big = pl.plain != kPlainMulti && !stats && items >= k.many_items;
+        pl.flat = k.flat && pl.plain != kPlainMulti && !stats && p.no_uv != 0u;
     }
     return pl;
 }
diff --git a/renderbaby_amd/csrc/rb_runtime.cpp b/renderbaby_amd/csrc/rb_runtime.cpp
--- a/renderbaby_amd/csrc/rb_runtime.cpp
+++ b/renderbaby_amd/csrc/rb_runtime.cpp
@@ -204,6 +204,8 @@
     p.queue_batch = e->opt._reserved[2] ? std::min<uint32_t>(((std::min<uint32_t>(e->opt._reserved[2], 4096u) + 63u) / 64u) * 64u, 4096u) : 0u;
     p.no_leaf_stepping = e->opt._reserved[3];
     p.lds_mode = e->opt._reserved[4];
+    const bool single = p.u.bvh_node_count <= 1u && p.sph_nodes == nullptr && !e->trace_uv;
+    p.no_uv = (single && e->sc.no_uv && (e->sc.untex_lights || p.u.ground_enabled == 0u)) ? 1u : 0u;
     return p;
 }
 
@@ -337,7 +339,7 @@
         }
         if (ev[3]) HIP_TRY(e, hipEventRecord(ev[3], acc));
         if (overlap) HIP_TRY(e, hipEventRecord(e->ev_accumulated[part], acc));
-        if (li.kernel_name) e->last_kernel_name = li.kernel_name;
+        if (li.kernel_name) e->last_kernel_name = li.kernel_name, e->last_trace_form = li.trace_form;
         done += n;
         launches++;
     }
@@ -540,6 +542,7 @@
     if (const char* rw = std::getenv("RB_REFERENCE_WALK"); rw && rw[0] == '1')
         e->opt.flags = (e->opt.flags & ~(rb::kOwnTreeFlags | RB_FLAG_DEVICE_LBVH | RB_FLAG_CHUNK_WALK | RB_FLAG_SKIP_NEAR_DEGENERATE)) |
                        RB_FLAG_REFERENCE_WALK;
+    if (const char* uv = std::getenv("RB_TRACE_UV"); uv && uv[0] == '1') e->trace_uv = true;
     auto bail = [&](const char* what, hipError_t st) -> rb_engine* {
         rb::fail(nullptr, RB_ERR_DEVICE, "%s failed: %s", what, hipGetErrorString(st));
         rb_destroy(e);
@@ -1117,6 +1120,11 @@
     return rb::is_group(e) ? e->parts[0]->last_kernel_name : e->last_kernel_name;
 }
 
+uint32_t rb_debug_trace_form(const rb_engine* e) {
+    if (!e) return 0u;
+    return rb::is_group(e) ? e->parts[0]->last_trace_form : e->last_trace_form;
+}
+
 int rb_device_name(int device, char* buf, size_t buf_len) {
     if (!buf || buf_len == 0) return RB_ERR_NULL_ARGUMENT;
     hipDeviceProp_t prop;
diff --git a/renderbaby_amd/csrc/rb_update_plan.hpp b/renderbaby_amd/csrc/rb_update_plan.hpp
--- a/renderbaby_amd/csrc/rb_update_plan.hpp
+++ b/renderbaby_amd/csrc/rb_update_plan.hpp
@@ -45,7 +45,18 @@
     bool own_tree = false;
     uint32_t shard_rank = 0, shard_count = 0, stripe_rows = 0;
     ShardLayout layout(uint32_t h) const { return shard_layout(h, shard_rank, shard_count, stripe_rows); }
-};
+    bool untex_meshes = false, untex_spheres = false;
+    bool untex_lights = false;
+    bool no_uv = false;
+};
+
+template <typename T>
+inline bool untextured(const T* v, size_t n) {
+    if (n > 0 && !v) return false;
+    for (size_t i = 0; i < n; ++i)
+        if (v[i].material.texture_index >= 0) return false;
+    return true;
+}
 
 enum Field : uint32_t { kUniforms, kSpheres, kUvs, kMeshes, kLights, kNodes, kIndices, kTriangles, kTextures, kFieldCount };
 struct Refusal {
@@ -249,6 +260,19 @@
     return RB_OK;
 }
 
+
+inline void commit_trace_facts(SceneFacts& sc, const UpdatePlan& pl, const rb_config* cfg, Field f) {
+    const bool take = pl.act[f] == Act::Take;
+    const rb_field& fd = field_of(cfg, f);
+    switch (f) {
+        case kMeshes: sc.untex_meshes = !take || untextured(static_cast<const rb_mesh*>(fd.ptr), fd.count); break;
+        case kSpheres: sc.untex_spheres = !take || untextured(static_cast<const rb_sphere*>(fd.ptr), fd.count); break;
+        case kLights: sc.untex_lights = !take || (fd.count > 0 && untextured(static_cast<const rb_point_light*>(fd.ptr), fd.count)); break;
+        default: return;
+    }
+    sc.no_uv = sc.untex_meshes && sc.untex_spheres;
+}
+
 inline void commit_field(SceneFacts& sc, const UpdatePlan& pl, const rb_config* cfg, Field f) {
     if (f == kUniforms) {
         if (pl.act[f] == Act::Take) {
@@ -261,6 +285,7 @@
     }
     if (pl.act[f] == Act::None) return;
     sc.*kFields[f].len = pl.len[f];
+    commit_trace_facts(sc, pl, cfg, f);
     if (f == kNodes) {
         const rb_bvh_node* src = static_cast<const rb_bvh_node*>(cfg->bvh_nodes.ptr);
         sc.host_nodes.assign(src, src + pl.len[f]);
diff --git a/renderbaby_amd/engine.py b/renderbaby_amd/engine.py
--- a/renderbaby_amd/engine.py
+++ b/renderbaby_amd/engine.py
@@ -391,6 +391,9 @@
     def last_kernel_name(self):
         return (self._lib.rb_last_kernel_name(self._h) or b"").decode()
 
+    def trace_form(self):
+        return int(self._lib.rb_debug_trace_form(self._h))
+
     _ray_records = staticmethod(ray_records)
 
     def _device_call(self, fn, *args):
```

Measured after the change: 40190 Msamples/s, median of 6. 1.3% higher.
